# david-cortes/recometrics

Hardware: AMD Instinct MI355X
Metric: users/sec evaluated (all metrics, K=10) (higher is better)
Workload: dtype f32

## Files before the change

recometrics_amd/csrc/rm_device.hpp:

```cpp
#pragma once
#include <hip/hip_runtime.h>
#include <stdint.h>

namespace rm {

constexpr int WAVE = 64;
constexpr int GROUP_USERS = 32;
constexpr int TILE_ITEMS = 64;
constexpr int SWEEP_THREADS = 512;
constexpr int GROUPS_PER_BLOCK = 4;
constexpr int POS_CHUNK = 63;
constexpr int MAX_J = 6;
constexpr int STREAM_CLASS = MAX_J + 1;
constexpr int N_CLASSES = MAX_J + 2;
constexpr int IDX_EMPTY = 0x7fffffff;
constexpr int HEAVY_NPOS = 256;
enum : int { LM_LDS = 0, LM_HBM = 1, LM_HBM_APPEND = 2 };
constexpr int WAIT_VMCNT0 = 0x0F70;

enum : int { UF_NAN = 1, UF_ONLY_NDCG = 2, UF_KLEQN = 4, UF_ACTIVE = 8, UF_SKIP = 16 };

enum : int { RQ_P = 1, RQ_TP = 2, RQ_R = 4, RQ_AP = 8, RQ_TAP = 16, RQ_NDCG = 32, RQ_HIT = 64, RQ_RR = 128, RQ_ROC = 256, RQ_PR = 512 };

template <class T> struct Entry { T s; int idx; };
typedef Entry<float> ListEntry;

template <class T> struct PartialStat {
    T vmax, vmin;
    unsigned long long rocsum;
    int has_nan; int pad;
};

struct Plan {
    int n_active;
    int n_slots;
    int n_groups;
    int jmax;
    long long total_rows;
    int class_count[N_CLASSES];
    int class_offset[N_CLASSES + 1];
    int class_cursor[N_CLASSES];
    int n_long;
    int stream_enable;
    int max_npos;
    int n_stream_chunks;
    int nonfinite;
    int nonfinite_b;
    int n_noise_flagged;
    int n_heavy;
    int n_only_ndcg;
    unsigned long long amax_a, amax_b;
    int csr_bad;
    int csr_where;
    alignas(128) unsigned long long csr_desc_all[2];
    unsigned long long csr_desc_legit[2];
    unsigned long long csr_pad[12];
};
enum : int { CSR_BAD_INDPTR = 1, CSR_BAD_INDEX = 2, CSR_UNSORTED_TRAIN = 4, CSR_UNSORTED_TEST = 8 };

__device__ __forceinline__ float nan_sentinel_f() { return __int_as_float(0xffffffff); }
__device__ __forceinline__ float pos_inf_f() { return __int_as_float(0x7f800000); }
__device__ __forceinline__ float neg_inf_f() { return __int_as_float(0xff800000); }

__device__ __forceinline__ unsigned ord_key(float x) { const unsigned b = __float_as_uint(x); return b ^ ((b >> 31) ? 0xffffffffu : 0x80000000u); }
__device__ __forceinline__ float ord_unkey(unsigned k) { return __uint_as_float(k ^ ((k >> 31) ? 0x80000000u : 0xffffffffu)); }
__device__ __forceinline__ unsigned long long ord_key(double x)
{
    const unsigned long long b = (unsigned long long)__double_as_longlong(x);
    return b ^ ((b >> 63) ? 0xffffffffffffffffull : 0x8000000000000000ull);
}
__device__ __forceinline__ double ord_unkey(unsigned long long k)
{
    return __longlong_as_double((long long)(k ^ ((k >> 63) ? 0x8000000000000000ull : 0xffffffffffffffffull)));
}

template <class T> __device__ __forceinline__ T lane_bcast(T v, int src);
template <> __device__ __forceinline__ int lane_bcast<int>(int v, int src) { return __builtin_amdgcn_readlane(v, src); }
template <> __device__ __forceinline__ float lane_bcast<float>(float v, int src) { return __int_as_float(__builtin_amdgcn_readlane(__float_as_int(v), src)); }
template <> __device__ __forceinline__ double lane_bcast<double>(double v, int src)
{
    const long long b = __double_as_longlong(v);
    const unsigned lo = (unsigned)__builtin_amdgcn_readlane((int)(unsigned)b, src), hi = (unsigned)__builtin_amdgcn_readlane((int)(b >> 32), src);
    return __longlong_as_double((long long)(((unsigned long long)hi << 32) | lo));
}

__device__ __forceinline__ bool wave_any(bool c) { return __builtin_amdgcn_ballot_w64(c) != 0ull; }

template <class A> __device__ __forceinline__ const A *late_kernargs()
{
    auto p = __builtin_amdgcn_kernarg_segment_ptr();
    asm volatile("" : "+s"(p));
    return (const A *)p;
}
__device__ __forceinline__ constexpr int mfma32_row(int r, int h) { return (r & 3) + 8 * (r >> 2) + 4 * h; }

}
```

recometrics_amd/csrc/rm_finalize.hpp:

```cpp
#pragma once
#include "rm_device.hpp"
#include <type_traits>

namespace rm {

constexpr int MAX_PARTS = 128;
constexpr int FIN_THREADS = 128;
constexpr int FIN_TOPV = 64;
template <class T> inline size_t finalize_lds_bytes(int K, int n_part) { return (sizeof(T) * (size_t)(K < FIN_TOPV ? K : FIN_TOPV) + 4 * (size_t)n_part) * FIN_THREADS; }

struct AucPart { unsigned long long sum_ranks; double s1, s2; int nvalid, pad; };

template <class T, class S> struct FinalArgs {
    int m, n, K, n_part, req, cumulative, noise, gu, n_slots;
    const int *slot_user, *slot_chunk;
    const int *train_p, *test_p, *test_i; const T *test_v;
    const int *flags, *user_nslots, *uslot_base, *slot_index;
    const int *gj; const long long *grow;
    const Entry<S> *pl; const PartialStat<S> *pst; const unsigned *hist; const S *pos_score;
    const int *pos_item_tab;
    AucPart *auc_part;
    T *heavy_topv;
    unsigned char *heavy_nan;
    const int *heavy_users; int n_heavy;
    int heavy_npos, heavy_ld;
    const double *log2tab;
    T *p, *tp, *r, *ap, *tap, *ndcg, *hit, *rr, *roc, *pr;
    Entry<S> *merged;
    long long *rank_sorted;
    int *status;
    int stream_slot0;
    int rank_generic;
    int fin_slot0, fin_slot1;
    int fused_auc;
    int auc_defer_slot0;
    const S *stream_scores; long long stream_ld;
    const S *spos_score; const int *spos_item;
    unsigned *shist;
    int ext_topk; unsigned long long *sel_hi; unsigned *sel_lo; int sel_ld;
    int collected;
    int *noise_flag; Plan *plan;
};

template <class T> __device__ __forceinline__ T qnan();
template <> __device__ __forceinline__ float qnan<float>() { return __int_as_float(0x7fc00000); }
template <> __device__ __forceinline__ double qnan<double>() { return __longlong_as_double(0x7ff8000000000000ll); }

template <class T, class S>
__device__ void fill_user_nan(const FinalArgs<T, S> &a, int u)
{
    T *top8[8] = {a.p, a.tp, a.r, a.ap, a.tap, a.ndcg, a.hit, a.rr};
    for (int q = 0; q < 8; q++) {
        T *arr = top8[q];
        if (!arr) continue;
        if (!a.cumulative) arr[u] = qnan<T>();
        else for (int i = 0; i < a.K; i++) arr[(size_t)u * a.K + i] = qnan<T>();
    }
    if (a.roc) a.roc[u] = qnan<T>();
    if (a.pr) a.pr[u] = qnan<T>();
}

template <class S> __device__ __forceinline__ bool ent_before(const Entry<S> &x, const Entry<S> &y)
{
    return x.s > y.s || (x.s == y.s && x.idx < y.idx);
}

template <class T, class S>
__global__ void k_auc_slots(FinalArgs<T, S> a)
{
    const int slot = blockIdx.x * blockDim.x + threadIdx.x;
    if (slot >= a.stream_slot0) return;
    const int u = a.slot_user[slot], c = a.slot_chunk[slot];
    if (a.flags[u] & UF_ONLY_NDCG) return;
    const int te0 = a.test_p[u], npos = a.test_p[u + 1] - te0;
    const int GUr = a.gu;
    const int g = slot / GUr, ul = slot % GUr;
    const int PLg = (1 << a.gj[g]) - 1;
    const unsigned *H = a.hist + (a.grow[g] + g) * GUr + ul;
    const S *PS = a.pos_score + (a.grow[g] + g) * GUr + ul;
    const int pc = min(POS_CHUNK, npos - c * POS_CHUNK);
    unsigned long long above = 0, sum_ranks = 0;
    double s1 = 0, s2 = 0;
    int nvalid = 0;
    for (int b = PLg; b >= 1; b--) {
        above += H[(size_t)b * GUr];
        const int j = b - 1;
        if (j >= pc) continue;
        const S ps = PS[(size_t)j * GUr];
        if (isinf(ps) && ps > 0) continue;
        const unsigned long long rank = above + 1;
        sum_ranks += rank; nvalid++;
        s1 += 1. / (double)rank;
        s2 += (double)nvalid / (double)rank;
        if (a.rank_sorted) a.rank_sorted[te0 + c * POS_CHUNK + j] = (long long)rank;
    }
    AucPart r; r.sum_ranks = sum_ranks; r.s1 = s1; r.s2 = s2; r.nvalid = nvalid; r.pad = 0;
    a.auc_part[slot] = r;
}

constexpr int MERGE_WAVES = 4;
template <class T, class S>
__global__ __launch_bounds__(MERGE_WAVES * WAVE) void k_merge_positives(FinalArgs<T, S> a, int extra, int slot0)
{
    const int slot = slot0 + __builtin_amdgcn_readfirstlane((int)((blockIdx.x * blockDim.x + threadIdx.x) >> 6)), lane = threadIdx.x & 63;
    if (slot >= a.n_slots) return;
    const int u = a.slot_user[slot];
    const int K = a.K, NP = a.n_part;
    Entry<S> *L = (Entry<S> *)a.pl + ((size_t)slot * NP + extra) * K;
    S vmax = -(S)INFINITY, vmin = (S)INFINITY;
    int has_nan = 0, filled = 0;
    if (!(a.flags[u] & UF_ONLY_NDCG)) {
        const int te0 = a.test_p[u], npos = a.test_p[u + 1] - te0;
        const S *PS = a.spos_score + te0;
        const int *PI = a.spos_item + te0;
        for (int top = npos - 1; top >= 0; top -= WAVE) {
            const int i = top - lane;
            const S x = i >= 0 ? PS[i] : (S)INFINITY;
            const bool masked = isinf(x) && x > 0;
            const bool isn = x != x;
            const bool cand = !masked && !isn;
            has_nan |= isn ? 1 : 0;
            if (cand) {
                vmax = x > vmax ? x : vmax;
                vmin = x < vmin ? x : vmin;
                if (i >= 1) atomicAdd(&a.shist[te0 + i - 1], 1u);
            }
            if (filled < K) {
                const unsigned long long mk = __ballot(cand);
                const int pos = filled + __popcll(mk & ((1ull << lane) - 1ull));
                if (cand && pos < K) { L[pos].s = x; L[pos].idx = PI[i]; }
                filled += __popcll(mk);
            }
        }
    }
    #pragma unroll
    for (int d = 32; d >= 1; d >>= 1) {
        const S om = __shfl_xor(vmax, d), on = __shfl_xor(vmin, d);
        vmax = om > vmax ? om : vmax; vmin = on < vmin ? on : vmin;
        has_nan |= __shfl_xor(has_nan, d);
    }
    for (int i = (filled < K ? filled : K) + lane; i < K; i += WAVE) { L[i].s = -(S)INFINITY; L[i].idx = IDX_EMPTY; }
    if (lane == 0) {
        PartialStat<S> ps;
        ps.vmax = vmax; ps.vmin = vmin; ps.rocsum = 0; ps.has_nan = has_nan; ps.pad = 0;
        ((PartialStat<S> *)a.pst)[(size_t)slot * NP + extra] = ps;
    }
}

constexpr int STREAM_RANK_THREADS = 256;
constexpr int STREAM_RANK_ITEMS = 128;
constexpr int STREAM_RANK_LDS = 20 * 1024;
template <class S, int ILP, int LV>
__device__ __forceinline__ void rank_streamed_lds(const S *row, long long i0, int ipt, int n, const int *pit, int P, int top_rt, int lgsb_rt,
                                                  unsigned tab_addr, unsigned hist_addr)
{
    const int top = LV ? (1 << LV) : top_rt;
    const int lgsb = LV ? 14 - LV : lgsb_rt;
    typedef __attribute__((address_space(3))) const S *LdsS;
    typedef __attribute__((address_space(3))) unsigned *LdsU;
    const unsigned sb = 1u << lgsb;
    auto load_batch = [&](int it, S (&x)[ILP]) {
        #pragma unroll
        for (int q = 0; q < ILP; q++) {
            const long long item = i0 + (long long)(it + q) * STREAM_RANK_THREADS + threadIdx.x;
            x[q] = row[item < n ? item : n - 1];
        }
    };
    S nxt[ILP];
    load_batch(0, nxt);
    for (int it = 0; it < ipt; it += ILP) {
        S v[ILP]; unsigned o[ILP];
        #pragma unroll
        for (int q = 0; q < ILP; q++) {
            const long long item = i0 + (long long)(it + q) * STREAM_RANK_THREADS + threadIdx.x;
            v[q] = (nxt[q] == nxt[q] && item < n) ? nxt[q] : -(S)INFINITY; o[q] = 0;
        }
        load_batch(it + ILP, nxt);
        #pragma unroll
        for (unsigned st = ((unsigned)top >> 1) << lgsb; st >= sb; st >>= 1) {
            S pv[ILP];
            #pragma unroll
            for (int q = 0; q < ILP; q++) pv[q] = *(LdsS)(tab_addr + o[q] + st - sb);
            #pragma unroll
            for (int q = 0; q < ILP; q++) o[q] = (pv[q] < v[q]) ? o[q] + st : o[q];
        }
        S nx[ILP];
        #pragma unroll
        for (int q = 0; q < ILP; q++) nx[q] = *(LdsS)(tab_addr + o[q]);
        #pragma unroll
        for (int q = 0; q < ILP; q++) {
            int l = (int)(o[q] >> lgsb);
            if (nx[q] == v[q]) {
                const int item = (int)(i0 + (long long)(it + q) * STREAM_RANK_THREADS + threadIdx.x);
                while (l < P && *(LdsS)(tab_addr + ((unsigned)l << lgsb)) == v[q] && pit[l] > item) l++;
            }
            if (l >= 1) __hip_atomic_fetch_add((LdsU)(hist_addr + 4u * (unsigned)(l - 1)), 1u, __ATOMIC_RELAXED, __HIP_MEMORY_SCOPE_WORKGROUP);
        }
    }
}

template <class T, class S, class Count>
__device__ __forceinline__ void auc_walk_streamed(const FinalArgs<T, S> &a, int slot, int te0, int P, int lane, Count count)
{
    unsigned long long above = 0, sum_ranks = 0;
    double s2 = 0;
    int nvalid = 0;
    for (int base = P; base > 0; base -= WAVE) {
        const int j = base - 1 - lane;
        const bool live = j >= 0;
        const unsigned long long h = live ? (unsigned long long)count(j) : 0ull;
        unsigned long long incl = h;
        #pragma unroll
        for (int dd = 1; dd < WAVE; dd <<= 1) {
            const unsigned lo32 = (unsigned)__shfl_up((int)(unsigned)incl, dd), hi32 = (unsigned)__shfl_up((int)(unsigned)(incl >> 32), dd);
            if (lane >= dd) incl += ((unsigned long long)hi32 << 32) | lo32;
        }
        const S ps = live ? a.spos_score[te0 + j] : (S)0;
        const bool valid = live && !(isinf(ps) && ps > 0);
        const unsigned long long vm = __ballot(valid);
        const unsigned long long rank = above + incl + 1;
        const int myidx = nvalid + __popcll(vm & ((1ull << lane) - 1ull)) + 1;
        const double term = valid ? (double)myidx / (double)rank : 0.;
        unsigned long long rs = valid ? rank : 0ull;
        #pragma unroll
        for (int dd = 32; dd >= 1; dd >>= 1) {
            const unsigned lo32 = (unsigned)__shfl_xor((int)(unsigned)rs, dd), hi32 = (unsigned)__shfl_xor((int)(unsigned)(rs >> 32), dd);
            rs += ((unsigned long long)hi32 << 32) | lo32;
        }
        sum_ranks += rs;
        for (unsigned long long mm = vm; mm; mm &= mm - 1) s2 += lane_bcast<double>(term, __ffsll((long long)mm) - 1);
        if (a.rank_sorted && valid) a.rank_sorted[te0 + j] = (long long)rank;
        const int last = (base < WAVE ? base : WAVE) - 1;
        above += ((unsigned long long)(unsigned)__shfl((int)(unsigned)(incl >> 32), last) << 32) | (unsigned)__shfl((int)(unsigned)incl, last);
        nvalid += __popcll(vm);
    }
    if (lane == 0) { AucPart r; r.sum_ranks = sum_ranks; r.s1 = 0; r.s2 = s2; r.nvalid = nvalid; r.pad = 0; a.auc_part[slot] = r; }
}

template <class S>
__device__ __forceinline__ bool rank_block_walks(int fused_auc, int P)
{
    if (!(fused_auc & 1)) return false;
    constexpr int per = (int)sizeof(S) / 4;
    int top = 1;
    while (top <= P) top <<= 1;
    return (long long)top * per + P + 1 <= STREAM_RANK_LDS / 4;
}

#define RM_FCMP_LT(m, p, x) asm volatile("v_cmp_lt_f32 %0, %1, %2" : "=s"(m) : "v"(p), "v"(x))
#define RM_FCMP_LT_S(m, p, x) asm volatile("v_cmp_lt_f32 %0, %1, %2" : "=s"(m) : "s"(p), "v"(x))
#define RM_FSEL(d, a, b, m) asm volatile("v_cndmask_b32 %0, %1, %2, %3" : "=v"(d) : "v"(a), "v"(b), "s"(m))
template <int LV>
__device__ __forceinline__ void rank_streamed_fast(const float *row, int i0, int iters, const int *pit, int P, unsigned tab_addr, unsigned hist0_addr,
                                                   float piv_lo, float piv_root, float piv_hi)
{
    constexpr int ILP = 8;
    constexpr int LGSB = 14 - LV;
    constexpr unsigned SB = 1u << LGSB;
    constexpr unsigned Q = SB << (LV - 2);
    typedef __attribute__((address_space(3))) const float *LdsS;
    const float *src = row + i0 + (int)threadIdx.x;
    float nxt[ILP];
    #pragma unroll
    for (int q = 0; q < ILP; q++) nxt[q] = src[q * STREAM_RANK_THREADS];
    const unsigned a1 = tab_addr | Q, a2 = tab_addr | (2 * Q), a3 = tab_addr | (3 * Q);
    for (int it = 0; it < iters; it += ILP) {
        float v[ILP]; unsigned at[ILP];
        #pragma unroll
        for (int q = 0; q < ILP; q++) { v[q] = nxt[q]; at[q] = tab_addr; }
        src += ILP * STREAM_RANK_THREADS;
        if (it + ILP < iters) {
            #pragma unroll
            for (int q = 0; q < ILP; q++) nxt[q] = src[q * STREAM_RANK_THREADS];
        }
        unsigned long long mk0, mk1, mk2;
        #pragma unroll
        for (int i = 0; i < 3 * ILP + 2; i++) {
            if (i < 3 * ILP) {
                const float pv = i < ILP ? piv_lo : (i < 2 * ILP ? piv_root : piv_hi);
                if (i % 3 == 0) RM_FCMP_LT_S(mk0, pv, v[i % ILP]); else if (i % 3 == 1) RM_FCMP_LT_S(mk1, pv, v[i % ILP]); else RM_FCMP_LT_S(mk2, pv, v[i % ILP]);
            }
            if (i >= 2) {
                const int j = i - 2;
                const unsigned tgt = j < ILP ? a1 : (j < 2 * ILP ? a2 : a3);
                if (j % 3 == 0) RM_FSEL(at[j % ILP], at[j % ILP], tgt, mk0); else if (j % 3 == 1) RM_FSEL(at[j % ILP], at[j % ILP], tgt, mk1); else RM_FSEL(at[j % ILP], at[j % ILP], tgt, mk2);
            }
        }
        #pragma unroll
        for (int st = 1 << (LV - 3); st >= 1; st >>= 1) {
            float pv[ILP];
            #pragma unroll
            for (int q = 0; q < ILP; q++) pv[q] = *(LdsS)(at[q] + (unsigned)(st - 1) * SB);
            #pragma unroll
            for (int i = 0; i < ILP + 2; i++) {
                if (i == 0) __builtin_amdgcn_s_waitcnt(0xC47F); else if (i == 4) __builtin_amdgcn_s_waitcnt(0xC07F);
                if (i < ILP) { if (i % 3 == 0) RM_FCMP_LT(mk0, pv[i], v[i]); else if (i % 3 == 1) RM_FCMP_LT(mk1, pv[i], v[i]); else RM_FCMP_LT(mk2, pv[i], v[i]); }
                if (i >= 2) {
                    const int j = i - 2;
                    const unsigned cand = at[j] | ((unsigned)st * SB);
                    if (j % 3 == 0) RM_FSEL(at[j], at[j], cand, mk0); else if (j % 3 == 1) RM_FSEL(at[j], at[j], cand, mk1); else RM_FSEL(at[j], at[j], cand, mk2);
                }
            }
        }
        float nx[ILP];
        #pragma unroll
        for (int q = 0; q < ILP; q++) nx[q] = *(LdsS)(at[q]);
        bool tie = false;
        #pragma unroll
        for (int q = 0; q < ILP; q++) tie |= nx[q] == v[q];
        if (__any(tie)) {
            #pragma unroll
            for (int q = 0; q < ILP; q++) {
                if (nx[q] == v[q]) {
                    const int item = i0 + (it + q) * STREAM_RANK_THREADS + (int)threadIdx.x;
                    int l = (int)((at[q] - tab_addr) >> LGSB);
                    while (l < P && *(LdsS)(tab_addr + ((unsigned)l << LGSB)) == v[q] && pit[l] > item) l++;
                    at[q] = tab_addr + ((unsigned)l << LGSB);
                }
            }
        }
        const unsigned one = 1u;
        #pragma unroll
        for (int q = 0; q < ILP; q++) {
            const unsigned ha = hist0_addr + (((at[q] - tab_addr) >> LGSB) << 2);
            asm volatile("ds_add_u32 %0, %1" :: "v"(ha), "v"(one) : "memory");
        }
    }
    __builtin_amdgcn_s_waitcnt(0xC07F);
}

template <class T, class S>
__global__ __launch_bounds__(STREAM_RANK_THREADS) void k_rank_streamed(FinalArgs<T, S> a, int parts, int ipt, int row0)
{
    __shared__ __attribute__((aligned(16384))) char rk_smem[STREAM_RANK_LDS];
    const int d = row0 + blockIdx.x / parts, part = blockIdx.x % parts;
    const int slot = a.stream_slot0 + d;
    const int u = a.slot_user[slot];
    if (a.flags[u] & UF_ONLY_NDCG) return;
    const int te0 = a.test_p[u], P = a.test_p[u + 1] - te0;
    constexpr int WORDS = STREAM_RANK_LDS / 4;
    constexpr int per = (int)sizeof(S) / 4;
    int top = 1;
    while (top <= P) top <<= 1;
    int R = 0;
    if ((long long)top * per + P + 1 <= WORDS) { R = 1; while (R < 32 && (long long)top * 2 * R * per + P + 1 <= WORDS) R *= 2; }
    const int *pit = a.spos_item + te0;
    const S *row = a.stream_scores + (size_t)d * (size_t)a.stream_ld;
    const long long i0 = (long long)part * STREAM_RANK_THREADS * ipt;
    if (R > 0) {
        S *lds_s = (S *)rk_smem;
        unsigned *lds_h = (unsigned *)(rk_smem + sizeof(S) * (size_t)top * (size_t)R) + 1;
        for (int i = threadIdx.x; i < top * R; i += STREAM_RANK_THREADS) { const int e = i / R; lds_s[i] = e < P ? a.spos_score[te0 + e] : (S)INFINITY; }
        for (int i = threadIdx.x; i < P; i += STREAM_RANK_THREADS) lds_h[i] = 0u;
        __syncthreads();
        int lgsb = sizeof(S) == 4 ? 2 : 3;
        for (int r = R; r > 1; r >>= 1) lgsb++;
        const unsigned tab_addr = (unsigned)(size_t)(__attribute__((address_space(3))) char *)rk_smem + (unsigned)((threadIdx.x & (R - 1)) * sizeof(S));
        const unsigned hist_addr = (unsigned)(size_t)(__attribute__((address_space(3))) char *)lds_h;
        const bool full = (long long)top * R == 4096 / per;
        if (sizeof(S) == 4 && full && top >= 128 && top <= 1024 && !a.rank_generic) {
            const int inside = (int)((a.n - i0) / STREAM_RANK_THREADS);
            const int iters = inside <= 0 ? 0 : (inside < ipt ? inside : ipt) / 8 * 8;
            if (iters > 0) {
                const float *tabf = (const float *)lds_s;
                const float p_lo = tabf[(top / 4 - 1) * R], p_root = tabf[(top / 2 - 1) * R], p_hi = tabf[(3 * top / 4 - 1) * R];
                const float s_lo = __builtin_bit_cast(float, __builtin_amdgcn_readfirstlane(__builtin_bit_cast(int, p_lo)));
                const float s_root = __builtin_bit_cast(float, __builtin_amdgcn_readfirstlane(__builtin_bit_cast(int, p_root)));
                const float s_hi = __builtin_bit_cast(float, __builtin_amdgcn_readfirstlane(__builtin_bit_cast(int, p_hi)));
                const float *rowf = (const float *)row;
                const unsigned h0 = hist_addr - 4u;
                if (top == 128) rank_streamed_fast<7>(rowf, (int)i0, iters, pit, P, tab_addr, h0, s_lo, s_root, s_hi);
                else if (top == 256) rank_streamed_fast<8>(rowf, (int)i0, iters, pit, P, tab_addr, h0, s_lo, s_root, s_hi);
                else if (top == 512) rank_streamed_fast<9>(rowf, (int)i0, iters, pit, P, tab_addr, h0, s_lo, s_root, s_hi);
                else rank_streamed_fast<10>(rowf, (int)i0, iters, pit, P, tab_addr, h0, s_lo, s_root, s_hi);
            }
            if (iters < ipt) rank_streamed_lds<S, 8, 0>(row, i0 + (long long)iters * STREAM_RANK_THREADS, ipt - iters, a.n, pit, P, top, lgsb, tab_addr, hist_addr);
// ... 120 lines not shown
            }
            __syncthreads();
        }
    }
    for (int i = tid; i < K; i += SELECT_THREADS) {
        Entry<S> e;
        if (i < got) { e.s = ord_unkey((KeyT)hi[i]); e.idx = (int)~lo[i]; }
        else { e.s = (S)qnan<float>(); e.idx = -1; }
        M[i] = e;
    }
}

struct CollectGeom {
    int ublock0, n_ublocks, n_splits, tail_ublocks, tail_splits;
    int nsub, gu, lpu;
    int lane_cap;
    int extra_part;
};
template <class S> struct CollectKey;
template <> struct CollectKey<float> { typedef unsigned T; };
template <> struct CollectKey<double> { typedef unsigned long long T; };
inline int collect_capw(int K, int lane_cap) { return K <= 128 ? 512 : (K + lane_cap <= 1024 && 2 * K <= 1024 ? 1024 : 4096); }
constexpr int COLLECT_MAX_ENTRIES = 4096;
inline unsigned collect_grid(long long blocks) { return (unsigned)((blocks + 7) / 8 * 8); }
template <class T, class S, class ThrT, int CAPW>
__global__ __launch_bounds__(CAPW <= 1024 ? 256 : 64) void k_collect_topk(FinalArgs<T, S> a, CollectGeom g, const char *glists, const int *lane_cnt, const ThrT *thr_shared)
{
    typedef typename CollectKey<S>::T KeyT;
    constexpr int WPB = CAPW <= 1024 ? 4 : 1;
    __shared__ KeyT kh_all[WPB * CAPW];
    __shared__ unsigned kl_all[WPB * CAPW];
    const int lane = threadIdx.x & 63, wv_in_blk = __builtin_amdgcn_readfirstlane(threadIdx.x >> 6);
    const int per_xcd = gridDim.x >> 3;
    const int lblock = (blockIdx.x & 7) * per_xcd + (blockIdx.x >> 3);
    const int slot = lblock * WPB + wv_in_blk;
    if (slot >= a.n_slots) return;
    const int chunk = a.slot_chunk[slot], u = a.slot_user[slot];
    const ThrT bound_raw = thr_shared[slot];
    const bool live = chunk == 0;
    KeyT *kh = kh_all + wv_in_blk * CAPW;
    unsigned *kl = kl_all + wv_in_blk * CAPW;
    const int K = a.K;
    const int group = slot / g.gu, ul = slot % g.gu, gi = group % GROUPS_PER_BLOCK, blk_u = group / GROUPS_PER_BLOCK;
    const int nwaves = GROUPS_PER_BLOCK * g.nsub;
    const int rel = blk_u - g.ublock0, n_ub1 = g.n_ublocks - g.tail_ublocks;
    const bool in_tail = rel < g.tail_ublocks;
    const int nsplit = in_tail ? g.tail_splits : g.n_splits;
    const KeyT bound = (KeyT)bound_raw;
    int cur = 0;
    auto wave_sync = [&]() { __builtin_amdgcn_fence(__ATOMIC_ACQ_REL, "wavefront"); __builtin_amdgcn_wave_barrier(); };
    auto select_best = [&]() __attribute__((always_inline)) {
        if (cur <= K) return;
        wave_sync();
        constexpr int ROWS = CAPW / WAVE;
        KeyT kr[ROWS];
        #pragma unroll
        for (int r = 0; r < ROWS; r++) { const int i = r * WAVE + lane; kr[r] = i < cur ? kh[i] : (KeyT)0; }
        KeyT all_and = ~(KeyT)0, all_or = 0;
        #pragma unroll
        for (int r = 0; r < ROWS; r++) if (r * WAVE + lane < cur) { all_and &= kr[r]; all_or |= kr[r]; }
        #pragma unroll
        for (int d = 32; d >= 1; d >>= 1) { all_and &= __shfl_xor(all_and, d); all_or |= __shfl_xor(all_or, d); }
        const KeyT diff = all_and ^ all_or;
        constexpr int BITS = (int)sizeof(KeyT) * 8;
        int top = BITS - 1;
        while (top >= 0 && !((diff >> top) & 1)) top--;
        KeyT Tk = top >= 0 ? (all_and & ~(((KeyT)2 << top) - 1)) : all_and;
        for (int bit = top; bit >= 0; bit--) {
            const KeyT cand = Tk | ((KeyT)1 << bit);
            int c = 0;
            #pragma unroll
            for (int r = 0; r < ROWS; r++) c += __popcll(__ballot(kr[r] >= cand));
            if (c >= K) Tk = cand;
        }
        int n_gt = 0, n_eq = 0;
        #pragma unroll
        for (int r = 0; r < ROWS; r++) {
            const bool in = r * WAVE + lane < cur;
            n_gt += __popcll(__ballot(in && kr[r] > Tk)); n_eq += __popcll(__ballot(in && kr[r] == Tk));
        }
        const int need = K - n_gt;
        unsigned Lk = 0u;
        if (n_eq > need) {
            const int rows = (cur + WAVE - 1) / WAVE;
            for (int bit = 31; bit >= 0; bit--) {
                const unsigned cand = Lk | (1u << bit);
                int c = 0;
                for (int r = 0; r < rows; r++) { const int i = r * WAVE + lane; c += __popcll(__ballot(i < cur && kh[i] == Tk && kl[i] >= cand)); }
                if (c >= need) Lk = cand;
            }
        }
        int out = 0;
        #pragma unroll
        for (int r = 0; r < ROWS; r++) {
            if (r * WAVE >= cur) break;
            const int i = r * WAVE + lane;
            const KeyT x = kr[r]; const unsigned y = i < cur ? kl[i] : 0u;
            const bool keep = i < cur && (x > Tk || (x == Tk && y >= Lk));
            const unsigned long long m = __ballot(keep);
            if (keep) { const int at = out + __popcll(m & ((1ull << lane) - 1ull)); kh[at] = x; kl[at] = y; }
            out += __popcll(m);
        }
        cur = out;
        wave_sync();
    };
    auto sort_regs = [&](auto pr_tag) __attribute__((always_inline)) {
        constexpr int PR = decltype(pr_tag)::value, P = PR * WAVE;
        KeyT h[PR]; unsigned l[PR];
        #pragma unroll
        for (int r = 0; r < PR; r++) { const int i = r * WAVE + lane; const bool in = i < cur; h[r] = in ? kh[i] : (KeyT)0; l[r] = in ? kl[i] : 0u; }
        #pragma unroll
        for (int k2 = 2; k2 <= P; k2 <<= 1) {
            #pragma unroll
            for (int j = k2 >> 1; j > 0; j >>= 1) {
                if (j >= WAVE) {
                    const int jr = j / WAVE;
                    #pragma unroll
                    for (int r = 0; r < PR; r++) {
                        if (r & jr) continue;
                        const bool desc = (r & (k2 / WAVE)) == 0;
                        const bool lt = h[r] < h[r | jr] || (h[r] == h[r | jr] && l[r] < l[r | jr]);
                        if (desc ? lt : !lt) { const KeyT th = h[r]; h[r] = h[r | jr]; h[r | jr] = th; const unsigned tl = l[r]; l[r] = l[r | jr]; l[r | jr] = tl; }
                    }
                } else {
                    #pragma unroll
                    for (int r = 0; r < PR; r++) {
                        const KeyT oh = __shfl_xor(h[r], j); const unsigned ol = __shfl_xor(l[r], j);
                        const bool take_max = ((lane & j) == 0) == ((((r * WAVE) | lane) & k2) == 0);
                        const bool other_better = oh > h[r] || (oh == h[r] && ol > l[r]);
                        if (take_max ? other_better : !other_better) { h[r] = oh; l[r] = ol; }
                    }
                }
            }
        }
        #pragma unroll
        for (int r = 0; r < PR; r++) { kh[r * WAVE + lane] = h[r]; kl[r * WAVE + lane] = l[r]; }
        wave_sync();
    };
    auto sort_kept = [&]() __attribute__((always_inline)) {
        wave_sync();
        if (CAPW <= 1024) {
            if (cur <= 64) sort_regs(std::integral_constant<int, 1>{});
            else if (cur <= 128) sort_regs(std::integral_constant<int, 2>{});
            else if (cur <= 256) sort_regs(std::integral_constant<int, 4>{});
            else sort_regs(std::integral_constant<int, 8>{});
        } else {
            if (cur <= 512) sort_regs(std::integral_constant<int, 8>{});
            else if (cur <= 1024) sort_regs(std::integral_constant<int, 16>{});
            else sort_regs(std::integral_constant<int, 32>{});
        }
    };
    auto reduce = [&]() __attribute__((always_inline)) { select_best(); };
    auto gather = [&](int c, auto get) __attribute__((always_inline)) {
        for (int i0 = 0; i0 < c; i0 += WAVE) {
            if (cur + WAVE > CAPW) reduce();
            KeyT key = 0; unsigned low = 0u;
            const bool take = i0 + lane < c && get(i0 + lane, key, low);
            const unsigned long long m = __ballot(take);
            if (take) { const int at = cur + __popcll(m & ((1ull << lane) - 1ull)); kh[at] = key; kl[at] = low; }
            cur += __popcll(m);
        }
    };
    constexpr int G = 4;
    constexpr bool PAIRS = sizeof(S) == 4;
    const int per_range = g.nsub * g.lpu, nsrc = nsplit * per_range;
    const char *bs[G]; const int *bi[G]; int cn[G]; int cmax = 0;
    auto describe = [&](int s0) __attribute__((always_inline)) {
        size_t cidx[G]; bool on[G];
        #pragma unroll
        for (int j = 0; j < G; j++) {
            const int src = s0 + j;
            on[j] = src < nsrc;
            const int srcc = on[j] ? src : 0;
            const int sp = srcc / per_range, rem = srcc % per_range, sub = rem / g.lpu, l = rem % g.lpu;
            const int bidx = in_tail ? n_ub1 * g.n_splits + sp * g.tail_ublocks + (g.tail_ublocks - 1 - rel)
                                     : sp * n_ub1 + (g.n_ublocks - 1 - rel);
            const size_t wv = (size_t)bidx * nwaves + (size_t)(sub * GROUPS_PER_BLOCK + gi);
            const int src_lane = ul + l * g.gu;
            const char *wbase = glists + wv * ((size_t)g.lane_cap * WAVE * (sizeof(S) + 4));
            cidx[j] = wv * WAVE + src_lane;
            bs[j] = wbase + (size_t)src_lane * (PAIRS ? 8 : sizeof(S));
            bi[j] = (const int *)(wbase + (size_t)g.lane_cap * WAVE * sizeof(S)) + src_lane;
        }
        int c[G];
        #pragma unroll
        for (int j = 0; j < G; j++) c[j] = lane_cnt[cidx[j]];
        cmax = 0;
        #pragma unroll
        for (int j = 0; j < G; j++) { cn[j] = (live && on[j]) ? c[j] : 0; cmax = cn[j] > cmax ? cn[j] : cmax; }
    };
    describe(0);
    if (g.extra_part >= 0) {
        const Entry<S> *px = a.pl + ((size_t)slot * a.n_part + g.extra_part) * K;
        gather(live ? K : 0, [&](int i, KeyT &key, unsigned &low) {
            Entry<S> e;
            __builtin_memcpy(&e, px + i, sizeof(e));
            if (e.idx == IDX_EMPTY) return false;
            key = ord_key(e.s); low = ~(unsigned)e.idx;
            return true;
        });
    }
    for (int s0 = 0; s0 < nsrc; s0 += G) {
        if (s0) describe(s0);
        for (int i0 = 0; i0 < cmax; i0 += WAVE) {
            if (cur + G * WAVE > CAPW) reduce();
            const int i = i0 + lane;
            S sc[G]; int it[G];
            #pragma unroll
            for (int j = 0; j < G; j++) {
                sc[j] = (S)0; it[j] = 0;
                if (i < cn[j]) {
                    if (PAIRS) {
                        const uint2 e = *(const uint2 *)(bs[j] + (size_t)i * (WAVE * 8));
                        sc[j] = (S)__uint_as_float(e.x); it[j] = (int)e.y;
                    } else {
                        sc[j] = *(const S *)(bs[j] + (size_t)i * (WAVE * sizeof(S)));
                        it[j] = bi[j][(size_t)i * WAVE];
                    }
                }
            }
            #pragma unroll
            for (int j = 0; j < G; j++) {
                const KeyT key = ord_key(sc[j]);
                const bool take = i < cn[j] && key >= bound;
                const unsigned long long m = __ballot(take);
                if (take) { const int at = cur + __popcll(m & ((1ull << lane) - 1ull)); kh[at] = key; kl[at] = ~(unsigned)it[j]; }
                cur += __popcll(m);
            }
        }
    }
    wave_sync();
    select_best();
    sort_kept();
    if (!live) return;
    Entry<S> *M = a.merged + (size_t)u * K;
    for (int i = lane; i < K; i += WAVE) {
        Entry<S> e;
        if (i < cur) { e.s = ord_unkey(kh[i]); e.idx = (int)~kl[i]; }
        else { e.s = (S)qnan<float>(); e.idx = -1; }
        M[i] = e;
    }
}

template <class T, class S>
__global__ void k_auc_streamed(FinalArgs<T, S> a, int row0, int row1)
{
    const int w = row0 + __builtin_amdgcn_readfirstlane((blockIdx.x * blockDim.x + threadIdx.x) >> 6), lane = threadIdx.x & 63;
    if (w >= row1) return;
    const int slot = a.stream_slot0 + w;
    const int u = a.slot_user[slot];
    if (a.flags[u] & UF_ONLY_NDCG) return;
    const int te0 = a.test_p[u], P = a.test_p[u + 1] - te0;
    if (rank_block_walks<S>(a.fused_auc, P)) return;
    const unsigned *sh = a.shist + te0;
    auc_walk_streamed<T, S>(a, slot, te0, P, lane, [&](int j) { return sh[j]; });
}

template <class T, class S>
__global__ void k_top_values(FinalArgs<T, S> a)
{
    const int w = __builtin_amdgcn_readfirstlane((blockIdx.x * blockDim.x + threadIdx.x) >> 6), lane = threadIdx.x & 63;
    if (w >= a.n_heavy) return;
    const int u = a.heavy_users[w];
    const int te0 = a.test_p[u], npos = a.test_p[u + 1] - te0;
    const int L = a.K < npos ? a.K : npos;
    if (L > a.heavy_ld) return;
    const T *tv = a.test_v + te0;
    T *out = a.heavy_topv + (size_t)u * a.heavy_ld;
    bool any_nan = false;
    T pv = 0; int pi = -1;
    constexpr int CACHE = 32;
    const bool cached = npos <= WAVE * CACHE;
    T xv[CACHE];
    if (cached) {
        #pragma unroll
        for (int i = 0; i < CACHE; i++) xv[i] = lane + WAVE * i < npos ? tv[lane + WAVE * i] : (T)0;
    }
    for (int r = 0; r < L; r++) {
        bool found = false; T bv = 0; int bi = 0x7fffffff;
        auto consider = [&](T x, int t) {
            if (r == 0) any_nan |= x != x;
            if (r > 0 && !(x < pv || (x == pv && t > pi))) return;
            if (!found || x > bv) { found = true; bv = x; bi = t; }
        };
        if (cached) {
            #pragma unroll
            for (int i = 0; i < CACHE; i++) if (lane + WAVE * i < npos) consider(xv[i], lane + WAVE * i);
        } else {
            for (int t = lane; t < npos; t += WAVE) consider(tv[t], t);
        }
        #pragma unroll
        for (int d = 32; d >= 1; d >>= 1) {
            const T ov = __shfl_xor(bv, d); const int oi = __shfl_xor(bi, d); const bool of = __shfl_xor((int)found, d) != 0;
            if (of && (!found || ov > bv || (ov == bv && oi < bi))) { found = true; bv = ov; bi = oi; }
        }
        pv = bv; pi = bi;
        if (lane == 0) out[r] = bv;
    }
    const unsigned long long nm = __ballot(any_nan);
    if (lane == 0) a.heavy_nan[u] = nm ? 1 : 0;
}

template <class T, class S>
__global__ void k_finalize_skipped(FinalArgs<T, S> a)
{
    const int u = blockIdx.x * blockDim.x + threadIdx.x;
    if (u >= a.m || !(a.flags[u] & UF_NAN)) return;
    const int te0 = a.test_p[u], npos = a.test_p[u + 1] - te0;
    if (a.status) a.status[u] = 1;
    Entry<S> *M = a.merged + (size_t)u * a.K;
    for (int i = 0; i < a.K; i++) { M[i].s = (S)qnan<float>(); M[i].idx = -1; }
    fill_user_nan(a, u);
}

template <class T, class S>
__device__ __forceinline__ void finalize_auc(const FinalArgs<T, S> &a, int u, int base, int npos, int C)
{
    const int nsl = a.user_nslots[u];
    unsigned long long sum_ranks = 0; int h = 0; double ap_full = 0;
    for (int c = nsl - 1; c >= 0; c--) {
        const AucPart r = a.auc_part[a.slot_index[base + c]];
        sum_ranks += r.sum_ranks;
        ap_full = nsl == 1 ? r.s2 : ap_full + ((double)h * r.s1 + r.s2);
        h += r.nvalid;
    }
    const unsigned long long P = (unsigned long long)npos, Nneg = (unsigned long long)C - P;
    if (a.roc) a.roc[u] = (T)(1. - (double)(sum_ranks - (P * (P + 1)) / 2) / (double)(P * Nneg));
    if (a.pr) a.pr[u] = (T)(ap_full / (double)npos);
}

template <class T, class S>
__global__ void k_finalize_auc(FinalArgs<T, S> a)
{
    const int slot = a.auc_defer_slot0 + blockIdx.x * blockDim.x + threadIdx.x;
    if (slot >= a.n_slots || a.slot_chunk[slot] != 0) return;
    const int u = a.slot_user[slot];
    const T probe = a.roc ? a.roc[u] : a.pr[u];
    if (probe != probe) return;
    const int npos = a.test_p[u + 1] - a.test_p[u];
    const int C = a.n - (a.train_p[u + 1] - a.train_p[u]);
    finalize_auc(a, u, a.uslot_base[u], npos, C);
}

template <class T, class S>
__global__ void k_finalize(FinalArgs<T, S> a)
{
    extern __shared__ __attribute__((aligned(16))) char fin_smem[];
    T *topv_base = (T *)fin_smem;
    unsigned short *head_base = (unsigned short *)(fin_smem + sizeof(T) * (a.K < FIN_TOPV ? a.K : FIN_TOPV) * FIN_THREADS);
    const int slot = a.fin_slot0 + blockIdx.x * blockDim.x + threadIdx.x;
    if (slot >= a.fin_slot1 || a.slot_chunk[slot] != 0) return;
    const int u = a.slot_user[slot];
    const int K = a.K, n = a.n;
    const int f = a.flags[u];
    const int te0 = a.test_p[u], npos = a.test_p[u + 1] - te0;
    if (a.status) a.status[u] = 1;
    Entry<S> *M = a.merged + (size_t)u * K;
    const bool merged_ready = a.ext_topk || a.collected;
    if (!merged_ready) for (int i = 0; i < K; i++) { M[i].s = (S)qnan<float>(); M[i].idx = -1; }

    const int ntr = a.train_p[u + 1] - a.train_p[u];
    const int C = n - ntr;
    const bool only_ndcg = f & UF_ONLY_NDCG, kleqn = f & UF_KLEQN;
    const int base = a.uslot_base[u];
    const int s0 = a.slot_index[base];
    const int NP = a.n_part;

    unsigned short *head = head_base + threadIdx.x;
    unsigned short *alive = head_base + (size_t)NP * FIN_THREADS + threadIdx.x;
    S vmax = -(S)INFINITY, vmin = (S)INFINITY; bool any_nan = false;
    const Entry<S> *PL = a.pl + (size_t)s0 * NP * K;
    int n_alive = 0;
    for (int q = 0; q < NP; q++) {
        const bool empty = !merged_ready && PL[(size_t)q * K].idx == IDX_EMPTY;
        head[q * FIN_THREADS] = empty ? (unsigned short)K : (unsigned short)0;
        if (!empty) alive[(n_alive++) * FIN_THREADS] = (unsigned short)q;
        const PartialStat<S> ps = a.pst[(size_t)s0 * NP + q];
        vmax = ps.vmax > vmax ? ps.vmax : vmax;
        vmin = ps.vmin < vmin ? ps.vmin : vmin;
        any_nan |= ps.has_nan != 0;
    }
    for (int i = 0; i < (merged_ready ? 0 : K); i++) {
        int best = -1; Entry<S> be; be.s = 0; be.idx = 0;
        for (int t = 0; t < n_alive; t++) {
            const int q = alive[t * FIN_THREADS];
            const int hq = head[q * FIN_THREADS];
            if (hq >= K) continue;
            const Entry<S> e = PL[(size_t)q * K + hq];
            if (best < 0 || ent_before(e, be)) { best = q; be = e; }
        }
        if (best >= 0) head[best * FIN_THREADS]++;
        else be.idx = IDX_EMPTY;
        if (be.idx == IDX_EMPTY) { be.idx = -1; be.s = (S)qnan<float>(); }
        M[i] = be;
    }
    const int W = K < C ? K : C;

    const bool ref_full = ((a.req & RQ_ROC) && !only_ndcg) || K >= C;
    bool invalid = any_nan;
    if (a.noise) invalid |= (vmax == vmin) || isinf(vmax) || isinf(vmin);
    else {
        const S hi = M[0].s, lo = ref_full ? vmin : M[W - 1].s;
        invalid |= isinf(hi) || isinf(lo) || hi == lo || M[W - 1].idx < 0;
    }
    if (invalid) {
        for (int i = 0; i < K; i++) { M[i].s = (S)qnan<float>(); M[i].idx = -1; }
        if (a.rank_sorted) for (int t = 0; t < npos; t++) a.rank_sorted[te0 + t] = 0;
        fill_user_nan(a, u); return;
    }
    if (a.status) a.status[u] = 0;
    if (a.noise_flag) {
        bool zone = false;
        for (int i = 0; i < W; i++) { const S x = M[i].s; zone |= (x < (S)0 ? -x : x) < (S)6.103515625e-05f; }
        if (zone && atomicExch(&a.noise_flag[u], 1) == 0) atomicAdd(&a.plan->n_noise_flagged, 1);
    }

    const int *ti = a.test_i + te0;
    const T *tv = a.test_v ? a.test_v + te0 : nullptr;
    const size_t st = (size_t)u * K;
    T *cp = a.p ? a.p + st : nullptr, *ctp = a.tp ? a.tp + st : nullptr, *cr = a.r ? a.r + st : nullptr;
    T *cap = a.ap ? a.ap + st : nullptr, *ctap = a.tap ? a.tap + st : nullptr, *cndcg = a.ndcg ? a.ndcg + st : nullptr;
    T *chit = a.hit ? a.hit + st : nullptr, *crr = a.rr ? a.rr + st : nullptr;
    const bool cum = a.cumulative;

    const bool top = a.req & (RQ_P | RQ_TP | RQ_R | RQ_AP | RQ_TAP | RQ_NDCG | RQ_HIT | RQ_RR);
    bool walked = false;
    int hits = 0, first = 0x7fffffff;
    double avg_p = 0, dcg = 0;
    if (top && (!kleqn || (a.req & (RQ_AP | RQ_TAP | RQ_RR | RQ_NDCG)))) {
        walked = true;
        for (int ix = 0; ix < W; ix++) {
            const int item = M[ix].idx;
            int lo = 0, hi = npos;
            while (lo < hi) { const int mid = (lo + hi) >> 1; if (ti[mid] < item) lo = mid + 1; else hi = mid; }
            if (lo < npos && ti[lo] == item) {
                hits++;
                avg_p += hits / (double)(ix + 1);
                dcg += tv ? ((double)tv[lo] / a.log2tab[ix]) : 0.;
                first = first < ix ? first : ix;
            }
            if (cum) {
                const int mn = (ix + 1) < npos ? (ix + 1) : npos;
                if (cp) cp[ix] = (T)(hits / (double)(ix + 1));
                if (ctp) ctp[ix] = (T)(hits / (double)mn);
                if (cr) cr[ix] = (T)(hits / (double)npos);
                if (cap) cap[ix] = (T)(avg_p / (double)npos);
                if (ctap) ctap[ix] = (T)(avg_p / (double)mn);
                if (cndcg) cndcg[ix] = (T)dcg;
                if (chit) chit[ix] = (T)(hits > 0);
                if (crr) crr[ix] = (T)(hits ? ((double)1 / (double)(first + 1)) : 0.);
            }
        }
        if (!cum) {
            const int mn = K < npos ? K : npos;
            if (a.p) a.p[u] = (T)((double)hits / (double)K);
            if (a.tp) a.tp[u] = (T)((double)hits / (double)mn);
            if (a.r) a.r[u] = (T)((double)hits / (double)npos);
            if (a.ap) a.ap[u] = (T)(avg_p / (double)npos);
            if (a.tap) a.tap[u] = (T)(avg_p / (double)mn);
            if (a.hit) a.hit[u] = (T)(hits > 0);
            if (a.rr) a.rr[u] = (T)(hits ? (1. / (double)(first + 1)) : 0.);
        } else if (K > C) {
            for (int i = C; i < K; i++) {
                if (cp) cp[i] = qnan<T>(); if (ctp) ctp[i] = qnan<T>(); if (cr) cr[i] = qnan<T>(); if (chit) chit[i] = qnan<T>();
                if (cap) cap[i] = cap[C - 1]; if (ctap) ctap[i] = ctap[C - 1]; if (crr) crr[i] = crr[C - 1]; if (cndcg) cndcg[i] = cndcg[C - 1];
            }
        }
    }

    if (kleqn) {
        if (!cum) {
            if (a.p) a.p[u] = qnan<T>(); if (a.tp) a.tp[u] = qnan<T>(); if (a.r) a.r[u] = qnan<T>(); if (a.hit) a.hit[u] = qnan<T>();
        } else if (!walked) {
            for (int i = 0; i < K; i++) { if (cp) cp[i] = qnan<T>(); if (ctp) ctp[i] = qnan<T>(); if (cr) cr[i] = qnan<T>(); if (chit) chit[i] = qnan<T>(); }
        }
    } else if (only_ndcg) {
        if (!cum) {
            if (a.p) a.p[u] = qnan<T>(); if (a.tp) a.tp[u] = qnan<T>(); if (a.r) a.r[u] = qnan<T>(); if (a.ap) a.ap[u] = qnan<T>();
            if (a.tap) a.tap[u] = qnan<T>(); if (a.hit) a.hit[u] = qnan<T>(); if (a.rr) a.rr[u] = qnan<T>();
        } else {
            for (int i = 0; i < K; i++) {
                if (cp) cp[i] = qnan<T>(); if (ctp) ctp[i] = qnan<T>(); if (cr) cr[i] = qnan<T>(); if (cap) cap[i] = qnan<T>();
                if (ctap) ctap[i] = qnan<T>(); if (chit) chit[i] = qnan<T>(); if (crr) crr[i] = qnan<T>();
            }
        }
    }

    if (only_ndcg) {
        if (a.roc) a.roc[u] = qnan<T>();
        if (a.pr) a.pr[u] = qnan<T>();
    } else if (a.req & (RQ_ROC | RQ_PR)) {
        if (slot >= a.auc_defer_slot0) {
            if (a.roc) a.roc[u] = (T)0;
            if (a.pr) a.pr[u] = (T)0;
        } else finalize_auc(a, u, base, npos, C);
    }

    if (a.ndcg) {
        const int L = K < npos ? K : npos;
        constexpr int TOPV = FIN_TOPV;
        T *topv = topv_base + threadIdx.x;
        bool has_nan_val = false;
        const bool buffered = L <= TOPV;
        auto pick_next = [&](bool have_prev, T pv, int pi, T &ov, int &oi) {
            bool found = false; T bv = 0; int bi = -1;
            for (int t = 0; t < npos; t++) {
                const T x = tv[t];
                if (have_prev && !(x < pv || (x == pv && t > pi))) continue;
                if (!found || x > bv) { found = true; bv = x; bi = t; }
            }
            ov = bv; oi = bi; return found;
        };
        const bool listed = a.heavy_topv && npos > a.heavy_npos && L <= a.heavy_ld;
        const T *hv = listed ? a.heavy_topv + (size_t)u * a.heavy_ld : nullptr;
        if (listed) has_nan_val = a.heavy_nan[u] != 0;
        if (listed && buffered) {
            for (int i = 0; i < L; i++) topv[i * FIN_THREADS] = hv[i];
        } else if (listed) {
        } else if (buffered) {
            int cnt = 0;
            T kth = 0;
            for (int t0 = 0; t0 < npos; t0 += 8) {
                T xb[8];
                #pragma unroll
                for (int q = 0; q < 8; q++) xb[q] = t0 + q < npos ? tv[t0 + q] : (T)0;
                #pragma unroll
                for (int q = 0; q < 8; q++) {
                    if (t0 + q >= npos) break;
                    const T x = xb[q];
                    has_nan_val |= x != x;
                    if (cnt < L || x > kth) {
                        int j = cnt < L ? cnt : L - 1;
                        while (j > 0 && topv[(j - 1) * FIN_THREADS] < x) { topv[j * FIN_THREADS] = topv[(j - 1) * FIN_THREADS]; j--; }
                        topv[j * FIN_THREADS] = x;
                        cnt = cnt < L ? cnt + 1 : cnt;
                        if (cnt == L) kth = topv[(L - 1) * FIN_THREADS];
                    }
                }
            }
        } else {
            for (int t = 0; t < npos; t++) has_nan_val |= tv[t] != tv[t];
        }
        T pv = 0; int pi = -1; bool hp = false;
        auto next_value = [&](int i) -> T {
            if (buffered) return topv[i * FIN_THREADS];
            if (listed) return hv[i];
            T x; int xi; pick_next(hp, pv, pi, x, xi); hp = true; pv = x; pi = xi; return x;
        };
        T vmaxv = 0, vlast = 0;
        if (buffered) { vmaxv = topv[0]; vlast = topv[(L - 1) * FIN_THREADS]; }
        else if (listed) { vmaxv = hv[0]; vlast = hv[L - 1]; }
        else {
            for (int i = 0; i < L; i++) { const T x = next_value(i); if (i == 0) vmaxv = x; vlast = x; }
            hp = false; pv = 0; pi = -1;
        }
        if (has_nan_val || isinf(vmaxv) || isinf(vlast) || vmaxv <= 0) {
            if (!cum) a.ndcg[u] = qnan<T>(); else for (int i = 0; i < K; i++) cndcg[i] = qnan<T>();
            return;
        }
        double idcg = 0;
        if (!cum) {
            for (int ix = 0; ix < L; ix++) {
                const T x = next_value(ix);
                if (!(vlast >= 0) && x <= 0) break;
                idcg += (double)x / a.log2tab[ix];
            }
            a.ndcg[u] = (T)(dcg / idcg);
        } else {
            if (vlast >= 0) {
                for (int ix = 0; ix < L; ix++) {
                    const T x = next_value(ix);
                    idcg += (double)x / a.log2tab[ix];
                    cndcg[ix] = (T)((double)cndcg[ix] / idcg);
                }
            } else {
                int ix = 0;
                for (; ix < L; ix++) {
                    const T x = next_value(ix);
                    if (x < 0) break;
                    idcg += (double)x / a.log2tab[ix];
                    cndcg[ix] = (T)((double)cndcg[ix] / idcg);
                }
                for (; ix < L; ix++) cndcg[ix] = (T)((double)cndcg[ix] / idcg);
            }
            if (npos < K) { const int e = K < C ? K : C; for (int i = npos; i < e; i++) cndcg[i] = cndcg[npos - 1]; }
        }
    }
}

template <class S> struct RecoArgs {
    int m, n, K, n_part;
    const int *flags, *uslot_base, *slot_index, *train_p;
    const Entry<S> *pl; const PartialStat<S> *pst;
    const Entry<S> *merged;
    int *idx; S *score; int *status;
};
constexpr int RECO_THREADS = 128, RECO_CHUNK = 16, RECO_LD = RECO_CHUNK + 1;
template <class S> inline size_t reco_lds_bytes(int n_part, bool merged_ready)
{
    return merged_ready ? 0 : (sizeof(S) + 4) * (size_t)RECO_THREADS * RECO_LD + 4 * (size_t)n_part * RECO_THREADS;
}

template <class S>
__global__ __launch_bounds__(RECO_THREADS) void k_finalize_reco(RecoArgs<S> a)
{
    extern __shared__ __attribute__((aligned(16))) char reco_smem[];
    __shared__ int len_s[RECO_THREADS];
    const int tid = threadIdx.x;
    const long long u0 = (long long)blockIdx.x * RECO_THREADS;
    const int users_here = (int)(a.m - u0 < RECO_THREADS ? a.m - u0 : RECO_THREADS);
    const int u = (int)u0 + tid;
    const int K = a.K, NP = a.n_part;
    const bool active = tid < users_here && (a.flags[u] & UF_ACTIVE);
    int s0 = 0, W = 0, status = 1;
    if (active) {
        s0 = a.slot_index[a.uslot_base[u]];
        const int C = a.n - (a.train_p[u + 1] - a.train_p[u]);
        S vmax = -(S)INFINITY, vmin = (S)INFINITY; bool any_nan = false;
        for (int q = 0; q < NP; q++) {
            const PartialStat<S> ps = a.pst[(size_t)s0 * NP + q];
            vmax = ps.vmax > vmax ? ps.vmax : vmax;
            vmin = ps.vmin < vmin ? ps.vmin : vmin;
            any_nan |= ps.has_nan != 0;
        }
        status = (any_nan || vmax == (S)INFINITY || vmin == -(S)INFINITY) ? 2 : 0;
        W = status ? 0 : (K < C ? K : C);
    }
    if (tid < users_here) a.status[u] = status;
    const size_t out0 = (size_t)u0 * K;
    if (a.merged) {
        len_s[tid] = W;
        __syncthreads();
        const long long total = (long long)users_here * K;
        for (long long e = tid; e < total; e += RECO_THREADS) {
            const int ul = (int)(e / K), p = (int)(e - (long long)ul * K);
            Entry<S> be; be.s = (S)qnan<float>(); be.idx = -1;
            if (p < len_s[ul]) be = a.merged[out0 + e];
            a.idx[out0 + e] = be.idx;
            if (a.score) a.score[out0 + e] = be.s;
        }
        return;
    }
    S *tile_s = (S *)reco_smem;
    int *tile_i = (int *)(reco_smem + sizeof(S) * RECO_THREADS * RECO_LD);
    unsigned short *head_base = (unsigned short *)(tile_i + RECO_THREADS * RECO_LD);
    unsigned short *head = head_base + tid, *alive = head_base + (size_t)NP * RECO_THREADS + tid;
    const Entry<S> *PL = a.pl + (size_t)s0 * NP * K;
    int n_alive = 0;
    if (W > 0) {
        for (int q = 0; q < NP; q++) {
            const bool empty = PL[(size_t)q * K].idx == IDX_EMPTY;
            head[q * RECO_THREADS] = empty ? (unsigned short)K : (unsigned short)0;
            if (!empty) alive[(n_alive++) * RECO_THREADS] = (unsigned short)q;
        }
    }
    for (int c0 = 0; c0 < K; c0 += RECO_CHUNK) {
        const int kc = K - c0 < RECO_CHUNK ? K - c0 : RECO_CHUNK;
        for (int i = 0; i < kc; i++) {
            Entry<S> be; be.s = (S)qnan<float>(); be.idx = -1;
            if (c0 + i < W) {
                int best = -1;
                for (int t = 0; t < n_alive; t++) {
                    const int q = alive[t * RECO_THREADS];
                    const int hq = head[q * RECO_THREADS];
                    if (hq >= K) continue;
                    const Entry<S> e = PL[(size_t)q * K + hq];
                    if (best < 0 || ent_before(e, be)) { best = q; be = e; }
                }
                if (best >= 0) head[best * RECO_THREADS]++;
                if (best < 0 || be.idx == IDX_EMPTY) { be.s = (S)qnan<float>(); be.idx = -1; }
            }
            tile_s[tid * RECO_LD + i] = be.s; tile_i[tid * RECO_LD + i] = be.idx;
        }
        __syncthreads();
        for (int e = tid; e < users_here * kc; e += RECO_THREADS) {
            const int ul = e / kc, p = e - ul * kc;
            const size_t at = out0 + (size_t)ul * K + c0 + p;
            a.idx[at] = tile_i[ul * RECO_LD + p];
            if (a.score) a.score[at] = tile_s[ul * RECO_LD + p];
        }
        __syncthreads();
    }
}

}
```

recometrics_amd/csrc/rm_lib.hip:

```cpp
#include <hip/hip_runtime.h>

#include <algorithm>
#include <array>
#include <cmath>
#include <cstdio>
#include <cstring>
#include <cstdlib>
#include <type_traits>
#include <atomic>
#include <chrono>
#include <condition_variable>
#include <csignal>
#include <functional>
#include <limits>
#include <map>
#include <memory>
#include <mutex>
#include <string>
#include <thread>
#include <vector>

#include "../../include/recometrics_hip.h"
#include "rm_device.hpp"
#include "rm_prep.hpp"
#include "rm_launch.hpp"
#include "rm_finalize.hpp"
#include "rm_noise.hpp"

namespace {

using namespace rm;

thread_local std::string g_err;
struct RmError { int code; std::string msg; };

#define HIP_CHECK(expr)                                                                                   \
    do {                                                                                                  \
        hipError_t e_ = (expr);                                                                           \
        if (e_ != hipSuccess)                                                                             \
            throw RmError{e_ == hipErrorOutOfMemory ? RM_ERR_NOMEM : RM_ERR_HIP,                          \
                          std::string(#expr) + ": " + hipGetErrorString(e_)};                             \
    } while (0)

struct Switches {
    bool no_train_bits, no_spec, no_side, ext_topk, no_test_mask, hbm_lists, nsub2, no_pending, no_pos_beside, no_seed, rank_generic,
         no_fused_auc, no_defer_auc, noise_sequential, one_context, noise_per_batch, host_trace, no_pos_flat;
    long long free_mb, stream_budget_mb, noise_budget_mb, lane_cap_min, lane_min_k, lane_cap_set, sample_seed;
    double batch_users;
    std::string splits;
    static bool on(const char *name) { return getenv(name) != nullptr; }
    static long long num(const char *name) { const char *e = getenv(name); return e ? atoll(e) : -1; }
    void load()
    {
        no_train_bits = on("RM_DEBUG_NO_TRAIN_BITS"); no_spec = on("RM_DEBUG_NO_SPEC"); no_side = on("RM_DEBUG_NO_SIDE");
        ext_topk = on("RM_DEBUG_EXT_TOPK"); no_test_mask = on("RM_DEBUG_NO_TEST_MASK");
        hbm_lists = on("RM_DEBUG_HBM_LISTS"); nsub2 = on("RM_DEBUG_NSUB2"); no_pending = on("RM_DEBUG_NO_PENDING");
        no_pos_beside = on("RM_DEBUG_NO_POS_BESIDE"); no_seed = on("RM_DEBUG_NO_SEED");
        rank_generic = on("RM_DEBUG_RANK_GENERIC"); no_fused_auc = on("RM_DEBUG_NO_FUSED_AUC");
        no_defer_auc = on("RM_DEBUG_NO_DEFER_AUC"); noise_sequential = on("RM_DEBUG_NOISE_SEQUENTIAL");
        one_context = on("RM_DEBUG_ONE_CONTEXT"); noise_per_batch = on("RM_DEBUG_NOISE_PER_BATCH"); host_trace = on("RM_HOST_TRACE");
        no_pos_flat = on("RM_DEBUG_NO_POS_FLAT");
        free_mb = num("RM_DEBUG_FREE_MB"); stream_budget_mb = num("RM_STREAM_BUDGET_MB");
        noise_budget_mb = num("RM_NOISE_BUDGET_MB");
        lane_min_k = num("RM_DEBUG_LANE_MIN_K");
        lane_cap_set = num("RM_DEBUG_LANE_CAP");
        sample_seed = num("RM_DEBUG_SAMPLE_SEED");
        lane_cap_min = num("RM_DEBUG_LANE_CAP_MIN");
        const char *b = getenv("RM_BATCH_USERS"); batch_users = b ? atof(b) : 0.0;
        const char *s = getenv("RM_DEBUG_SPLITS"); splits = s ? s : "";
    }
    Switches() { load(); }
};
Switches g_sw;

std::atomic<long long> g_ws_bytes{0};
inline long long debug_free_cap()
{
    return g_sw.free_mb >= 0 ? (g_sw.free_mb << 20) : -1;
}

struct RunTrace {
    std::mutex mu; std::vector<std::pair<const char *, double>> pts; std::chrono::steady_clock::time_point t0 = std::chrono::steady_clock::now();
    void point(const char *what) { std::lock_guard<std::mutex> lk(mu); if (pts.size() > 4096) pts.clear(); pts.emplace_back(what, std::chrono::duration<double, std::milli>(std::chrono::steady_clock::now() - t0).count()); }
};
RunTrace g_run_trace;
#define RM_TRACE_POINT(what) do { if (g_sw.host_trace) g_run_trace.point(what); } while (0)

std::atomic<unsigned long long> g_ws_stamp{1};
struct Workspace {
    struct Buf { void *ptr = nullptr; size_t bytes = 0; unsigned long long stamp = 0; };
    std::map<std::string, Buf> bufs;
    void *get(const std::string &name, size_t bytes)
    {
        bytes = std::max<size_t>(bytes, 256);
        Buf &b = bufs[name];
        if (b.bytes < bytes) {
            if (b.ptr) { (void)hipFree(b.ptr); g_ws_bytes -= (long long)b.bytes; b = Buf{}; }
            const size_t cap = bytes + bytes / 8;
            const long long sim = debug_free_cap();
            if (sim >= 0 && g_ws_bytes.load() + (long long)cap > sim)
                throw RmError{RM_ERR_NOMEM, "hipMalloc(" + name + ", " + std::to_string(cap) + " B): beyond RM_DEBUG_FREE_MB"};
            hipError_t e = hipMalloc(&b.ptr, cap);
            if (e != hipSuccess) { b.ptr = nullptr; throw RmError{RM_ERR_NOMEM, "hipMalloc(" + name + ", " + std::to_string(cap) + " B): " + hipGetErrorString(e)}; }
            b.bytes = cap; b.stamp = g_ws_stamp.fetch_add(1);
            g_ws_bytes += (long long)cap;
        }
        return b.ptr;
    }
    Buf peek(const char *name) const { auto it = bufs.find(name); return it == bufs.end() ? Buf{} : it->second; }
    void release()
    {
        for (auto &kv : bufs) if (kv.second.ptr) { (void)hipFree(kv.second.ptr); g_ws_bytes -= (long long)kv.second.bytes; }
        bufs.clear();
    }
};
struct PackedItems {
    unsigned long long stamp = 0, tag = 0; int tile = 0, ng = 0;
    unsigned long long amax_b = 0; int nonfinite_b = 0;
    bool of_call(unsigned long long t) const { return t != 0 && t == tag; }
    bool holds(const Workspace &ws, unsigned long long t, int tile_items, int NG) const { return of_call(t) && stamp == ws.peek("Bp").stamp && tile == tile_items && ng == NG; }
    void set(const Workspace &ws, unsigned long long t, int tile_items, int NG) { stamp = ws.peek("Bp").stamp; tag = t; tile = tile_items; ng = NG; }
    void invalidate() { stamp = 0; tag = 0; }
};
struct DenseRows {
    unsigned long long stamp = 0; long long words = 0; int m = 0;
    bool masked = false, partial = false;
    unsigned long long tag = 0; const int *train_p = nullptr;
    bool valid(const Workspace &ws) const { return stamp != 0 && stamp == ws.peek("train_bits").stamp; }
    bool fits(const Workspace &ws, int m_, long long words_, bool masked_) const { return valid(ws) && !partial && words == words_ && m == m_ && masked == masked_; }
    bool built_by(const Workspace &ws, unsigned long long t, const int *train_p_, int m_) const { return valid(ws) && t != 0 && t == tag && train_p == train_p_ && m == m_ && !partial; }
    const unsigned *rows(const Workspace &ws) const { return (const unsigned *)ws.peek("train_bits").ptr; }
    void set(const Workspace &ws, long long words_, int m_, bool masked_, bool partial_, unsigned long long t, const int *train_p_)
    { stamp = ws.peek("train_bits").stamp; words = words_; m = m_; masked = masked_; partial = partial_; tag = t; train_p = train_p_; }
    void invalidate() { stamp = 0; tag = 0; }
};
struct DiscountTable {
    unsigned long long stamp = 0; int K = 0;
    bool holds(const Workspace &ws, int K_) const { return stamp != 0 && stamp == ws.peek("log2tab").stamp && K >= K_; }
    void set(const Workspace &ws, int K_) { stamp = ws.peek("log2tab").stamp; K = K_; }
};
enum SideMark { SIDE_FORK, SIDE_JOIN, SIDE_PLAN_FORK, SIDE_CHECKS_DONE, SIDE_ROWS_AND_PACKS, SIDE_ROWS_FOR_POS, SIDE_TOP_VALUES,
                SIDE_SWEEP_FORK, SIDE_SWEEP_DEEP_DONE, SIDE_MERGED, SIDE_MARKS };
enum PosMark { POS_PLAN_FORK, POS_MAXIMA_DONE, POS_SCORES_AFTER_COPY, POS_SCORES_DONE, POS_TABLES_INIT, POS_STREAMED_PLACED, POS_MARKS };
enum PassEvent { EV_START, EV_PREP_END , EV_SWEEP_END, EV_END, EV_COUNT };
struct NoiseWords {
    int first_early;
    int first_final;
    int sequential;
    int range_early;
    int batch_flagged;
};
static_assert(sizeof(NoiseWords) <= 64, "the noise words share one 64-byte page-locked allocation");
struct Ctx {
    int device = 0, slot = 0;
    std::mutex mu;
    Workspace ws;
    hipEvent_t ev[EV_COUNT] = {nullptr, nullptr, nullptr, nullptr};
    bool ev_valid = false, ev_recorded = false;
    hipStream_t side_stream = nullptr; std::array<hipEvent_t, SIDE_MARKS> side_marks{};
    hipStream_t pos_stream = nullptr; std::array<hipEvent_t, POS_MARKS> pos_marks{};
    hipEvent_t done = nullptr;
    hipStream_t own_stream = nullptr;
    hipStream_t up_stream = nullptr;
    hipEvent_t up_ev[2] = {nullptr, nullptr};
    NoiseWords *noise_words = nullptr; hipEvent_t flags_ev = nullptr, pass_ev = nullptr;
    void need_noise_words()
    {
        if (noise_words) return;
        HIP_CHECK(hipHostMalloc((void **)&noise_words, 64, hipHostMallocDefault));
        HIP_CHECK(hipEventCreateWithFlags(&flags_ev, hipEventDisableTiming));
        HIP_CHECK(hipEventCreateWithFlags(&pass_ev, hipEventDisableTiming));
    }
    void *pinned = nullptr; size_t pinned_bytes = 0;
    void *pinned_get(size_t bytes)
    {
        if (pinned_bytes < bytes) {
            if (pinned) { (void)hipHostFree(pinned); pinned = nullptr; pinned_bytes = 0; }
            if (hipHostMalloc(&pinned, bytes + bytes / 8, hipHostMallocDefault) != hipSuccess) { pinned = nullptr; throw RmError{RM_ERR_NOMEM, "hipHostMalloc of the output staging buffer failed"}; }
            pinned_bytes = bytes + bytes / 8;
        }
        return pinned;
    }
    double timings[8] = {0, 0, 0, 0, 0, 0, 0, 0};
    int timed_slots = 0, total_slots = 0;
    double acc[4] = {0, 0, 0, 0};
    PackedItems packed; DenseRows dense; DiscountTable discounts;
    bool high_priority = false;
    Plan *pinned_plan = nullptr;
    void stage_ms(float ms[4]) const
    {
        const int from[4] = {EV_START, EV_PREP_END, EV_SWEEP_END, EV_START}, to[4] = {EV_PREP_END, EV_SWEEP_END, EV_END, EV_END};
        for (int i = 0; i < 4; i++) (void)hipEventElapsedTime(&ms[i], ev[from[i]], ev[to[i]]);
    }
};
inline hipError_t create_stream(hipStream_t *st, bool high_priority)
{
    if (high_priority) {
        int least = 0, greatest = 0;
        if (hipDeviceGetStreamPriorityRange(&least, &greatest) == hipSuccess && greatest != least)
            return hipStreamCreateWithPriority(st, hipStreamNonBlocking, greatest);
        (void)hipGetLastError();
    }
    return hipStreamCreateWithFlags(st, hipStreamNonBlocking);
}
std::mutex g_ctx_mu;
std::map<std::pair<int, int>, std::unique_ptr<Ctx>> g_ctx;
thread_local Ctx *g_last_ctx = nullptr;

Ctx &context(int slot)
{
    int dev = 0;
    HIP_CHECK(hipGetDevice(&dev));
    std::lock_guard<std::mutex> lk(g_ctx_mu);
    auto &p = g_ctx[std::make_pair(dev, slot)];
    if (!p) { p.reset(new Ctx()); p->device = dev; p->slot = slot; }
    return *p;
}
constexpr int PEER_SLOT = 1 << 12, NOISE_SLOT = 1 << 13;
Ctx &peer_context(const Ctx &cx, int offset = PEER_SLOT)
{
    std::lock_guard<std::mutex> lk(g_ctx_mu);
    auto &p = g_ctx[std::make_pair(cx.device, cx.slot + offset)];
    if (!p) { p.reset(new Ctx()); p->device = cx.device; p->slot = cx.slot + offset; p->high_priority = offset == NOISE_SLOT; }
    return *p;
}

template <class T> struct Call {
    const T *A; size_t lda; const T *B; size_t ldb;
    int m, n, k;
    const int *train_p, *train_i; long long nnz_train;
    const int *test_p, *test_i; const T *test_v; long long nnz_test;
    int K; bool cumulative, noise;
    T *out[10];
    bool cold; int min_items_pool, min_pos_test;
    int *topk_idx; T *topk_score; long long *pos_rank; int *status;
    unsigned long long items_tag;
    unsigned long long seed; long long user0;
    const unsigned char *only_users;
    const int *noise_row; int noise_row0;
    const T *noise_E; long long noise_ld;
    int *noise_flag;
    bool same_train_rows = false;
    long long eval_users = -1;
    int *flag_snapshot = nullptr; int *flag_count_host = nullptr; hipEvent_t flags_event = nullptr;
    const unsigned *ext_bits = nullptr; long long ext_words = 0; bool ext_masked = false;
    int *first_pass_flags = nullptr;
    bool csr_checked = false;
    int dense_fit = -1;
    bool reco = false;
};
struct MetricLayout {
    bool want[10]; size_t per, rec_off[10], rec_w = 0;
    template <class P> MetricLayout(P *const *outs, size_t per_) : per(per_)
    {
        for (int i = 0; i < 10; i++) { want[i] = outs[i] != nullptr; rec_off[i] = rec_w; if (want[i]) rec_w += width(i); }
    }
    size_t width(int i) const { return i >= 8 ? 1 : per; }
    size_t block_off(int i, size_t users) const { return rec_off[i] * users; }
    size_t block_size(size_t users) const { return rec_w * users; }
    template <class T> void point_at(T *block, size_t users, T **out) const { for (int i = 0; i < 10; i++) out[i] = want[i] ? block + block_off(i, users) : nullptr; }
};
template <class T>
inline void set_exact_pass(Call<T> &c, const unsigned char *only, const int *noise_row, int row0, const T *E, long long ld, int rows)
{
    c.only_users = only; c.noise_row = noise_row; c.noise_row0 = row0; c.noise_E = E; c.noise_ld = ld; c.eval_users = rows;
    c.noise_flag = nullptr; c.first_pass_flags = nullptr; c.flag_snapshot = nullptr;
    c.csr_checked = true;
}
constexpr int RM_INTERNAL_UNSORTED = 1000;

inline unsigned cdiv(long long a, long long b) { return (unsigned)((a + b - 1) / b); }

template <class T> __global__ void k_iota(T *p, int count)
{
    const int i = blockIdx.x * blockDim.x + threadIdx.x;
    if (i < count) p[i] = (T)i;
}

template <class S>
__global__ void k_export_rank(int m, int K, const Entry<S> *merged, int *topk_idx, S *topk_score, const int *flags)
{
    const long long i = (long long)blockIdx.x * blockDim.x + threadIdx.x;
    if (i >= (long long)m * K || (flags[i / K] & UF_SKIP)) return;
    topk_idx[i] = merged[i].idx;
    topk_score[i] = merged[i].s;
}

__global__ void k_export_pos_rank(long long nnz, int m, const int *test_p, const int *flags, const int *pos_order,
                                  const long long *rank_sorted, long long *pos_rank, int have_ranks, const int *status)
{
    const int u = blockIdx.x * blockDim.x + threadIdx.x;
    if (u >= m || (flags[u] & UF_SKIP)) return;
    const bool ranked = have_ranks && (flags[u] & UF_ACTIVE) && !(flags[u] & UF_ONLY_NDCG) && !(status && status[u] == 1);
    for (int e = test_p[u]; e < test_p[u + 1]; e++) pos_rank[e] = ranked ? rank_sorted[test_p[u] + pos_order[e]] : 0;
}

template <class T> struct Prec;
template <> struct Prec<float> {
    static constexpr int GU = GROUP_USERS;
    typedef float4 PackT;  typedef u32x2 ListT;  typedef SweepArgs Args;
    static int supported_ng(int k) { const int ng = (k + 7) / 8; for (int o : {2, 3, 4, 5, 6, 7, 8, 10, 12, 13, 16, 32, 64}) if (ng <= o) return o; return (ng + 15) / 16 * 16; }
    static const char *limit() { return "unsupported factor count"; }
    static size_t lds_b(int NG, int tile = TILE_ITEMS) { return 2ull * std::min(NG, 16) * 2 * tile * 16; }
    static long long items_units(int tiles, int NG, int tile = TILE_ITEMS) { return (long long)tiles * NG * 2 * tile; }
    static long long users_units(int groups, int NG) { return (long long)groups * NG * 2 * GU; }
    static constexpr bool has_pending = true, pending_for_append = false;
    static constexpr size_t pend_key_bytes = 8;
    static constexpr int pend_cap_max = 8;
    static constexpr int max_nsub = 3;
    static size_t lists_b(int, int K) { return (size_t)GROUPS_PER_BLOCK * (K + 2) * GU * 8; }
    static void set_pending(SweepArgs &sa, int cap, int off) { sa.pend_cap = cap; sa.pend_off = off; }
    static void set_sync(SweepArgs &sa, int off) { sa.sync_off = off; }
    static void set_ublocks(SweepArgs &sa, int first, int count) { sa.ublock0 = first; sa.n_ublocks = count; }
    static int lane_cap(int K) { return (2 * K + 16 + 15) / 16 * 16; }
    static constexpr int lanes_per_user = 2, lane_tile = 16;
};
template <> struct Prec<double> {
    static constexpr int GU = GROUP_USERS64;
    typedef double2 PackT;  typedef u32x4 ListT;  typedef Sweep64Args Args;
    static int supported_ng(int k) { const int ng = (k + 7) / 8; for (int o : {2, 3, 4, 5, 6, 7, 8, 16, 32, 64}) if (ng <= o) return o; return (ng + 7) / 8 * 8; }
    static const char *limit() { return "unsupported factor count"; }
    static size_t lds_b(int NG, int = TILE_ITEMS) { return 2ull * std::min(NG, 8) * 4 * TILE_ITEMS * 16; }
    static long long items_units(int tiles, int NG, int = TILE_ITEMS) { return (long long)tiles * NG * 4 * TILE_ITEMS; }
    static long long users_units(int groups, int NG) { return (long long)groups * NG * 4 * GU; }
    static constexpr bool has_pending = true, pending_for_append = true;
    static constexpr size_t pend_key_bytes = 12;
    static constexpr int pend_cap_max = 3;
    static constexpr int max_nsub = 2;
    static size_t lists_b(int ns, int K) { return 4ull * ns * K * GU * sizeof(ListT); }
    static void set_pending(Sweep64Args &sa, int cap, int off) { sa.pend_cap = cap; sa.pend_off = off; }
    static void set_sync(Sweep64Args &sa, int off) { sa.sync_off = off; }
    static void set_ublocks(Sweep64Args &sa, int first, int count) { sa.ublock0 = first; sa.n_ublocks = count; }
    static int lane_cap(int K) { return (K + lane_sel_slack(K) + 8 + 16 + 15) / 16 * 16; }
    static constexpr int lanes_per_user = 4, lane_tile = 8;
};

inline void check_launch(int rc)
{
    if (rc == -1) throw RmError{RM_ERR_UNSUPPORTED, "unsupported factor count"};
    if (rc != 0) throw RmError{RM_ERR_HIP, std::string("sweep launch: ") + hipGetErrorString((hipError_t)rc)};
}
inline void dispatch_sweep(bool auc, bool dump, bool llds, int nsub, int NG, dim3 grid, size_t lds, hipStream_t stream, const SweepArgs &sa)
{
    check_launch(launch_sweep32(auc, dump, llds ? 0 : (sa.buffered_lists ? 2 : 1), nsub, NG, grid, lds, stream, sa));
}
inline void dispatch_sweep(bool auc, bool dump, bool llds, int, int NG, dim3 grid, size_t lds, hipStream_t stream, const Sweep64Args &sa)
{
    check_launch(launch_sweep64(auc, dump, llds ? 0 : (sa.buffered_lists ? 2 : 1), NG, grid, lds, stream, sa));
}

inline void pack_operands(const float *A, size_t lda, const float *B, size_t ldb, int n, int k, int NG, int tile_items, const int *slot_user,
                          int n_slots, float4 *Ap, long long ap, float4 *Bp, long long bp, hipStream_t stream, bool items = true)
{
    if (items) {
        const size_t lds = pack_items_tile_lds(NG, tile_items);
        const long long tiles = bp / ((long long)NG * 2 * tile_items);
        bool tiled = lds <= 96 * 1024 && tiles * NG * 2 * tile_items == bp;
        if (tiled && lds > 48 * 1024)
            tiled = hipFuncSetAttribute((const void *)k_pack_items_tile<float>, hipFuncAttributeMaxDynamicSharedMemorySize, (int)lds) == hipSuccess;
        if (tiled) {
            hipLaunchKernelGGL(k_pack_items_tile<float>, dim3((unsigned)tiles), dim3(256), lds, stream, B, ldb, n, k, NG, tile_items, Bp);
            if (hipGetLastError() != hipSuccess) tiled = false;
        }
        if (!tiled) hipLaunchKernelGGL(k_pack_items<float>, dim3(cdiv(bp, 256)), dim3(256), 0, stream, B, ldb, n, k, NG, tile_items, Bp, bp);
    }
    if (ap > 0) hipLaunchKernelGGL(k_pack_users<float>, dim3(cdiv(ap, 256)), dim3(256), 0, stream, A, lda, k, NG, slot_user, n_slots, Ap, ap);
}
inline void pack_operands(const double *A, size_t lda, const double *B, size_t ldb, int n, int k, int NG, int, const int *slot_user,
                          int n_slots, double2 *Ap, long long ap, double2 *Bp, long long bp, hipStream_t stream, bool items = true)
{
    if (items) hipLaunchKernelGGL(k_pack_items64<double>, dim3(cdiv(bp, 256)), dim3(256), 0, stream, B, ldb, n, k, NG, Bp, bp);
    if (ap > 0) hipLaunchKernelGGL(k_pack_users64<double>, dim3(cdiv(ap, 256)), dim3(256), 0, stream, A, lda, k, NG, slot_user, n_slots, Ap, ap);
}

constexpr size_t LDS_LIMIT = 160 * 1024;
constexpr size_t SYNC_BYTES = 32;

inline long long free_plus_owned(const Workspace &ws, std::initializer_list<const char *> names)
{
    size_t fr = 0, tot = 0;
    HIP_CHECK(hipMemGetInfo(&fr, &tot));
    const long long sim = debug_free_cap();
    if (sim >= 0) fr = (size_t)std::max<long long>(0, std::min<long long>((long long)fr, sim - g_ws_bytes.load()));
    long long owned = 0;
    for (const char *nm : names) { auto it = ws.bufs.find(nm); if (it != ws.bufs.end()) owned += (long long)it->second.bytes; }
    return (long long)fr + owned;
}
inline long long stream_budget_bytes(const Workspace &ws)
{
    if (g_sw.stream_budget_mb >= 0) return g_sw.stream_budget_mb << 20;
    return free_plus_owned(ws, {"stream_scores", "sel_hi", "sel_lo"}) / 3;
}

template <class T> inline long long lane_list_bytes(int K, long long n_blocks) { return n_blocks * 8 * WAVE * (long long)Prec<T>::lane_cap(K) * (long long)(sizeof(T) + 4); }
template <class T> inline bool lane_lists_possible(int K, bool three_subtiles = false)
{
    const long long min_k = g_sw.lane_min_k >= 0 ? g_sw.lane_min_k : (three_subtiles ? 20 : (sizeof(T) == 8 ? 1 : 14));
    return !g_sw.ext_topk && K >= min_k && K + Prec<T>::lane_cap(K) <= COLLECT_MAX_ENTRIES;
}
template <class T> inline long long lane_blocks_bound(long long m) { return (m + 4 * Prec<T>::GU - 1) / (4 * Prec<T>::GU) + 1024; }
inline long long lane_budget_bytes(const Workspace &ws) { return free_plus_owned(ws, {"glists", "stream_scores", "sel_hi", "sel_lo"}) / 3; }
template <class T> inline bool lane_lists_fit(const Workspace &ws, int K, long long m, bool three_subtiles)
{
    return lane_lists_possible<T>(K, three_subtiles) && lane_list_bytes<T>(K, lane_blocks_bound<T>(m)) <= lane_budget_bytes(ws);
}

inline long long dense_row_words(long long n) { return (n + 191) / 192 * 6; }
inline bool dense_rows_fit(const Workspace &ws, int m, long long n)
{
    const long long words = dense_row_words(n);
    if (words > TRAIN_BITS_MAX_WORDS || g_sw.no_train_bits) return false;
    const unsigned long long bytes = (unsigned long long)m * (unsigned long long)words * 4ull;
    if (bytes <= (1ull << 30)) return true;
    if (bytes > (8ull << 30)) return false;
    return (long long)bytes <= free_plus_owned(ws, {"train_bits", "stream_scores", "sel_hi", "sel_lo"}) / 4;
}
template <class C> inline void set_train_bits(SweepArgs &sa, Ctx &cx, const C &c, int m, int n, bool fit, hipStream_t stream, bool mask_test, bool early = false, bool early_masked = false,
                                              unsigned char *ent_masked = nullptr)
{
    Workspace &ws = cx.ws;
    const long long words = dense_row_words(n);
    const size_t bytes = (size_t)m * (size_t)words * 4;
    sa.train_bits = nullptr; sa.train_words = 0;
    if (!fit) { cx.dense.invalidate(); return; }
    unsigned *bits = (unsigned *)ws.get("train_bits", bytes);
    const bool ready = (early && early_masked == mask_test) || (c.same_train_rows && cx.dense.fits(ws, m, words, mask_test));
    if (!ready)
        launch_train_bits(stream, m, n, (int)words, c.train_p, c.train_i, (mask_test || ent_masked) ? c.test_p : nullptr, c.test_i, bits,
                          (const Plan *)ws.get("plan", sizeof(Plan)), c.only_users, ent_masked, mask_test);
    cx.dense.set(ws, words, m, mask_test, ready ? cx.dense.partial : c.only_users != nullptr, c.items_tag, c.train_p);
    sa.train_bits = bits; sa.train_words = (int)words;
}
template <class C> inline void set_train_bits(Sweep64Args &, Ctx &, const C &, int, int, bool, hipStream_t, bool, bool = false, bool = false, unsigned char * = nullptr) {}
inline void set_part_extra(SweepArgs &sa, int extra) { sa.part_extra = extra; }
inline void set_part_extra(Sweep64Args &, int) {}
inline void set_spec(SweepArgs &sa)
{
    sa.spec = (sa.check_nan || sa.noise_E || sa.ext_topk || g_sw.no_spec) ? 0 : (sa.train_bits ? 1 : 2);
}
inline void set_spec(Sweep64Args &sa) { sa.spec = (sa.check_nan || sa.noise_E || sa.ext_topk || g_sw.no_spec) ? 0 : 1; }
inline void set_ext_bits(SweepArgs &sa, const unsigned *bits, int words) { sa.train_bits = bits; sa.train_words = words; }
inline void set_ext_bits(Sweep64Args &, const unsigned *, int) {}

template <class T> inline int sample_seed_items(const Workspace &ws, int K, int n, long long n_slots, bool off, bool lists = false)
{
    if (off || g_sw.sample_seed == 0) return 0;
    int S;
    if (g_sw.sample_seed > 0) {
        S = 64;
        for (int c : {256, 1024, 2048, 4096}) if (g_sw.sample_seed >= c) S = c;
    } else {
        S = K <= 128 ? 1024 : (K <= 384 ? 2048 : 4096);
        if (lists) { if (K < 12) return 0; S = 256; }
        if ((long long)S * 6 > n || K * 2 > S) return 0;
        if (sizeof(T) == 8 && K < 16) return 0;
    }
    if (S > n || K > S) return 0;
    if ((long long)sizeof(T) * n_slots * S > free_plus_owned(ws, {"sample_scores"}) / 8) return 0;
    return S;
}
template <class T, class Args>
inline void seed_from_sample(const Args &sa, Workspace &ws, int S, int NG, int n_slots, int n_ublocks, hipStream_t stream, const void *items64 = nullptr, void *lists = nullptr)
{
    typedef Prec<T> P;
    typedef typename std::remove_pointer<decltype(Args{}.thr_shared)>::type ThrT;
    T *sample = (T *)ws.get("sample_scores", sizeof(T) * (size_t)n_slots * (size_t)S);
    Args sd = sa;
    sd.n = S; sd.tiles_total = S / TILE_ITEMS; sd.K = 1; sd.n_splits = 1; sd.tail_ublocks = 0; sd.tail_splits = 1; sd.part_splits = 1;
    sd.buffered_lists = 0; sd.ext_topk = 0; sd.lane_cap = 0; sd.lane_cnt = nullptr; sd.spec = 0; sd.dump = sample;
    if (items64) { sd.Bp = (decltype(sd.Bp))items64; sd.glists = (decltype(sd.glists))lists; set_ext_bits(sd, nullptr, 0); }
    P::set_pending(sd, 0, 0);
    P::set_sync(sd, (int)P::lds_b(NG));
    dispatch_sweep(false, true, false, 2, NG, dim3((unsigned)n_ublocks), P::lds_b(NG) + SYNC_BYTES, stream, sd);
    const dim3 grid((unsigned)cdiv(n_slots, 4)), block(256);
#define RM_SEED_LAUNCH(NV) hipLaunchKernelGGL((k_seed_from_sample<T, ThrT, NV>), grid, block, 0, stream, n_slots, sa.K, (const T *)sample, sa.slot_user, sa.slot_chunk, sa.train_p, sa.train_i, sa.thr_shared)
    switch (S) {
    case 4096: RM_SEED_LAUNCH(64); break;
    case 2048: RM_SEED_LAUNCH(32); break;
    case 1024: RM_SEED_LAUNCH(16); break;
    case 256: RM_SEED_LAUNCH(4); break;
    default: RM_SEED_LAUNCH(1); break;
    }
#undef RM_SEED_LAUNCH
    check_launch(hipGetLastError());
}

template <class T>
void throw_csr_defects(const Plan &hp, const Call<T> &c, Ctx &cx)
{
    const bool unsorted = hp.csr_desc_all[0] != hp.csr_desc_legit[0] || hp.csr_desc_all[1] != hp.csr_desc_legit[1];
    if (!hp.csr_bad && !unsorted) return;
    cx.dense.invalidate();
    if (hp.csr_bad & CSR_BAD_INDPTR)
        throw RmError{RM_ERR_INVALID, "CSR index pointers of row " + std::to_string((long long)c.user0 + hp.csr_where) + " are negative, decreasing or beyond the index array"};
    if (hp.csr_bad & CSR_BAD_INDEX)
        throw RmError{RM_ERR_INVALID, "CSR column index out of range [0, " + std::to_string(c.n) + ") in row " + std::to_string((long long)c.user0 + hp.csr_where)};
    throw RmError{RM_INTERNAL_UNSORTED, "CSR rows are not sorted"};
}
inline void launch_csr_index_checks(int m, int n, const int *train_p, const int *train_i, long long nnz_train, const int *test_p, const int *test_i, long long nnz_test,
                                    Plan *plan, hipStream_t stream)
{
    hipLaunchKernelGGL(k_check_csr_starts, dim3(cdiv(m, 1024)), dim3(1024), 0, stream, m, train_p, train_i, test_p, test_i, plan);
    auto blocks = [](long long nnz) { return dim3((unsigned)std::min<long long>((nnz / 4 + 2 + CHECK_FLAT_THREADS - 1) / CHECK_FLAT_THREADS, CHECK_FLAT_BLOCKS)); };
    if (nnz_train > 0) hipLaunchKernelGGL(k_check_csr_flat, blocks(nnz_train), dim3(CHECK_FLAT_THREADS), 0, stream, m, n, train_p, train_i, plan, 0);
    if (nnz_test > 0) hipLaunchKernelGGL(k_check_csr_flat, blocks(nnz_test), dim3(CHECK_FLAT_THREADS), 0, stream, m, n, test_p, test_i, plan, 1);
}
inline void launch_csr_checks(int m, int n, const int *train_p, const int *train_i, long long nnz_train, const int *test_p, const int *test_i, long long nnz_test,
                              Plan *plan, const unsigned char *, hipStream_t stream)
{
    hipLaunchKernelGGL(k_check_csr_ptr, dim3(cdiv(m, 256)), dim3(256), 0, stream, m, train_p, nnz_train, test_p, nnz_test, plan);
    launch_csr_index_checks(m, n, train_p, train_i, nnz_train, test_p, test_i, nnz_test, plan, stream);
}
template <class T>
void check_csr_now(const Call<T> &c, hipStream_t stream, Ctx &cx)
{
    Plan *plan = (Plan *)cx.ws.get("plan", sizeof(Plan));
    if (cx.ev_valid) HIP_CHECK(hipStreamWaitEvent(stream, cx.done, 0));
    HIP_CHECK(hipMemsetAsync(plan, 0, sizeof(Plan), stream));
    launch_csr_checks(c.m, c.n, c.train_p, c.train_i, c.nnz_train, c.test_p, c.test_i, c.nnz_test, plan, c.only_users, stream);
    Plan hp;
    HIP_CHECK(hipMemcpyAsync(&hp, plan, sizeof(Plan), hipMemcpyDeviceToHost, stream));
    HIP_CHECK(hipStreamSynchronize(stream));
    throw_csr_defects(hp, c, cx);
}

struct Beside {
    hipStream_t &st; hipEvent_t *const ev; const int n_ev; const hipStream_t call; const bool high_priority; bool enabled;
    long long handed = 0, joined = 0, at[SIDE_MARKS] = {};
    static_assert((int)POS_MARKS <= (int)SIDE_MARKS, "at[] holds the roles of either stream");
    Beside(hipStream_t &s, hipEvent_t *e, int n, hipStream_t call_, bool hp, bool on_) : st(s), ev(e), n_ev(n), call(call_), high_priority(hp), enabled(on_) {}
    ~Beside() { if (handed > joined && st) (void)hipStreamSynchronize(st); }
    hipStream_t get()
    {
        if (!st) {
            HIP_CHECK(create_stream(&st, high_priority));
            for (int i = 0; i < n_ev; i++) HIP_CHECK(hipEventCreateWithFlags(&ev[i], hipEventDisableTiming));
        }
        return st;
    }
    hipStream_t on() { if (!enabled) return call; handed++; return get(); }
    void cut(int role) { if (enabled) { get(); HIP_CHECK(hipEventRecord(ev[role], call)); } }
    hipStream_t behind(int role) { if (!enabled) return call; HIP_CHECK(hipStreamWaitEvent(st, ev[role], 0)); handed++; return st; }
    hipStream_t fork(int role) { cut(role); return behind(role); }
    void mark(int role) { if (enabled) { HIP_CHECK(hipEventRecord(ev[role], st)); at[role] = handed; } }
    void joined_at(int role) { joined = std::max(joined, at[role]); at[role] = 0; }
    void await(int role, hipStream_t into) { if (enabled) { HIP_CHECK(hipStreamWaitEvent(into, ev[role], 0)); if (into == call) joined_at(role); } }
    void join(int role) { mark(role); await(role, call); }
    bool marked(int role) const { return at[role] != 0; }
    void sync() { if (enabled && st) { HIP_CHECK(hipStreamSynchronize(st)); joined = handed; } }
};

template <class T> inline size_t sweep_lds(int NG, int K, bool want_auc, bool with_lists, int ns, int j)
{
    typedef Prec<T> P;
    const size_t head = P::lds_b(NG, 32 * ns) + (with_lists ? P::lists_b(ns, K) : 0);
    const size_t tb = ((size_t)1 << j) * P::GU * sizeof(T);
    return want_auc ? (head + tb - 1) / tb * tb + (size_t)GROUPS_PER_BLOCK * (1 << j) * P::GU * (sizeof(T) + 4) : head;
}

struct Geometry {
    int jmax, n_ublocks, nsub, tile_items, n_waves, tiles_total;
    int n_splits, tail_ublocks, tail_splits, part_splits;
    bool mask_test, use_ext_bits, list_in_lds, want_pending;
    int n_part, part_extra;
    size_t per_key, lds_total, sync_off; int pend_cap;
    int u_split, j_shallow; size_t lds_l;
};
template <class T>
Geometry sweep_geometry(const Call<T> &c, const Plan &hp, int NG, bool want_auc, bool want_lane, bool ext_topk, bool check_nan, bool dense_ok,
                        const Switches &sw)
{
    typedef Prec<T> P;
    const int n = c.n, K = c.K;
    Geometry g{};
    g.jmax = want_auc ? hp.jmax : 0;
    g.n_ublocks = (hp.n_groups + GROUPS_PER_BLOCK - 1) / GROUPS_PER_BLOCK;
    const int n_ublocks = g.n_ublocks;
    auto lds_need_n = [&](bool with_lists, int ns) { return sweep_lds<T>(NG, K, want_auc, with_lists, ns, g.jmax); };
    g.nsub = 2;
    if (!ext_topk && !want_lane && P::max_nsub >= 3 && NG <= 8 && lds_need_n(true, 3) + SYNC_BYTES <= LDS_LIMIT && !sw.hbm_lists && !sw.nsub2)
        g.nsub = 3;
    const int nsub = g.nsub;
    g.tile_items = 32 * nsub; g.n_waves = 4 * nsub;
    g.tiles_total = (n + g.tile_items - 1) / g.tile_items;
    const int tiles_total = g.tiles_total;
    int n_splits = 1, tail_ublocks = 0, tail_splits = 0;
    if (n_ublocks > 0) {
        const int n_cu = 256;
        const int max_splits = std::max(1, std::min(MAX_PARTS / nsub, tiles_total / 16));
        const int max_tail = max_splits;
        const double fixed = 13.0 + 0.004 * std::max(0.25, K / 10.0) * tiles_total;
        auto block = [&](int sct) { return (double)tiles_total / sct + fixed; };
        const double slack = want_lane ? 0.2 : 0.1;
        auto last = [&](double rounds) { return std::max(std::ceil(rounds - 1e-9), rounds + slack); };
        double best = 1e300;
        for (int sct = 1; sct <= max_splits; sct++) {
            const double t1 = last((double)n_ublocks * sct / n_cu) * block(sct);
            if (t1 < best - 1e-9) { best = t1; n_splits = sct; tail_ublocks = 0; tail_splits = 0; }
            const long long full = (long long)n_ublocks * sct / n_cu;
            const int main_ub = (int)(full * n_cu / sct), tail_ub = n_ublocks - main_ub;
            if (full == 0 || tail_ub == 0) continue;
            for (int ts = sct + 1; ts <= max_tail; ts++) {
                const double t2 = (double)main_ub * sct / n_cu * block(sct) + last((double)tail_ub * ts / n_cu) * block(ts);
                if (t2 < best * 0.99) { best = t2; n_splits = sct; tail_ublocks = tail_ub; tail_splits = ts; }
            }
        }
    }
    if (!sw.splits.empty()) {
        int v[3] = {1, 0, 0};
        sscanf(sw.splits.c_str(), "%d,%d,%d", &v[0], &v[1], &v[2]);
        n_splits = std::max(1, std::min(v[0], std::max(1, MAX_PARTS / nsub)));
        tail_ublocks = std::max(0, std::min(v[1], n_ublocks)); tail_splits = std::max(1, std::min(v[2], std::max(1, MAX_PARTS / nsub)));
        if (tail_ublocks == 0) tail_splits = 0;
    }
    g.n_splits = n_splits; g.tail_ublocks = tail_ublocks; g.tail_splits = tail_splits;
    g.part_splits = std::max(n_splits, tail_splits);
    g.mask_test = std::is_same<T, float>::value && want_auc && !ext_topk && !check_nan && hp.n_slots > 0 &&
                  dense_ok && hp.n_slots == hp.n_active && hp.n_only_ndcg == 0 &&
                  nsub * g.part_splits + 1 <= MAX_PARTS && !sw.no_test_mask;
    g.use_ext_bits = c.ext_bits != nullptr && c.ext_words == dense_row_words(n) && (!c.ext_masked || g.mask_test);
    if (g.use_ext_bits) g.mask_test = c.ext_masked;
    g.n_part = nsub * g.part_splits + (g.mask_test ? 1 : 0);
    g.part_extra = g.mask_test ? 1 : 0;
    g.list_in_lds = !ext_topk && !want_lane && lds_need_n(true, nsub) + SYNC_BYTES <= LDS_LIMIT && !sw.hbm_lists;
    g.want_pending = !ext_topk && !want_lane && P::has_pending && !sw.no_pending;
    g.per_key = (size_t)g.n_waves * WAVE * P::pend_key_bytes;
    g.pend_cap = g.want_pending ? P::pend_cap_max : 0;
    g.lds_total = std::min<size_t>(LDS_LIMIT, lds_need_n(g.list_in_lds, nsub) + SYNC_BYTES + g.pend_cap * g.per_key);
    g.sync_off = g.lds_total - SYNC_BYTES;
    g.u_split = 0; g.j_shallow = -1; g.lds_l = 0;
    if (!g.list_in_lds && !want_lane && K <= 32 && want_auc && !sw.hbm_lists) {
        for (int j = g.jmax - 1; j >= 0 && g.j_shallow < 0; j--)
            if (sweep_lds<T>(NG, K, want_auc, true, nsub, j) + SYNC_BYTES <= LDS_LIMIT) g.j_shallow = j;
        if (g.j_shallow >= 0) g.u_split = hp.class_offset[g.j_shallow + 1] / (GROUPS_PER_BLOCK * P::GU);
    }
    if (g.u_split > 0)
        g.lds_l = std::min<size_t>(LDS_LIMIT, sweep_lds<T>(NG, K, want_auc, true, nsub, g.j_shallow) + SYNC_BYTES + g.pend_cap * g.per_key);
    return g;
}

template <class T>
struct Pipeline {
    typedef Prec<T> P;
    typedef typename std::remove_pointer<decltype(typename P::Args{}.thr_shared)>::type ThrT;
    static constexpr int GU = P::GU;
    const Call<T> &c; hipStream_t stream; Ctx &cx; Workspace &ws;
    const int m, n, k, K;
    const bool use_side = !g_sw.no_side;
    Beside side, pos;
    int min_items_pool = 0, min_pos_test = 0, req = 0, NG = 0; bool want_auc = false;
    int *flags = nullptr, *user_nslots = nullptr, *uslot_base = nullptr, *heavy_users = nullptr; Plan *plan = nullptr;
    int *slot_user = nullptr, *slot_chunk = nullptr, *slot_index = nullptr, *gj = nullptr, *sc_user = nullptr, *sc_chunk = nullptr;
    long long *grow = nullptr; double *log2tab = nullptr;
    ClassifyArgs ca{};
    bool want_lane = false, ext_topk = false, items_known = false, dense_ok = false;
    bool bits_early = false, bits_early_masked = false, masked_from_bits = false, flat_early = false;
    Plan hp{};
    int n_slots = 0, n_stream = 0, stream_slot0 = 0; bool check_nan = false;
    Geometry g{};
    FinalArgs<T, T> fa{};
    Entry<T> *merged = nullptr; long long *rank_sorted = nullptr;
    T *pos_score = nullptr; unsigned *hist = nullptr; int *pos_order = nullptr, *pos_item = nullptr;
    Entry<T> *pl = nullptr; PartialStat<T> *pst = nullptr;
    T *stream_scores = nullptr, *spos_score = nullptr; int *spos_item = nullptr; unsigned *shist = nullptr;
    long long stream_ld = 0;
    typename P::Args sa{};
    typename P::ListT *glists = nullptr; int *lane_cnt = nullptr; ThrT *thr_shared = nullptr;
    bool lane_lists = false;
    bool collect = false; CollectGeom collect_g{};

    Pipeline(const Call<T> &c_, hipStream_t s, Ctx &cx_)
        : c(c_), stream(s), cx(cx_), ws(cx_.ws), m(c_.m), n(c_.n), k(c_.k), K(c_.K),
          side(cx_.side_stream, cx_.side_marks.data(), SIDE_MARKS, s, cx_.high_priority, use_side),
          pos(cx_.pos_stream, cx_.pos_marks.data(), POS_MARKS, s, cx_.high_priority, use_side) {}

    void begin()
    {
        min_items_pool = std::max(std::max(c.min_items_pool, K), 2);
        min_pos_test = std::min(c.min_pos_test, 1);
        if (c.reco) { min_items_pool = 1; min_pos_test = 0; }
        for (int i = 0; i < 10; i++) if (c.out[i] && !c.reco) req |= (1 << i);
        want_auc = req & (RQ_ROC | RQ_PR);
        NG = P::supported_ng(k);
        if (NG < 0) throw RmError{RM_ERR_UNSUPPORTED, std::string(P::limit()) + " (got " + std::to_string(k) + ")"};
        if (!cx.ev_valid) {
            for (int i = 0; i < EV_COUNT; i++) HIP_CHECK(hipEventCreate(&cx.ev[i]));
            HIP_CHECK(hipEventCreateWithFlags(&cx.done, hipEventDisableTiming));
            cx.ev_valid = true;
        } else {
            HIP_CHECK(hipStreamWaitEvent(stream, cx.done, 0));
        }
        g_last_ctx = &cx;
        HIP_CHECK(hipEventRecord(cx.ev[EV_START], stream));
        RM_TRACE_POINT("run: start");
    }

    void plan_stage()
    {
        flags = (int *)ws.get("flags", sizeof(int) * (size_t)m);
        user_nslots = (int *)ws.get("user_nslots", sizeof(int) * (size_t)m);
        uslot_base = (int *)ws.get("uslot_base", sizeof(int) * (size_t)m);
        plan = (Plan *)ws.get("plan", sizeof(Plan));
        heavy_users = (int *)ws.get("heavy_users", sizeof(int) * (size_t)m);
        ca = ClassifyArgs{m, n, K, c.train_p, c.test_p, req, c.cold ? 1 : 0, min_items_pool, min_pos_test, want_auc ? 1 : 0,
                          flags, user_nslots, heavy_users, plan};
        ca.only = c.only_users; ca.reco = c.reco ? 1 : 0;
        ca.heavy_npos = K > FIN_TOPV ? FIN_TOPV : HEAVY_NPOS;
        ca.check_ptr = c.csr_checked ? 0 : 1; ca.nnz_train = c.nnz_train; ca.nnz_test = c.nnz_test;
        const long long stream_ld_max = ((long long)n + 191) / 192 * 192;
        want_lane = lane_lists_fit<T>(ws, K, c.eval_users >= 0 ? std::min<long long>(c.eval_users, m) : m, P::max_nsub >= 3 && NG <= 8);
        ext_topk = (!want_lane && K > 256) || g_sw.ext_topk;
        long long stream_cap = 0;
        if (want_auc || ext_topk) {
            stream_cap = stream_budget_bytes(ws) / (stream_ld_max * (long long)sizeof(T));
            const long long m_rows = c.eval_users >= 0 ? std::min<long long>(c.eval_users, m) : m;
            if (ext_topk) {
                if (m_rows > stream_cap) throw RmError{RM_ERR_NOMEM, "k_metrics > 256 keeps one score row (" + std::to_string(stream_ld_max * (long long)sizeof(T)) +
                                           " B) per user in device memory: " + std::to_string(m_rows) + " users do not fit, at most " + std::to_string(stream_cap) + " per call"};
                ca.force_stream = 1;
            } else if (stream_cap > 0) ca.allow_stream = 1;
        }
        const long long slot_bound = (long long)m + c.nnz_test / POS_CHUNK + 1;
        const long long group_bound = slot_bound / GU + 2;
        slot_user = (int *)ws.get("slot_user", sizeof(int) * (size_t)slot_bound);
        slot_chunk = (int *)ws.get("slot_chunk", sizeof(int) * (size_t)slot_bound);
        slot_index = (int *)ws.get("slot_index", sizeof(int) * (size_t)slot_bound);
        unsigned char *slot_j = (unsigned char *)ws.get("slot_j", (size_t)slot_bound);
        gj = (int *)ws.get("gj", sizeof(int) * (size_t)group_bound);
        grow = (long long *)ws.get("grow", sizeof(long long) * (size_t)group_bound);
        sc_user = (int *)ws.get("sc_user", sizeof(int) * (size_t)slot_bound);
        sc_chunk = (int *)ws.get("sc_chunk", sizeof(int) * (size_t)slot_bound);
        int *tile_total = nullptr, *tile_offset = nullptr;
        const int n_tiles = (int)cdiv(m, 1024);
        if (m > 8192) {
            tile_total = (int *)ws.get("scan_tile_total", sizeof(int) * (size_t)n_tiles);
            tile_offset = (int *)ws.get("scan_tile_offset", sizeof(int) * (size_t)n_tiles);
        }
        items_known = cx.packed.of_call(c.items_tag);
        if (!c.reco) log2tab = (double *)ws.get("log2tab", sizeof(double) * (size_t)K);
        if (!c.reco && !cx.discounts.holds(ws, K)) {
            std::vector<double> lt((size_t)K);
            for (int i = 0; i < K; i++) lt[i] = std::log2(i + 2);
            HIP_CHECK(hipMemcpy(log2tab, lt.data(), sizeof(double) * (size_t)K, hipMemcpyHostToDevice));
            cx.discounts.set(ws, K);
        }
        if (!cx.pinned_plan) HIP_CHECK(hipHostMalloc((void **)&cx.pinned_plan, sizeof(Plan), hipHostMallocDefault));
        dense_ok = std::is_same<T, float>::value && (c.ext_bits ? true : c.dense_fit >= 0 ? c.dense_fit != 0 : dense_rows_fit(ws, m, n));
        flat_early = want_auc && !c.only_users && c.nnz_test > 0 && !g_sw.no_pos_flat;
        int *ent_user = nullptr; unsigned char *ent_masked = nullptr;
        PosArgs<T> pf{};
        if (flat_early) {
            ent_user = (int *)ws.get("ent_user", sizeof(int) * (size_t)c.nnz_test);
            ent_masked = (unsigned char *)ws.get("ent_masked", (size_t)c.nnz_test);
            pf.m = m; pf.n = n; pf.k = k; pf.A = c.A; pf.lda = c.lda; pf.B = c.B; pf.ldb = c.ldb;
            pf.train_p = c.train_p; pf.train_i = c.train_i; pf.test_p = c.test_p; pf.test_i = c.test_i; pf.flags = flags;
            pf.pos_tmp = (T *)ws.get("pos_tmp", sizeof(T) * (size_t)c.nnz_test);
            if (sizeof(T) == 4) pf.pos_key = (unsigned long long *)ws.get("pos_key", 8 * ((size_t)c.nnz_test + 8));
            pf.noise_row = c.noise_row; pf.noise_row0 = c.noise_row0; pf.noise_E = c.noise_E; pf.noise_ld = c.noise_ld;
            pf.noise_flag = c.noise_flag; pf.plan = plan;
        }
        for (int attempt = 0; ; attempt++) {
            if (attempt == 0) HIP_CHECK(hipMemsetAsync(plan, 0, sizeof(Plan), stream));
            else {
                const size_t at = offsetof(Plan, n_noise_flagged);
                HIP_CHECK(hipMemsetAsync(plan, 0, at, stream));
                HIP_CHECK(hipMemsetAsync((char *)plan + at + sizeof(int), 0, sizeof(Plan) - at - sizeof(int), stream));
            }
            hipLaunchKernelGGL(k_classify, dim3(cdiv(m, 1024)), dim3(1024), 0, stream, ca);
            side.cut(SIDE_PLAN_FORK); pos.cut(POS_PLAN_FORK);
            if (tile_total) {
                hipLaunchKernelGGL(k_scan_tiles, dim3(n_tiles), dim3(1024), 0, stream, user_nslots, uslot_base, m, tile_total);
                hipLaunchKernelGGL(k_scan_exclusive, dim3(1), dim3(1024), 0, stream, tile_total, tile_offset, n_tiles, &plan->n_slots, plan, GU);
            } else {
                hipLaunchKernelGGL(k_scan_exclusive, dim3(1), dim3(1024), 0, stream, user_nslots, uslot_base, m, &plan->n_slots, plan, GU);
            }
            AssignArgs aa{m, c.test_p, flags, user_nslots, uslot_base, want_auc ? 1 : 0, plan, slot_user, slot_chunk, slot_index, slot_j, sc_user, sc_chunk,
                          ext_topk ? 1 : 0, tile_offset};
            hipLaunchKernelGGL(k_assign_slots, dim3(cdiv(m, ASSIGN_THREADS)), dim3(ASSIGN_THREADS), 0, stream, aa);
            hipLaunchKernelGGL(k_block_tables, dim3(1), dim3(1024), 0, stream, plan, slot_j, gj, grow, GU);
            const hipStream_t aux = side.behind(SIDE_PLAN_FORK), aux2 = pos.behind(POS_PLAN_FORK);
            if (!c.csr_checked) launch_csr_index_checks(m, n, c.train_p, c.train_i, c.nnz_train, c.test_p, c.test_i, c.nnz_test, plan, aux);
            side.mark(SIDE_CHECKS_DONE);
            hipLaunchKernelGGL(k_absmax<T>, dim3(512), dim3(256), 0, aux2, c.A, c.lda, (long long)m, k, &plan->amax_a, &plan->nonfinite);
            if (!items_known) hipLaunchKernelGGL(k_absmax<T>, dim3(1024), dim3(256), 0, aux2, c.B, c.ldb, (long long)n, k, &plan->amax_b, &plan->nonfinite_b);
            pos.mark(POS_MAXIMA_DONE);
            if (attempt == 0 && flat_early) hipLaunchKernelGGL(k_entry_users, dim3(cdiv(cdiv(m, WAVE) * WAVE, 256)), dim3(256), 0, pos.on(), m, c.test_p, ent_user, plan);
            if (attempt == 0 && std::is_same<T, float>::value && use_side && !c.ext_bits && dense_ok) {
                SweepArgs probe{};
                const bool guess = want_auc && !ext_topk && !g_sw.no_test_mask;
                (void)ws.get("train_bits", (size_t)m * (size_t)dense_row_words(n) * 4);
                if (!(c.same_train_rows && cx.dense.fits(ws, m, dense_row_words(n), guess))) {
                    set_train_bits(probe, cx, c, m, n, dense_ok, side.on(), guess, false, false, flat_early ? ent_masked : nullptr);
                    side.mark(SIDE_ROWS_AND_PACKS); side.mark(SIDE_ROWS_FOR_POS);
                    bits_early = true; bits_early_masked = guess; masked_from_bits = flat_early;
                }
            }
            side.await(SIDE_CHECKS_DONE, stream); pos.await(POS_MAXIMA_DONE, stream);
            HIP_CHECK(hipMemcpyAsync(cx.pinned_plan, plan, sizeof(Plan), hipMemcpyDeviceToHost, stream));
            if (attempt == 0 && flat_early) {
                const hipStream_t sc = pos.fork(POS_SCORES_AFTER_COPY);
                hipLaunchKernelGGL(k_pos_scores_flat<T>, dim3(cdiv(c.nnz_test, POSF_WAVES * WAVE)), dim3(POSF_WAVES * WAVE), 0, sc, pf, ent_user);
                if (masked_from_bits) side.await(SIDE_ROWS_FOR_POS, sc);
                else hipLaunchKernelGGL(k_test_masked, dim3(cdiv(m, TM_USERS)), dim3(256), 0, sc, m, c.test_p, c.test_i, c.train_p, c.train_i, ent_user, ent_masked, plan);
                hipLaunchKernelGGL(k_pos_apply_masked<T>, dim3(cdiv(c.nnz_test, 256)), dim3(256), 0, sc, pf, ent_masked);
                pos.mark(POS_SCORES_DONE);
            }
            RM_TRACE_POINT("run: plan chain + side kernels enqueued");
            HIP_CHECK(hipStreamSynchronize(stream));
            RM_TRACE_POINT("run: plan read back");
            hp = *cx.pinned_plan;
            throw_csr_defects(hp, c, cx);
            if (ca.allow_stream && !ca.force_stream && hp.class_count[STREAM_CLASS] > stream_cap && attempt == 0) {
                ca.allow_stream = 0; ca.check_ptr = 0;
                side.sync(); pos.sync();
                continue;
            }
            break;
        }
        throw_csr_defects(hp, c, cx);
        n_slots = hp.n_slots;
        n_stream = (want_auc || ext_topk) ? hp.class_count[STREAM_CLASS] : 0;
        stream_slot0 = n_stream > 0 ? hp.class_offset[STREAM_CLASS] : n_slots;
        if (items_known) { hp.amax_b = cx.packed.amax_b; hp.nonfinite_b = cx.packed.nonfinite_b; }
        else { cx.packed.amax_b = hp.amax_b; cx.packed.nonfinite_b = hp.nonfinite_b; }
        double amax_a, amax_b;
        std::memcpy(&amax_a, &hp.amax_a, 8); std::memcpy(&amax_b, &hp.amax_b, 8);
        const double tmax = std::is_same<T, float>::value ? 3.0e38 : 1.0e308;
        check_nan = hp.nonfinite || hp.nonfinite_b || !((double)k * amax_a * 1.001 < tmax / std::max(amax_b, 1e-300));
    }

    void launch_top_values()
    {
        if (!(fa.ndcg && hp.n_heavy > 0)) return;
        fa.heavy_ld = std::max(1, std::min(K, hp.max_npos));
        fa.heavy_topv = (T *)ws.get("heavy_topv", sizeof(T) * (size_t)m * (size_t)fa.heavy_ld);
        fa.heavy_nan = (unsigned char *)ws.get("heavy_nan", (size_t)m);
        fa.heavy_users = heavy_users; fa.n_heavy = hp.n_heavy;
        hipLaunchKernelGGL((k_top_values<T, T>), dim3(cdiv((long long)hp.n_heavy * WAVE, 256)), dim3(256), 0, side.fork(SIDE_FORK), fa);
        side.mark(SIDE_TOP_VALUES);
    }

    void prep()
    {
        if (!c.reco || want_lane || ext_topk) merged = (Entry<T> *)ws.get("merged", sizeof(Entry<T>) * (size_t)m * K);
        if (c.pos_rank) rank_sorted = (long long *)ws.get("rank_sorted", sizeof(long long) * (size_t)std::max<long long>(c.nnz_test, 1));
        if (rank_sorted) HIP_CHECK(hipMemsetAsync(rank_sorted, 0, sizeof(long long) * (size_t)std::max<long long>(c.nnz_test, 1), stream));
        fa.m = m; fa.n = n; fa.K = K; fa.req = req; fa.cumulative = c.cumulative ? 1 : 0; fa.noise = c.noise ? 1 : 0; fa.gu = GU;
        fa.train_p = c.train_p; fa.test_p = c.test_p; fa.test_i = c.test_i; fa.test_v = c.test_v;
        fa.flags = flags; fa.user_nslots = user_nslots; fa.uslot_base = uslot_base; fa.slot_index = slot_index;
        fa.gj = gj; fa.grow = grow; fa.log2tab = log2tab;
        fa.p = c.out[0]; fa.tp = c.out[1]; fa.r = c.out[2]; fa.ap = c.out[3]; fa.tap = c.out[4];
        fa.ndcg = c.out[5]; fa.hit = c.out[6]; fa.rr = c.out[7]; fa.roc = c.out[8]; fa.pr = c.out[9];
        fa.merged = merged; fa.rank_sorted = rank_sorted; fa.status = c.status;
        fa.noise_flag = c.noise_flag; fa.plan = plan;
        fa.n_slots = n_slots; fa.slot_user = slot_user; fa.slot_chunk = slot_chunk;
        fa.stream_slot0 = stream_slot0;
        if (want_auc && n_slots > 0) fa.auc_part = (AucPart *)ws.get("auc_part", sizeof(AucPart) * (size_t)n_slots);
        fa.heavy_npos = ca.heavy_npos;
        stream_ld = (long long)g.tiles_total * g.tile_items;
        if (n_slots == 0) return;
        const int n_groups = hp.n_groups, tiles_total = g.tiles_total, tile_items = g.tile_items;

        const long long bp_units = P::items_units(tiles_total, NG, tile_items), ap_units = P::users_units(n_groups, NG);
        typename P::PackT *Bp = (typename P::PackT *)ws.get("Bp", 16 * (size_t)bp_units);
        typename P::PackT *Ap = (typename P::PackT *)ws.get("Ap", 16 * (size_t)ap_units);
        const bool items_packed = cx.packed.holds(ws, c.items_tag, tile_items, NG);
        const bool packs_side = use_side && want_auc && cx.side_stream != nullptr;
        pack_operands(c.A, c.lda, c.B, c.ldb, n, k, NG, tile_items, slot_user, n_slots, Ap, ap_units, Bp, bp_units, packs_side ? side.on() : stream, !items_packed);
        if (packs_side) side.mark(SIDE_ROWS_AND_PACKS);
        cx.packed.set(ws, c.items_tag, tile_items, NG);
        launch_top_values();

        if (bits_early && (bits_early_masked != g.mask_test || (g.use_ext_bits && dense_ok))) side.await(SIDE_ROWS_AND_PACKS, stream);
        if (g.use_ext_bits && dense_ok) set_ext_bits(sa, c.ext_bits, (int)c.ext_words);
        else set_train_bits(sa, cx, c, m, n, dense_ok, stream, g.mask_test, bits_early, bits_early_masked);

        if (want_auc) positives();

        if (n_stream > 0) stream_scores = (T *)ws.get("stream_scores", sizeof(T) * (size_t)n_stream * (size_t)stream_ld);
        if (!ext_topk) pl = (Entry<T> *)ws.get("pl", sizeof(Entry<T>) * (size_t)n_slots * g.n_part * K);
        pst = (PartialStat<T> *)ws.get("pst", sizeof(PartialStat<T>) * (size_t)n_slots * g.n_part);
        const unsigned n_blocks = (unsigned)((g.n_ublocks - g.tail_ublocks) * g.n_splits + g.tail_ublocks * g.tail_splits);
        lane_lists = want_lane && !ext_topk;
        int lane_cap = lane_lists ? P::lane_cap(K) : 0;
        if (lane_lists && g_sw.lane_cap_set > 0) lane_cap = (int)std::min<long long>(std::max<long long>(P::lane_cap(K), (g_sw.lane_cap_set + 15) / 16 * 16), (COLLECT_MAX_ENTRIES - K) / 16 * 16);
        if (lane_lists && g_sw.lane_cap_min >= 0)
            lane_cap = std::min(lane_cap, (K + lane_sel_slack(K) + 16 + 1 + 15) / 16 * 16);
        if (lane_lists) {
            glists = (typename P::ListT *)ws.get("glists", (size_t)n_blocks * g.n_waves * WAVE * (size_t)lane_cap * (sizeof(T) + 4));
            lane_cnt = (int *)ws.get("lane_cnt", sizeof(int) * (size_t)n_blocks * g.n_waves * WAVE);
        } else if (!g.list_in_lds && !ext_topk) {
            glists = (typename P::ListT *)ws.get("glists", sizeof(typename P::ListT) * (size_t)n_blocks * g.n_waves * GU * (2 * K + 32));
        }

        thr_shared = (ThrT *)ws.get("thr_shared", sizeof(ThrT) * (size_t)n_slots);
        if (want_auc && !ext_topk && !g_sw.no_seed)
            hipLaunchKernelGGL((k_seed_thresholds<T, ThrT>), dim3(cdiv(n_slots, 256)), dim3(256), 0, stream, n_slots, stream_slot0, K, GU, slot_user, slot_chunk,
                               user_nslots, flags, c.test_p, grow, pos_score, spos_score, thr_shared);
        else HIP_CHECK(hipMemsetAsync(thr_shared, 0, sizeof(ThrT) * (size_t)n_slots, stream));
        sa.thr_shared = thr_shared;
        sa.n = n; sa.K = K; sa.ngt = NG; sa.n_slots = n_slots; sa.n_groups = n_groups; sa.n_ublocks = g.n_ublocks;
        sa.n_splits = g.n_splits; sa.tail_ublocks = g.tail_ublocks; sa.tail_splits = g.tail_splits; sa.part_splits = g.part_splits; sa.tiles_total = tiles_total; sa.jmax = g.jmax; sa.check_nan = check_nan ? 1 : 0; sa.buffered_lists = (want_lane || ext_topk) ? 1 : 0; sa.ext_topk = ext_topk ? 1 : 0;
        sa.Ap = (decltype(sa.Ap))Ap; sa.Bp = (decltype(sa.Bp))Bp; sa.slot_user = slot_user; sa.slot_chunk = slot_chunk;
        sa.train_p = c.train_p; sa.train_i = c.train_i; sa.gj = gj; sa.grow = grow;
        sa.pos_score = pos_score; sa.pos_item = pos_item; sa.hist = hist; sa.glists = glists; sa.lane_cap = lane_cap; sa.lane_cnt = lane_cnt; sa.pl = pl; sa.pst = pst; sa.dump = nullptr;
        P::set_pending(sa, g.pend_cap, 0);
        P::set_sync(sa, (int)g.sync_off);
        sa.stream_slot0 = stream_slot0; sa.stream_ld = stream_ld; sa.stream_scores = stream_scores;
        set_part_extra(sa, g.part_extra);
        sa.noise_row = c.noise_row; sa.noise_row0 = c.noise_row0; sa.noise_E = c.noise_E; sa.noise_ld = c.noise_ld;
        set_spec(sa);

        if (side.marked(SIDE_ROWS_AND_PACKS)) side.await(SIDE_ROWS_AND_PACKS, stream);
        const bool sample_lists = !lane_lists && !ext_topk && sizeof(T) == 4;
        const int sample_S = (lane_lists || sample_lists) ? sample_seed_items<T>(ws, K, n, n_slots, check_nan || c.noise_E != nullptr, sample_lists) : 0;
        if (sample_S > 0 && !sample_lists) seed_from_sample<T>(sa, ws, sample_S, NG, n_slots, g.n_ublocks, stream);
        else if (sample_S > 0) {
            const long long units = P::items_units(sample_S / TILE_ITEMS, NG);
            typename P::PackT *Bs = (typename P::PackT *)ws.get("sample_items", 16 * (size_t)units);
            void *Ls = ws.get("sample_lists", sizeof(typename P::ListT) * (size_t)g.n_ublocks * 8 * GU * (2 + 32));
            pack_operands(c.A, c.lda, c.B, c.ldb, sample_S, k, NG, TILE_ITEMS, slot_user, 0, Ap, 0, Bs, units, stream, true);
            seed_from_sample<T>(sa, ws, sample_S, NG, n_slots, g.n_ublocks, stream, Bs, Ls);
        }
        RM_TRACE_POINT("run: preparation enqueued");
    }

    void positives()
    {
        const int n_groups = hp.n_groups;
        const long long rows = hp.total_rows + n_groups;
        pos_score = (T *)ws.get("pos_score", sizeof(T) * (size_t)(rows + 1) * GU);
        pos_item = (int *)ws.get("pos_item", sizeof(int) * (size_t)(rows + 1) * GU);
        hist = (unsigned *)ws.get("hist", sizeof(unsigned) * (size_t)(rows + 1) * GU);
        T *pos_tmp = (T *)ws.get("pos_tmp", sizeof(T) * (size_t)std::max<long long>(c.nnz_test, 1));
        pos_order = (int *)ws.get("pos_order", sizeof(int) * (size_t)std::max<long long>(c.nnz_test, 1));
        PosArgs<T> pa{m, n, k, c.A, c.lda, c.B, c.ldb, c.train_p, c.train_i, c.test_p, c.test_i,
                      flags, user_nslots, uslot_base, slot_index, grow, pos_tmp, pos_order, pos_score, pos_item, GU};
        pa.noise_row = c.noise_row; pa.noise_row0 = c.noise_row0; pa.noise_E = c.noise_E; pa.noise_ld = c.noise_ld;
        pa.noise_flag = c.noise_flag; pa.plan = plan;
        if (sizeof(T) == 4)
            pa.pos_key = (unsigned long long *)ws.get("pos_key", 8 * ((size_t)std::max<long long>(c.nnz_test, 1) + 8));
        const bool flat = flat_early;
        const bool pos_beside = use_side && n_stream > 0 && stream_slot0 > 0 && !g_sw.no_pos_beside;
        hipStream_t ps = pos_beside ? pos.on() : stream;
        PosArgs<T> pb = pa;
        const hipStream_t fill = (flat && pos_beside) ? stream : ps;
        if (n_stream > 0) {
            const size_t nz = (size_t)std::max<long long>(c.nnz_test, 1);
            spos_score = (T *)ws.get("spos_score", sizeof(T) * nz);
            spos_item = (int *)ws.get("spos_item", sizeof(int) * nz);
            shist = (unsigned *)ws.get("shist", sizeof(unsigned) * nz);
            pb.stream = 1; pb.spos_score = spos_score; pb.spos_item = spos_item;
            hipLaunchKernelGGL(k_init_tables<T>, dim3(cdiv((long long)nz, 256)), dim3(256), 0, fill, spos_score, shist, (long long)nz);
        }
        const int nsc = hp.n_stream_chunks;
        hipLaunchKernelGGL(k_init_tables<T>, dim3(cdiv(rows * GU, 256)), dim3(256), 0, stream, pos_score, hist, rows * GU);
        if (flat) {
            if (pos_beside) ps = pos.fork(POS_TABLES_INIT);
            pos.await(POS_SCORES_DONE, stream);
        } else {
            if (n_stream > 0) hipLaunchKernelGGL(k_pos_scores<T>, dim3(cdiv(nsc, POSS_WAVES)), dim3(POSS_WAVES * WAVE), 0, ps, pb, sc_user, sc_chunk, nsc);
            if (stream_slot0 > 0) hipLaunchKernelGGL(k_pos_scores<T>, dim3(cdiv(stream_slot0, POSS_WAVES)), dim3(POSS_WAVES * WAVE), 0, stream, pa, slot_user, slot_chunk, stream_slot0);
        }
        if (n_stream > 0) hipLaunchKernelGGL(k_pos_place<T>, dim3(cdiv((long long)nsc * WAVE, 256)), dim3(256), 0, ps, pb, sc_user, sc_chunk, nsc);
        if (stream_slot0 > 0) hipLaunchKernelGGL(k_pos_place<T>, dim3(cdiv((long long)stream_slot0 * WAVE, 256)), dim3(256), 0, stream, pa, slot_user, slot_chunk, stream_slot0);
        if (pos_beside) pos.join(POS_STREAMED_PLACED);
    }

    void sweep()
    {
        if (c.flag_snapshot) {
            if (n_slots > 0) {
                HIP_CHECK(hipMemcpyAsync(c.flag_snapshot, c.noise_flag, sizeof(int) * (size_t)m, hipMemcpyDeviceToDevice, stream));
                HIP_CHECK(hipMemcpyAsync(c.flag_count_host, &plan->n_noise_flagged, sizeof(int), hipMemcpyDeviceToHost, stream));
            } else {
                HIP_CHECK(hipMemsetAsync(c.flag_snapshot, 0, sizeof(int) * (size_t)m, stream));
                *c.flag_count_host = 0;
            }
            HIP_CHECK(hipEventRecord(c.flags_event, stream));
        }
        HIP_CHECK(hipEventRecord(cx.ev[EV_PREP_END], stream));
        double *tm = cx.timings;
        if (n_slots == 0) {
            HIP_CHECK(hipEventRecord(cx.ev[EV_SWEEP_END], stream));
            tm[4] = 0; tm[5] = 0; tm[6] = 0; tm[7] = 0;
            return;
        }
        const unsigned n_blocks = (unsigned)((g.n_ublocks - g.tail_ublocks) * g.n_splits + g.tail_ublocks * g.tail_splits);
        if (g.u_split > 0) {
            const int u_split = g.u_split, n_ublocks = g.n_ublocks;
            side.enabled = true;
            typename P::Args sb = sa;
            P::set_ublocks(sb, u_split, n_ublocks - u_split);
            typename P::Args sl = sa;
            P::set_ublocks(sl, 0, u_split);
            sl.tail_ublocks = std::min(g.tail_ublocks, u_split);
            sb.tail_ublocks = g.tail_ublocks - sl.tail_ublocks;
            P::set_pending(sl, g.pend_cap, 0);
            P::set_sync(sl, (int)(g.lds_l - SYNC_BYTES));
            dispatch_sweep(want_auc, false, false, g.nsub, NG, dim3((unsigned)((n_ublocks - u_split - sb.tail_ublocks) * g.n_splits + sb.tail_ublocks * g.tail_splits)), g.lds_total, side.fork(SIDE_SWEEP_FORK), sb);
            side.mark(SIDE_SWEEP_DEEP_DONE);
            dispatch_sweep(want_auc, false, true, g.nsub, NG, dim3((unsigned)((u_split - sl.tail_ublocks) * g.n_splits + sl.tail_ublocks * g.tail_splits)), g.lds_l, stream, sl);
            side.await(SIDE_SWEEP_DEEP_DONE, stream);
            side.enabled = use_side;
        } else {
            dispatch_sweep(want_auc, false, g.list_in_lds, g.nsub, NG, dim3(n_blocks), g.lds_total, stream, sa);
        }
        RM_TRACE_POINT("run: sweep enqueued");
        HIP_CHECK(hipEventRecord(cx.ev[EV_SWEEP_END], stream));
        if (lane_lists) {
            collect = true;
            collect_g = CollectGeom{sa.ublock0, sa.n_ublocks, g.n_splits, g.tail_ublocks, g.tail_splits, g.nsub, GU, P::lanes_per_user, sa.lane_cap, g.part_extra ? g.n_part - 1 : -1};
        }
        tm[4] = g.u_split > 0 ? 2 : 1; tm[5] = g.n_splits; tm[6] = n_blocks; tm[7] = (double)g.lds_total;
        cx.timed_slots = n_slots;
        cx.total_slots = n_slots;
    }

    int stream_parts() const { return (int)cdiv(n, STREAM_RANK_THREADS * STREAM_RANK_ITEMS); }
    void rank_streamed_rows(int r0, int r1, hipStream_t st)
    {
        if (r1 <= r0) return;
        const int parts = stream_parts();
        const int ipt = ((int)cdiv(n, (long long)parts * STREAM_RANK_THREADS) + 7) / 8 * 8;
        hipLaunchKernelGGL((k_rank_streamed<T, T>), dim3((unsigned)((long long)(r1 - r0) * parts)), dim3(STREAM_RANK_THREADS), 0, st, fa, parts, ipt, r0);
    }
    void auc_streamed_rows(int r0, int r1, hipStream_t st)
    {
        if (r1 <= r0) return;
        hipLaunchKernelGGL((k_auc_streamed<T, T>), dim3(cdiv((long long)(r1 - r0) * WAVE, 256)), dim3(256), 0, st, fa, r0, r1);
    }
    void finalize_slots(int s0, int s1, size_t fin_lds)
    {
        if (s1 <= s0) return;
        fa.fin_slot0 = s0; fa.fin_slot1 = s1;
        hipLaunchKernelGGL((k_finalize<T, T>), dim3(cdiv(s1 - s0, FIN_THREADS)), dim3(FIN_THREADS), fin_lds, stream, fa);
    }

    void collect_lists()
    {
        if (!collect) return;
        fa.collected = 1;
        const char *gl = (const char *)glists;
        if (collect_capw(K, collect_g.lane_cap) == 512)
            hipLaunchKernelGGL((k_collect_topk<T, T, ThrT, 512>), dim3(collect_grid(cdiv(n_slots, 4))), dim3(256), 0, stream, fa, collect_g, gl, lane_cnt, (const ThrT *)thr_shared);
        else if (collect_capw(K, collect_g.lane_cap) == 1024)
            hipLaunchKernelGGL((k_collect_topk<T, T, ThrT, 1024>), dim3(collect_grid(cdiv(n_slots, 4))), dim3(256), 0, stream, fa, collect_g, gl, lane_cnt, (const ThrT *)thr_shared);
        else
            hipLaunchKernelGGL((k_collect_topk<T, T, ThrT, 4096>), dim3(collect_grid(n_slots)), dim3(64), 0, stream, fa, collect_g, gl, lane_cnt, (const ThrT *)thr_shared);
    }
    void select_lists()
    {
        if (!(n_slots > 0 && ext_topk)) return;
        int sel_ld = 2;
        while (sel_ld < K) sel_ld <<= 1;
        fa.ext_topk = 1; fa.sel_ld = sel_ld;
        fa.sel_hi = (unsigned long long *)ws.get("sel_hi", sizeof(unsigned long long) * (size_t)n_slots * sel_ld);
        fa.sel_lo = (unsigned *)ws.get("sel_lo", sizeof(unsigned) * (size_t)n_slots * sel_ld);
        hipLaunchKernelGGL((k_select_topk<T, T>), dim3(n_slots), dim3(SELECT_THREADS), 0, stream, fa);
    }

    void finalize_reco()
    {
        fa.n_part = g.n_part; fa.pl = pl; fa.pst = pst;
        fa.stream_slot0 = stream_slot0; fa.stream_scores = stream_scores; fa.stream_ld = stream_ld;
        collect_lists();
        select_lists();
        const bool merged_ready = n_slots > 0 && (collect || ext_topk);
        RecoArgs<T> ra{m, n, K, g.n_part, flags, uslot_base, slot_index, c.train_p, pl, pst, merged_ready ? merged : nullptr,
                       c.topk_idx, c.topk_score, c.status};
        const size_t lds = reco_lds_bytes<T>(g.n_part, merged_ready);
        if (lds > 48 * 1024) HIP_CHECK(hipFuncSetAttribute((const void *)k_finalize_reco<T>, hipFuncAttributeMaxDynamicSharedMemorySize, (int)lds));
        hipLaunchKernelGGL(k_finalize_reco<T>, dim3(cdiv(m, RECO_THREADS)), dim3(RECO_THREADS), lds, stream, ra);
        HIP_CHECK(hipGetLastError());
    }

    void finalize()
    {
        fa.n_part = g.n_part; fa.pl = pl; fa.pst = pst; fa.hist = hist; fa.pos_score = pos_score; fa.pos_item_tab = pos_item;
        fa.stream_slot0 = stream_slot0; fa.stream_scores = stream_scores; fa.stream_ld = stream_ld;
        fa.spos_score = spos_score; fa.spos_item = spos_item; fa.shist = shist;
        fa.rank_generic = (g_sw.rank_generic ? 1 : 0);
        const bool ranks_beside = use_side && n_slots > 0 && want_auc && n_stream > 0;
        bool auc_launch = true;
        if (stream_parts() == 1 && !g_sw.no_fused_auc) {
            fa.fused_auc = 1 | (g.mask_test ? 2 : 0);
            long long top = 1;
            while (top <= hp.max_npos) top <<= 1;
            auc_launch = ext_topk || !(top * (long long)(sizeof(T) / 4) + hp.max_npos + 1 <= STREAM_RANK_LDS / 4);
        }
        hipStream_t rank_stream = stream;
        if (ranks_beside) { rank_stream = side.fork(SIDE_FORK); rank_streamed_rows(0, n_stream, rank_stream); }
        if (g.mask_test) {
            if (n_slots > stream_slot0)
                hipLaunchKernelGGL((k_merge_positives<T, T>), dim3(cdiv(n_slots - stream_slot0, MERGE_WAVES)), dim3(MERGE_WAVES * WAVE), 0, stream, fa, g.n_part - 1, stream_slot0);
            if (ranks_beside && auc_launch) rank_stream = side.fork(SIDE_MERGED);
        }
        if (ranks_beside && auc_launch) auc_streamed_rows(0, n_stream, rank_stream);
        hipLaunchKernelGGL((k_finalize_skipped<T, T>), dim3(cdiv(m, 256)), dim3(256), 0, stream, fa);
        if (side.marked(SIDE_TOP_VALUES)) side.await(SIDE_TOP_VALUES, stream);
        collect_lists();
        select_lists();
        if (n_slots > 0) {
            if (want_auc) {
                if (n_stream > 0 && !ranks_beside) { rank_streamed_rows(0, n_stream, stream); if (auc_launch) auc_streamed_rows(0, n_stream, stream); }
                if (stream_slot0 > 0) hipLaunchKernelGGL((k_auc_slots<T, T>), dim3(cdiv(stream_slot0, 256)), dim3(256), 0, stream, fa);
            }
            const size_t fin_lds = finalize_lds_bytes<T>(K, g.n_part);
            HIP_CHECK(hipFuncSetAttribute((const void *)k_finalize<T, T>, hipFuncAttributeMaxDynamicSharedMemorySize, (int)fin_lds));
            fa.auc_defer_slot0 = n_slots;
            if (ranks_beside && (req & (RQ_ROC | RQ_PR)) && !g_sw.no_defer_auc) {
                fa.auc_defer_slot0 = stream_slot0;
                finalize_slots(0, n_slots, fin_lds);
                side.join(SIDE_JOIN);
                hipLaunchKernelGGL((k_finalize_auc<T, T>), dim3(cdiv(n_slots - stream_slot0, 256)), dim3(256), 0, stream, fa);
            } else if (ranks_beside) {
                finalize_slots(0, stream_slot0, fin_lds);
                side.join(SIDE_JOIN);
                finalize_slots(stream_slot0, n_slots, fin_lds);
            } else finalize_slots(0, n_slots, fin_lds);
        }
        HIP_CHECK(hipGetLastError());
    }

    void export_ranks()
    {
        if (c.topk_idx && !c.reco)
            hipLaunchKernelGGL(k_export_rank<T>, dim3(cdiv((long long)m * K, 256)), dim3(256), 0, stream, m, K, merged, c.topk_idx, c.topk_score, flags);
        if (c.pos_rank)
            hipLaunchKernelGGL(k_export_pos_rank, dim3(cdiv(m, 128)), dim3(128), 0, stream, c.nnz_test, m, c.test_p, flags, pos_order, rank_sorted, c.pos_rank,
                               (want_auc && n_slots > 0) ? 1 : 0, c.status);
        RM_TRACE_POINT("run: finalisation enqueued");
        HIP_CHECK(hipEventRecord(cx.ev[EV_END], stream));
        HIP_CHECK(hipEventRecord(cx.done, stream));
        cx.ev_recorded = true;
        HIP_CHECK(hipGetLastError());
    }
};

template <class T>
void run(const Call<T> &c, hipStream_t stream, Ctx &cx)
{
    Pipeline<T> p(c, stream, cx);
    p.begin();
    p.plan_stage();
    p.g = sweep_geometry<T>(c, p.hp, p.NG, p.want_auc, p.want_lane, p.ext_topk, p.check_nan, p.dense_ok, g_sw);
    p.prep();
    p.sweep();
    if (c.reco) p.finalize_reco(); else p.finalize();
    p.export_ranks();
}

std::atomic<unsigned long long> g_call_counter{1};

template <class T> struct NoiseGeom {
    int per; long long e_ld, d_ld, cap;
    NoiseGeom(const Workspace &ws, int n)
    {
        per = sizeof(T) == 4 ? 1 : 2;
        e_ld = ((long long)n + 191) / 192 * 192;
        d_ld = ((long long)n * per + MT_N - 1) / MT_N * MT_N;
        const long long row_bytes = e_ld * (long long)sizeof(T) + d_ld * 4;
        long long budget;
        if (g_sw.noise_budget_mb >= 0) budget = g_sw.noise_budget_mb << 20;
        else budget = free_plus_owned(ws, {"noise_draws", "noise_rows"}) / 3;
        cap = std::max<long long>(1, std::min<long long>(budget / row_bytes, 1 << 20));
    }
};
template <class T>
void noise_make_rows(Ctx &cx, const Call<T> &c0, const NoiseGeom<T> &g, const int *row_user, int rows, const int *train_p, long long user0,
                     unsigned *D, T *E, hipStream_t stream, const unsigned *own_bits = nullptr, long long own_words = 0)
{
    const int n = c0.n, m = c0.m;
    hipLaunchKernelGGL(k_mt_draws, dim3(cdiv(rows, MT_WAVES)), dim3(MT_WAVES * WAVE), 0, stream, row_user, rows, c0.seed, user0,
                       train_p, n, g.per, D, g.d_ld);
    const bool dense = row_user != nullptr && cx.dense.built_by(cx.ws, c0.items_tag, train_p, m);
    if (own_bits)
        hipLaunchKernelGGL(k_noise_rows_bits<T>, dim3(rows), dim3(NOISE_ROWS_THREADS), sizeof(int) * (size_t)(2 * own_words + 1), stream, row_user, rows,
                           own_bits, (int)own_words, n, 0, train_p, c0.train_i, c0.test_p, c0.test_i, D, g.d_ld, E, g.e_ld);
    else if (dense)
        hipLaunchKernelGGL(k_noise_rows_bits<T>, dim3(rows), dim3(NOISE_ROWS_THREADS), sizeof(int) * (size_t)(2 * cx.dense.words + 1), stream, row_user, rows,
                           cx.dense.rows(cx.ws), (int)cx.dense.words, n, cx.dense.masked ? 1 : 0, train_p, c0.train_i, c0.test_p, c0.test_i,
                           D, g.d_ld, E, g.e_ld);
    else
        hipLaunchKernelGGL(k_noise_rows<T>, dim3(cdiv((long long)rows * g.e_ld, 256)), dim3(256), 0, stream, row_user, rows, train_p, c0.train_i, n,
                           D, g.d_ld, E, g.e_ld);
}

template <class T>
int noise_exact_pass(const Call<T> &c0, const int *flag, const int *skip, int n_known, hipStream_t stream, Ctx &cx, const int **row_user_out = nullptr)
{
    Workspace &ws = cx.ws;
    const int m = c0.m;
    const NoiseGeom<T> g(ws, c0.n);
    int *noise_row = (int *)ws.get("noise_row", sizeof(int) * (size_t)m);
    int *row_user = (int *)ws.get("noise_row_user", sizeof(int) * (size_t)(n_known >= 0 ? std::max(n_known, 1) : m));
    int *counter = (int *)ws.get("noise_counter", sizeof(int));
    unsigned char *only = (unsigned char *)ws.get("noise_only", (size_t)m);
    HIP_CHECK(hipMemsetAsync(counter, 0, sizeof(int), stream));
    hipLaunchKernelGGL(k_noise_assign_rows, dim3(cdiv(m, 256)), dim3(256), 0, stream, m, flag, skip, noise_row, row_user, counter);
    int n_flagged = n_known;
    if (n_known < 0) {
        HIP_CHECK(hipMemcpyAsync(&cx.noise_words->sequential, counter, sizeof(int), hipMemcpyDeviceToHost, stream));
        HIP_CHECK(hipStreamSynchronize(stream));
        n_flagged = cx.noise_words->sequential;
    }
    if (row_user_out) *row_user_out = row_user;
    for (long long r0 = 0; r0 < n_flagged; r0 += g.cap) {
        const int rows = (int)std::min<long long>(g.cap, n_flagged - r0);
        hipLaunchKernelGGL(k_noise_select, dim3(cdiv(m, 256)), dim3(256), 0, stream, m, noise_row, (int)r0, (int)r0 + rows, only);
        unsigned *D = (unsigned *)ws.get("noise_draws", sizeof(unsigned) * (size_t)rows * (size_t)g.d_ld);
        T *E = (T *)ws.get("noise_rows", sizeof(T) * (size_t)rows * (size_t)g.e_ld);
        noise_make_rows<T>(cx, c0, g, row_user + r0, rows, c0.train_p, c0.user0, D, E, stream);
        Call<T> c = c0;
        set_exact_pass<T>(c, only, noise_row, (int)r0, E, g.e_ld, rows);
        run<T>(c, stream, cx);
    }
    return n_flagged;
}

template <class T> struct NoiseBeside {
    Ctx &cx;
    Ctx *pc = nullptr; hipStream_t ps = nullptr;
    std::unique_lock<std::mutex> lock;
    int *noise_row = nullptr, *row_user = nullptr; unsigned char *only = nullptr;
    explicit NoiseBeside(Ctx &c) : cx(c) {}
    void open(hipEvent_t other = nullptr)
    {
        pc = &peer_context(cx, NOISE_SLOT);
        lock = std::unique_lock<std::mutex>(pc->mu);
        if (!pc->own_stream) HIP_CHECK(create_stream(&pc->own_stream, pc->high_priority));
        ps = pc->own_stream;
        HIP_CHECK(hipStreamWaitEvent(ps, cx.flags_ev, 0));
        if (other) HIP_CHECK(hipStreamWaitEvent(ps, other, 0));
    }
    int assign(int m, const int *flags, int known, int *word)
    {
        Workspace &pw = pc->ws;
        noise_row = (int *)pw.get("noise_row", sizeof(int) * (size_t)m);
        row_user = (int *)pw.get("noise_row_user", sizeof(int) * (size_t)(known > 0 ? known : m));
        int *counter = (int *)pw.get("noise_counter", sizeof(int));
        only = (unsigned char *)pw.get("noise_only", (size_t)m);
        HIP_CHECK(hipMemsetAsync(counter, 0, sizeof(int), ps));
        hipLaunchKernelGGL(k_noise_assign_rows, dim3(cdiv(m, 256)), dim3(256), 0, ps, m, flags, (const int *)nullptr, noise_row, row_user, counter);
        if (known > 0) return known;
        HIP_CHECK(hipMemcpyAsync(word, counter, sizeof(int), hipMemcpyDeviceToHost, ps));
        HIP_CHECK(hipStreamSynchronize(ps));
        return *word;
    }
    void rows(Call<T> &c, const NoiseGeom<T> &g, int rows_n, bool own_rows)
    {
        Workspace &pw = pc->ws;
        const int m = c.m, n = c.n;
        hipLaunchKernelGGL(k_noise_select, dim3(cdiv(m, 256)), dim3(256), 0, ps, m, noise_row, 0, rows_n, only);
        unsigned *D = (unsigned *)pw.get("noise_draws", sizeof(unsigned) * (size_t)rows_n * (size_t)g.d_ld);
        T *E = (T *)pw.get("noise_rows", sizeof(T) * (size_t)rows_n * (size_t)g.e_ld);
        const long long words = dense_row_words(n);
        unsigned *bits = nullptr;
        if (own_rows) {
            const bool fit = std::is_same<T, float>::value && dense_rows_fit(pw, m, n);
            if (fit) {
                bits = (unsigned *)pw.get("train_bits", (size_t)m * (size_t)words * 4);
                pc->dense.invalidate();
                launch_train_bits(ps, m, n, (int)words, c.train_p, c.train_i, (const int *)nullptr, c.test_i, bits, (const Plan *)nullptr, only);
                c.ext_bits = bits; c.ext_words = words; c.ext_masked = false;
            }
            c.dense_fit = fit ? 1 : 0;
        } else if (cx.dense.built_by(cx.ws, c.items_tag, c.train_p, m)) {
            c.ext_bits = cx.dense.rows(cx.ws); c.ext_words = cx.dense.words; c.ext_masked = cx.dense.masked;
        }
        noise_make_rows<T>(own_rows ? *pc : cx, c, g, row_user, rows_n, c.train_p, c.user0, D, E, ps, bits, words);
        set_exact_pass<T>(c, only, noise_row, 0, E, g.e_ld, rows_n);
    }
    void run_pass(const Call<T> &c)
    {
        try { run<T>(c, ps, *pc); }
        catch (...) {
            sync();
            if (pc->side_stream) (void)hipStreamSynchronize(pc->side_stream);
            g_last_ctx = &cx;
            throw;
        }
        g_last_ctx = &cx;
    }
    void sync() { if (pc) (void)hipStreamSynchronize(ps); }
};

template <class T>
void run_call(const Call<T> &c_in, hipStream_t stream, Ctx &cx, std::function<bool()> *defer = nullptr)
{
    if (defer) *defer = nullptr;
    if (!c_in.noise) { run<T>(c_in, stream, cx); return; }
    Call<T> c0 = c_in;
    if (c0.items_tag == 0) c0.items_tag = g_call_counter.fetch_add(1);
    Workspace &ws = cx.ws;
    const int m = c0.m;
    cx.need_noise_words();
    if (sizeof(T) == 4 && c0.first_pass_flags) {
        Call<T> c1 = c0;
        c1.noise_flag = c0.first_pass_flags;
        run<T>(c1, stream, cx);
        return;
    }
    if (sizeof(T) == 4 && c0.dense_fit < 0) c0.dense_fit = dense_rows_fit(ws, m, c0.n) ? 1 : 0;
    const NoiseGeom<T> g(ws, c0.n);
    const MetricLayout lay(c0.out, c0.cumulative ? (size_t)c0.K : 1);
    if (sizeof(T) == 8) {
        if (!c0.csr_checked) { check_csr_now<T>(c0, stream, cx); c0.csr_checked = true; }
        for (long long b0 = 0; b0 < m; b0 += g.cap) {
            const int mb = (int)std::min<long long>(g.cap, m - b0);
            Call<T> c = c0;
            c.A = c0.A + (size_t)b0 * c0.lda; c.m = mb; c.train_p = c0.train_p + b0; c.test_p = c0.test_p + b0; c.user0 = c0.user0 + b0;
            for (int i = 0; i < 10; i++) if (c0.out[i]) c.out[i] = c0.out[i] + (size_t)b0 * lay.width(i);
            if (c0.topk_idx) { c.topk_idx = c0.topk_idx + (size_t)b0 * c0.K; c.topk_score = c0.topk_score + (size_t)b0 * c0.K; c.status = c0.status + b0; }
            if (c0.only_users) c.only_users = c0.only_users + b0;
            unsigned *D = (unsigned *)ws.get("noise_draws", sizeof(unsigned) * (size_t)mb * (size_t)g.d_ld);
            T *E = (T *)ws.get("noise_rows", sizeof(T) * (size_t)mb * (size_t)g.e_ld);
            noise_make_rows<T>(cx, c0, g, nullptr, mb, c.train_p, c.user0, D, E, stream);
            c.noise_E = E; c.noise_ld = g.e_ld; c.noise_row = nullptr; c.noise_row0 = 0;
            run<T>(c, stream, cx);
        }
        return;
    }
    int *flag = (int *)ws.get("noise_flag", sizeof(int) * (size_t)m);
    HIP_CHECK(hipMemsetAsync(flag, 0, sizeof(int) * (size_t)m, stream));
    Call<T> c1 = c0;
    c1.noise_flag = flag;
    const bool beside = !c0.topk_idx && !c0.only_users && !g_sw.noise_sequential;
    int *snap = nullptr;
    if (beside) {
        snap = (int *)ws.get("noise_flag_snap", sizeof(int) * (size_t)m);
        cx.noise_words->first_early = 0;
        c1.flag_snapshot = snap; c1.flag_count_host = &cx.noise_words->first_early; c1.flags_event = cx.flags_ev;
    }
    Plan *plan = (Plan *)ws.get("plan", sizeof(Plan));
    int n_beside = 0;
    NoiseBeside<T> nb(cx);
    run<T>(c1, stream, cx);
    if (beside) {
        HIP_CHECK(hipEventSynchronize(cx.flags_ev));
        const int n_early = cx.noise_words->first_early;
        if (n_early > 0 && n_early <= g.cap) {
            nb.open();
            nb.assign(m, snap, n_early, nullptr);
            Call<T> c = c0;
            nb.rows(c, g, n_early, false);
            static const char *tnames[10] = {"t_p", "t_tp", "t_r", "t_ap", "t_tap", "t_ndcg", "t_hit", "t_rr", "t_roc", "t_pr"};
            ScatterArgs<T> sc{};
            for (int i = 0; i < 10; i++) {
                sc.width[i] = (int)lay.width(i);
                sc.dst[i] = c0.out[i];
                c.out[i] = c0.out[i] ? (T *)nb.pc->ws.get(tnames[i], sizeof(T) * (size_t)m * lay.width(i)) : nullptr;
                sc.src[i] = c.out[i];
            }
            nb.run_pass(c);
            HIP_CHECK(hipEventRecord(cx.pass_ev, nb.ps));
            HIP_CHECK(hipStreamWaitEvent(stream, cx.pass_ev, 0));
            hipLaunchKernelGGL(k_noise_scatter<T>, dim3(cdiv(m, 256)), dim3(256), 0, stream, m, snap, sc);
            HIP_CHECK(hipEventRecord(cx.done, stream));
            n_beside = n_early;
        }
    }
    int *n_flagged_host = &cx.noise_words->first_final;
    HIP_CHECK(hipMemcpyAsync(n_flagged_host, &plan->n_noise_flagged, sizeof(int), hipMemcpyDeviceToHost, stream));
    auto tail = [=, &cx]() -> bool {
        HIP_CHECK(hipStreamSynchronize(stream));
        cx.timings[4] = 0;
        const int n_flagged = *n_flagged_host - n_beside;
        if (n_flagged <= 0) return false;
        Call<T> c = c0;
        c.same_train_rows = true;
        noise_exact_pass<T>(c, flag, n_beside > 0 ? (const int *)snap : (const int *)nullptr, n_flagged, stream, cx);
        return true;
    };
    if (defer) *defer = tail;
    else tail();
}

template <class F> int guarded(F &&f)
{
    g_err.clear();
    try { f(); return RM_OK; }
    catch (const RmError &e) { g_err = e.msg; return e.code; }
    catch (const std::bad_alloc &) { g_err = "host allocation failed"; return RM_ERR_NOMEM; }
    catch (const std::exception &e) { g_err = e.what(); return RM_ERR_HIP; }
}

volatile std::sig_atomic_t g_interrupt = 0, g_interrupt_by_signal = 0;
std::atomic<bool> g_handler_locked{false};
extern "C" void rm_on_sigint(int) { g_interrupt = 1; g_interrupt_by_signal = 1; }
struct SignalGuard {
    void (*old_handler)(int) = nullptr;
    bool active = false;
    SignalGuard()
    {
        bool expected = false;
        if (g_handler_locked.compare_exchange_strong(expected, true)) {
            g_interrupt = 0; g_interrupt_by_signal = 0;
            old_handler = std::signal(SIGINT, rm_on_sigint);
            active = true;
        }
    }
    void restore()
    {
        if (active) { std::signal(SIGINT, old_handler); active = false; g_handler_locked.store(false); }
    }
    ~SignalGuard() { const bool mine = active; restore(); if (mine) { g_interrupt = 0; g_interrupt_by_signal = 0; } }
    void check()
    {
        if (!g_interrupt) return;
        const bool by_signal = g_interrupt_by_signal != 0;
        const bool mine = active;
        restore();
        if (mine) { g_interrupt = 0; g_interrupt_by_signal = 0; }
        if (by_signal && mine) std::raise(SIGINT);
        throw RmError{RM_ERR_INTERRUPTED, "Error: procedure was interrupted.\n"};
    }
};

std::mutex g_dev_mu;
std::vector<int> g_devices;

template <class T> struct HostCall {
    const T *A; size_t lda; const T *B; size_t ldb; int m, n, k;
    const int *trp, *tri, *tep, *tei; const T *tev;
    int K; bool cumulative, noise; T *outs[10]; bool cold; int mip, mpt;
    int *topk_idx; T *topk_score; long long *pos_rank; int *status;
    unsigned long long seed;
    int nthreads = 0;
    bool reco = false;
};

struct SharedItems {
    std::mutex mu; std::condition_variable cv;
    bool ready = false, failed = false;
    const void *src = nullptr; int src_device = 0;
    int copies_pending = 0;
    void copy_done() { std::lock_guard<std::mutex> lk(mu); copies_pending--; cv.notify_all(); }
};

inline void enable_peer_access(int dst_device, int src_device)
{
    static std::mutex mu;
    static std::map<std::pair<int, int>, bool> done;
    if (dst_device == src_device) return;
    std::lock_guard<std::mutex> lk(mu);
    bool &d = done[std::make_pair(dst_device, src_device)];
    if (d) return;
    d = true;
// ... 779 lines not shown
```

recometrics_amd/csrc/rm_prep.hpp:

```cpp
#pragma once
#include "rm_device.hpp"

namespace rm {

struct ClassifyArgs {
    int m, n, K;
    const int *train_p, *test_p;
    int req;
    int cold, min_items_pool, min_pos_test;
    int want_auc;
    int *flags;
    int *user_nslots;
    int *heavy_users;
    Plan *plan;
    const unsigned char *only;
    int force_stream;
    int allow_stream;
    int check_ptr;
    int heavy_npos;
    long long nnz_train, nnz_test;
    int reco;
};

__device__ __forceinline__ int chunk_depth(int pc)
{
    return 32 - __clz(pc);
}

__global__ void k_check_csr_ptr(int m, const int *train_p, long long nnz_train, const int *test_p, long long nnz_test, Plan *plan)
{
    const int u = blockIdx.x * blockDim.x + threadIdx.x;
    if (u >= m) return;
    const int a0 = train_p[u], a1 = train_p[u + 1], b0 = test_p[u], b1 = test_p[u + 1];
    if (a0 < 0 || a1 < a0 || (long long)a1 > nnz_train || b0 < 0 || b1 < b0 || (long long)b1 > nnz_test) { atomicOr(&plan->csr_bad, CSR_BAD_INDPTR); plan->csr_where = u; }
}
constexpr int CHECK_FLAT_THREADS = 256, CHECK_FLAT_BLOCKS = 1024;
__global__ __launch_bounds__(CHECK_FLAT_THREADS) void k_check_csr_flat(int m, int n, const int *indptr, const int *idx, Plan *plan, int which)
{
    if (plan->csr_bad & CSR_BAD_INDPTR) return;
    const long long e0 = indptr[0], e1 = indptr[m];
    const bool aligned = (((size_t)idx) & 15) == 0;
    unsigned desc = 0; bool bad = false; long long bad_at = 0;
    for (long long g = (e0 >> 2) + (long long)blockIdx.x * blockDim.x + threadIdx.x; (g << 2) < e1; g += (long long)gridDim.x * blockDim.x) {
        const long long e = g << 2;
        if (e >= e0 && e + 4 < e1 && aligned) {
            const int4 q = *(const int4 *)(idx + e);
            const int x4 = idx[e + 4];
            const int x[5] = {q.x, q.y, q.z, q.w, x4};
            #pragma unroll
            for (int i = 0; i < 4; i++) { if ((unsigned)x[i] >= (unsigned)n) { bad = true; bad_at = e + i; } desc += x[i] > x[i + 1]; }
        } else {
            for (int i = 0; i < 4; i++) {
                const long long f = e + i;
                if (f < e0 || f >= e1) continue;
                const int v = idx[f];
                if ((unsigned)v >= (unsigned)n) { bad = true; bad_at = f; }
                if (f + 1 < e1) desc += v > idx[f + 1];
            }
        }
    }
    if (bad) {
        int lo = 0, hi = m;
        while (lo < hi) { const int mid = (lo + hi + 1) >> 1; if ((long long)indptr[mid] <= bad_at) lo = mid; else hi = mid - 1; }
        atomicOr(&plan->csr_bad, CSR_BAD_INDEX); plan->csr_where = lo;
    }
    #pragma unroll
    for (int d = 32; d >= 1; d >>= 1) desc += __shfl_xor(desc, d);
    __shared__ unsigned blk;
    if (threadIdx.x == 0) blk = 0;
    __syncthreads();
    if ((threadIdx.x & 63) == 0 && desc) atomicAdd(&blk, desc);
    __syncthreads();
    if (threadIdx.x == 0 && blk) atomicAdd(&plan->csr_desc_all[which], (unsigned long long)blk);
}
__global__ __launch_bounds__(1024) void k_check_csr_starts(int m, const int *train_p, const int *train_i, const int *test_p, const int *test_i, Plan *plan)
{
    if (plan->csr_bad & CSR_BAD_INDPTR) return;
    __shared__ unsigned blk[2];
    if (threadIdx.x < 2) blk[threadIdx.x] = 0;
    __syncthreads();
    const int u = blockIdx.x * blockDim.x + threadIdx.x;
    unsigned d0 = 0, d1 = 0;
    if (u >= 1 && u < m) {
        const int s = train_p[u], e1 = train_p[m], e0 = train_p[0];
        if (train_p[u - 1] < s && s > e0 && s < e1) d0 = train_i[s - 1] > train_i[s];
        if (test_p) {
            const int t = test_p[u], f1 = test_p[m], f0 = test_p[0];
            if (test_p[u - 1] < t && t > f0 && t < f1) d1 = test_i[t - 1] > test_i[t];
        }
    }
    const unsigned long long b0 = __ballot(d0), b1 = __ballot(d1);
    if ((threadIdx.x & 63) == 0) {
        if (b0) atomicAdd(&blk[0], (unsigned)__popcll(b0));
        if (b1) atomicAdd(&blk[1], (unsigned)__popcll(b1));
    }
    __syncthreads();
    if (threadIdx.x < 2 && blk[threadIdx.x]) atomicAdd(&plan->csr_desc_legit[threadIdx.x], (unsigned long long)blk[threadIdx.x]);
}

__global__ void k_classify(ClassifyArgs a)
{
    const int u = blockIdx.x * blockDim.x + threadIdx.x;
    const bool skip = u < a.m && a.only && !a.only[u];
    bool live = u < a.m && !skip;
    if (skip) { a.flags[u] = UF_SKIP; a.user_nslots[u] = 0; }
    int ntr = 0, npos = 0;
    if (live) {
        const int a0 = a.train_p[u], a1 = a.train_p[u + 1], b0 = a.reco ? 0 : a.test_p[u], b1 = a.reco ? 0 : a.test_p[u + 1];
        if (a.check_ptr && (a0 < 0 || a1 < a0 || (long long)a1 > a.nnz_train || b0 < 0 || b1 < b0 || (long long)b1 > a.nnz_test)) {
            atomicOr(&a.plan->csr_bad, CSR_BAD_INDPTR); a.plan->csr_where = u;
        } else { ntr = a1 - a0; npos = b1 - b0; }
    }
    const int cand = a.n - ntr;
    bool isnan_user = !live || npos <= 0 || (ntr + npos >= a.n && !(a.req & RQ_NDCG)) || cand < a.min_items_pool ||
                      (!a.cold && ntr == 0) || npos < a.min_pos_test;
    if (a.reco) isnan_user = !live || cand < 1;
    const bool only_ndcg = !a.reco && (ntr + npos) >= a.n;
    const bool kleqn = cand <= a.K;
    if (!a.reco && !isnan_user && kleqn && !(a.req & (RQ_ROC | RQ_PR | RQ_AP | RQ_TAP | RQ_RR))) isnan_user = true;
    int f = 0, nsl = 0, myclass = -1, nfull = 0;
    if (isnan_user) f = UF_NAN;
    else {
        f = UF_ACTIVE | (only_ndcg ? UF_ONLY_NDCG : 0) | (kleqn ? UF_KLEQN : 0);
        if (a.force_stream || (a.want_auc && !only_ndcg && npos > POS_CHUNK && a.allow_stream)) {
            nsl = 1;
            myclass = STREAM_CLASS;
        } else if (a.want_auc && !only_ndcg) {
            nfull = npos / POS_CHUNK;
            const int rem = npos % POS_CHUNK;
            nsl = nfull + (rem ? 1 : 0);
            myclass = rem ? chunk_depth(rem) : -1;
        } else {
            nsl = 1;
            myclass = 0;
        }
    }
    __shared__ int blk_count[N_CLASSES + 3];
    __shared__ int blk_heavy[2];
    if (threadIdx.x < N_CLASSES + 3) blk_count[threadIdx.x] = 0;
    if (threadIdx.x < 2) blk_heavy[threadIdx.x] = 0;
    __syncthreads();
    const int lane = threadIdx.x & 63;
    const unsigned long long act = __ballot(!isnan_user);
    if (act && lane == __ffsll((long long)act) - 1) atomicAdd(&blk_count[N_CLASSES], __popcll(act));
    for (int j = 0; j < N_CLASSES; j++) {
        const unsigned long long mk = __ballot(myclass == j);
        if (mk && lane == __ffsll((long long)mk) - 1) atomicAdd(&blk_count[j], __popcll(mk));
    }
    if (nfull) atomicAdd(&blk_count[MAX_J], nfull);
    const bool lng = live && npos > POS_CHUNK;
    const unsigned long long lm = __ballot(lng);
    if (lm) {
        int mx = lng ? npos : 0;
        #pragma unroll
        for (int d = 32; d >= 1; d >>= 1) { const int o = __shfl_xor(mx, d); mx = o > mx ? o : mx; }
        if (lane == __ffsll((long long)lm) - 1) { atomicAdd(&blk_count[N_CLASSES + 1], __popcll(lm)); atomicMax(&blk_count[N_CLASSES + 2], mx); }
    }
    if (live) { a.flags[u] = f; a.user_nslots[u] = nsl; }
    const bool heavy = live && !isnan_user && npos > a.heavy_npos;
    const int heavy_at = heavy ? atomicAdd(&blk_heavy[0], 1) : 0;
    if (live && !isnan_user && only_ndcg) atomicAdd(&a.plan->n_only_ndcg, 1);
    __syncthreads();
    if (threadIdx.x == 0 && blk_heavy[0]) blk_heavy[1] = atomicAdd(&a.plan->n_heavy, blk_heavy[0]);
    __syncthreads();
    if (heavy) a.heavy_users[blk_heavy[1] + heavy_at] = u;
    if (threadIdx.x < N_CLASSES && blk_count[threadIdx.x]) atomicAdd(&a.plan->class_count[threadIdx.x], blk_count[threadIdx.x]);
    if (threadIdx.x == N_CLASSES && blk_count[N_CLASSES]) atomicAdd(&a.plan->n_active, blk_count[N_CLASSES]);
    if (threadIdx.x == N_CLASSES + 1 && blk_count[N_CLASSES + 1]) { atomicAdd(&a.plan->n_long, blk_count[N_CLASSES + 1]); atomicMax(&a.plan->max_npos, blk_count[N_CLASSES + 2]); }
}

__global__ __launch_bounds__(1024) void k_scan_tiles(const int *in, int *out, int count, int *tile_total)
{
    __shared__ int wsum[16];
    const int tid = threadIdx.x, lane = tid & 63, wave = __builtin_amdgcn_readfirstlane(tid >> 6);
    const int i = blockIdx.x * 1024 + tid;
    const int v = i < count ? in[i] : 0;
    int x = v;
    #pragma unroll
    for (int d = 1; d < 64; d <<= 1) { const int y = __shfl_up(x, d); if (lane >= d) x += y; }
    if (lane == 63) wsum[wave] = x;
    __syncthreads();
    int woff = 0;
    for (int w = 0; w < wave; w++) woff += wsum[w];
    if (i < count) out[i] = woff + x - v;
    if (tid == 1023) tile_total[blockIdx.x] = woff + x;
}
__device__ inline void plan_classes(Plan *p, int gu, int n_slots)
{
    int off = 0, jmax = 0;
    for (int j = 0; j < N_CLASSES; j++) {
        p->class_offset[j] = off;
        off += p->class_count[j];
        if (p->class_count[j] && j <= MAX_J) jmax = j;
        p->class_cursor[j] = 0;
    }
    p->class_offset[N_CLASSES] = off;
    p->n_groups = (n_slots + gu - 1) / gu;
    p->jmax = jmax;
}

__global__ void k_scan_exclusive(const int *in, int *out, int count, int *total_out, Plan *classes, int gu)
{
    __shared__ int wsum[16];
    __shared__ int carry_s;
    const int tid = threadIdx.x, lane = tid & 63, wave = __builtin_amdgcn_readfirstlane(tid >> 6);
    if (tid == 0) carry_s = 0;
    __syncthreads();
    for (int base = 0; base < count; base += 1024) {
        const int i = base + tid;
        const int v = i < count ? in[i] : 0;
        int x = v;
        #pragma unroll
        for (int d = 1; d < 64; d <<= 1) { const int y = __shfl_up(x, d); if (lane >= d) x += y; }
        if (lane == 63) wsum[wave] = x;
        __syncthreads();
        int woff = 0;
        for (int w = 0; w < wave; w++) woff += wsum[w];
        const int carry = carry_s;
        if (i < count) out[i] = carry + woff + x - v;
        __syncthreads();
        if (tid == 1023) carry_s = carry + woff + x;
        __syncthreads();
    }
    if (tid == 0 && total_out) *total_out = carry_s;
    if (tid == 0 && classes) plan_classes(classes, gu, carry_s);
}

struct AssignArgs {
    int m;
    const int *test_p, *flags, *user_nslots, *uslot_base;
    int want_auc;
    Plan *plan;
    int *slot_user, *slot_chunk, *slot_index;
    unsigned char *slot_j;
    int *sc_user, *sc_chunk;
    int force_stream;
    const int *tile_offset;
};

constexpr int ASSIGN_THREADS = 1024;
__global__ __launch_bounds__(ASSIGN_THREADS) void k_assign_slots(AssignArgs a)
{
    __shared__ int blk_count[N_CLASSES], blk_base[N_CLASSES], blk_chunks, blk_chunk_base;
    if (a.plan->csr_bad & CSR_BAD_INDPTR) return;
    const int u = blockIdx.x * blockDim.x + threadIdx.x;
    const int lane = threadIdx.x & 63;
    if (threadIdx.x < N_CLASSES) blk_count[threadIdx.x] = 0;
    if (threadIdx.x == N_CLASSES) blk_chunks = 0;
    __syncthreads();
    const int nsl = u < a.m ? a.user_nslots[u] : 0;
    const int npos = (nsl && a.test_p) ? a.test_p[u + 1] - a.test_p[u] : 0;
    int ubase = 0;
    if (u < a.m) {
        ubase = a.uslot_base[u] + (a.tile_offset ? a.tile_offset[u >> 10] : 0);
        if (a.tile_offset) ((int *)a.uslot_base)[u] = ubase;
    }
    const bool auc_user = nsl && a.want_auc && !(a.flags[u] & UF_ONLY_NDCG);
    int jlast = -1, in_blk = 0;
    const bool streamed = nsl && (a.force_stream || (auc_user && nsl == 1 && npos > POS_CHUNK));
    if (nsl) jlast = streamed ? STREAM_CLASS : auc_user ? chunk_depth(min(POS_CHUNK, npos - (nsl - 1) * POS_CHUNK)) : 0;
    for (int j = 0; j < N_CLASSES; j++) {
        const unsigned long long mk = __ballot(jlast == j);
        if (!mk) continue;
        const int leader = __ffsll((long long)mk) - 1;
        int base = 0;
        if (lane == leader) base = atomicAdd(&blk_count[j], __popcll(mk));
        base = __shfl(base, leader);
        if (jlast == j) in_blk = base + __popcll(mk & ((1ull << lane) - 1));
    }
    int full_at = 0;
    if (nsl > 1) full_at = atomicAdd(&blk_count[MAX_J], nsl - 1);
    const int nch = (streamed && auc_user) ? (npos + POS_CHUNK - 1) / POS_CHUNK : 0;
    int ch_at = 0;
    if (nch) ch_at = atomicAdd(&blk_chunks, nch);
    __syncthreads();
    if (threadIdx.x < N_CLASSES && blk_count[threadIdx.x]) blk_base[threadIdx.x] = atomicAdd(&a.plan->class_cursor[threadIdx.x], blk_count[threadIdx.x]);
    if (threadIdx.x == N_CLASSES && blk_chunks) blk_chunk_base = atomicAdd(&a.plan->n_stream_chunks, blk_chunks);
    __syncthreads();
    if (nch) {
        const int at = blk_chunk_base + ch_at;
        for (int c = 0; c < nch; c++) { a.sc_user[at + c] = u; a.sc_chunk[at + c] = c; }
    }
    if (nsl) {
        const int pos = a.plan->class_offset[jlast] + blk_base[jlast] + in_blk;
        a.slot_user[pos] = u;
        a.slot_chunk[pos] = nsl - 1;
        a.slot_j[pos] = (unsigned char)jlast;
        a.slot_index[ubase + nsl - 1] = pos;
    }
    for (int c = 0; c < nsl - 1; c++) {
        const int pos = a.plan->class_offset[MAX_J] + blk_base[MAX_J] + full_at + c;
        a.slot_user[pos] = u;
        a.slot_chunk[pos] = c;
        a.slot_j[pos] = (unsigned char)MAX_J;
        a.slot_index[ubase + c] = pos;
    }
}

__global__ __launch_bounds__(1024) void k_block_tables(Plan *p, const unsigned char *slot_j, int *gj, long long *grow, int gu)
{
    __shared__ int wsum[16];
    __shared__ long long carry_s;
    if (p->csr_bad & CSR_BAD_INDPTR) return;
    const int tid = threadIdx.x, lane = tid & 63, wave = __builtin_amdgcn_readfirstlane(tid >> 6);
    const int ng = p->n_groups, ns = p->n_slots;
    const int nb = (ng + GROUPS_PER_BLOCK - 1) / GROUPS_PER_BLOCK;
    if (tid == 0) carry_s = 0;
    __syncthreads();
    for (int base = 0; base < nb; base += 1024) {
        const int b = base + tid;
        int jb = 0, ngb = 0;
        if (b < nb) {
            const int glast = min(ng, (b + 1) * GROUPS_PER_BLOCK) - 1;
            const int slast = min(ns, (glast + 1) * gu) - 1;
            jb = slot_j[slast];
            if (jb == STREAM_CLASS) {
                const int first_stream = p->class_offset[STREAM_CLASS];
                jb = first_stream > b * GROUPS_PER_BLOCK * gu ? slot_j[first_stream - 1] : 0;
            }
            ngb = glast - b * GROUPS_PER_BLOCK + 1;
        }
        const int per_group = (1 << jb) - 1;
        const int v = ngb * per_group;
        int x = v;
        #pragma unroll
        for (int d = 1; d < 64; d <<= 1) { const int y = __shfl_up(x, d); if (lane >= d) x += y; }
        if (lane == 63) wsum[wave] = x;
        __syncthreads();
        int woff = 0;
        for (int w = 0; w < wave; w++) woff += wsum[w];
        const long long carry = carry_s;
        const long long mine = carry + woff + x - v;
        for (int q = 0; q < ngb; q++) {
            const int g = b * GROUPS_PER_BLOCK + q;
            gj[g] = jb;
            grow[g] = mine + (long long)q * per_group;
        }
        __syncthreads();
        if (tid == 1023) carry_s = carry + woff + x;
        __syncthreads();
    }
    if (tid == 0) p->total_rows = carry_s;
}

template <class T>
__global__ void k_absmax(const T *X, size_t ld, long long rows, int k, unsigned long long *amax_bits, int *nonfinite)
{
    double mx = 0.; bool bad = false;
    const long long total = rows * k;
    auto take = [&](T xv) {
        const double x = (double)xv;
        const double ax = x < 0 ? -x : x;
        bad |= !(ax <= 1.7976931348623157e308);
        mx = ax > mx ? ax : mx;
    };
    if (ld == (size_t)k && (((size_t)X) & 15) == 0) {
        constexpr int V = 16 / (int)sizeof(T);
        typedef T VecT __attribute__((ext_vector_type(16 / sizeof(T))));
        const long long nv = total / V;
        const long long stride = (long long)gridDim.x * blockDim.x;
        for (long long i = (long long)blockIdx.x * blockDim.x + threadIdx.x; i < nv; i += 4 * stride) {
            VecT q[4];
            #pragma unroll
            for (int u = 0; u < 4; u++) { const long long j = i + u * stride; q[u] = ((const VecT *)X)[j < nv ? j : i]; }
            #pragma unroll
            for (int u = 0; u < 4; u++)
                #pragma unroll
                for (int e = 0; e < V; e++) take(q[u][e]);
        }
        for (long long i = nv * V + (long long)blockIdx.x * blockDim.x + threadIdx.x; i < total; i += (long long)gridDim.x * blockDim.x) take(X[i]);
    } else {
        for (long long i = (long long)blockIdx.x * blockDim.x + threadIdx.x; i < total; i += (long long)gridDim.x * blockDim.x)
            take(X[(size_t)(i / k) * ld + (i % k)]);
    }
    #pragma unroll
    for (int d = 32; d >= 1; d >>= 1) { const double o = __shfl_xor(mx, d); mx = o > mx ? o : mx; }
    __shared__ unsigned long long blk_max;
    __shared__ int blk_bad;
    if (threadIdx.x == 0) { blk_max = 0ull; blk_bad = 0; }
    __syncthreads();
    const bool anybad = __any(bad);
    if ((threadIdx.x & 63) == 0) {
        if (!anybad) atomicMax(&blk_max, (unsigned long long)__double_as_longlong(mx));
        else atomicOr(&blk_bad, 1);
    }
    __syncthreads();
    if (threadIdx.x == 0) {
        if (blk_bad) atomicOr(nonfinite, 1);
        else if (blk_max) atomicMax(amax_bits, blk_max);
    }
}

template <class T, class KeyT>
__device__ __forceinline__ KeyT seed_of_slot(int slot, int stream_slot0, int K, int gu, const int *slot_user, const int *slot_chunk, const int *user_nslots,
                                             const int *flags, const int *test_p, const long long *grow, const T *pos_score, const T *spos_score)
{
    const int u = slot_user[slot];
    if (slot_chunk[slot] != 0 || user_nslots[u] != 1 || (flags[u] & UF_ONLY_NDCG)) return (KeyT)0;
    const int te0 = test_p[u], P = test_p[u + 1] - te0;
    if (P < K) return (KeyT)0;
// ... 668 lines not shown
```

Before: 17.64 million.

## Fuse top-K walk into merge, move NDCG top-values to side kernel, add duplicate detection

The finalize merge now keeps up to eight partition heads in registers and feeds each merged entry directly into the metric walk, which removes the separate pass that re-read the merged list. The per-user NDCG ideal top-value insertion sort moves out of k_finalize into a new side-stream kernel, k_top_values_rows, so finalize needs less LDS. Users with a single slot compute AUC inline from the histogram table, and the k_auc_slots launch is skipped when every active user has exactly one slot. CSR validation now also counts equal neighbouring test items so that duplicates can gate the test-masking path. In exchange the code is more complex, there is an extra kernel launch, and the binary search is skipped for non-extra partitions, which relies on masking being correct.

```diff
diff --git a/recometrics_amd/csrc/rm_device.hpp b/recometrics_amd/csrc/rm_device.hpp
--- a/recometrics_amd/csrc/rm_device.hpp
+++ b/recometrics_amd/csrc/rm_device.hpp
@@ -54,7 +54,8 @@
     int csr_where;
     alignas(128) unsigned long long csr_desc_all[2];
     unsigned long long csr_desc_legit[2];
-    unsigned long long csr_pad[12];
+    unsigned long long csr_eq_all, csr_eq_legit;
+    unsigned long long csr_pad[10];
 };
 enum : int { CSR_BAD_INDPTR = 1, CSR_BAD_INDEX = 2, CSR_UNSORTED_TRAIN = 4, CSR_UNSORTED_TEST = 8 };
 
diff --git a/recometrics_amd/csrc/rm_finalize.hpp b/recometrics_amd/csrc/rm_finalize.hpp
--- a/recometrics_amd/csrc/rm_finalize.hpp
+++ b/recometrics_amd/csrc/rm_finalize.hpp
@@ -7,12 +7,15 @@
 constexpr int MAX_PARTS = 128;
 constexpr int FIN_THREADS = 128;
 constexpr int FIN_TOPV = 64;
-template <class T> inline size_t finalize_lds_bytes(int K, int n_part) { return (sizeof(T) * (size_t)(K < FIN_TOPV ? K : FIN_TOPV) + 4 * (size_t)n_part) * FIN_THREADS; }
+constexpr int FIN_HEADS = 8;
+inline size_t finalize_lds_bytes(int n_part) { return 4 * (size_t)n_part * FIN_THREADS; }
+template <class T> inline size_t top_values_lds_bytes(int K) { return sizeof(T) * (size_t)(K < FIN_TOPV ? K : FIN_TOPV) * FIN_THREADS; }
 
 struct AucPart { unsigned long long sum_ranks; double s1, s2; int nvalid, pad; };
 
 template <class T, class S> struct FinalArgs {
     int m, n, K, n_part, req, cumulative, noise, gu, n_slots;
+    int part_extra;
     const int *slot_user, *slot_chunk;
     const int *train_p, *test_p, *test_i; const T *test_v;
     const int *flags, *user_nslots, *uslot_base, *slot_index;
@@ -72,6 +75,7 @@
     if (slot >= a.stream_slot0) return;
     const int u = a.slot_user[slot], c = a.slot_chunk[slot];
     if (a.flags[u] & UF_ONLY_NDCG) return;
+    if (a.user_nslots[u] == 1) return;
     const int te0 = a.test_p[u], npos = a.test_p[u + 1] - te0;
     const int GUr = a.gu;
     const int g = slot / GUr, ul = slot % GUr;
@@ -798,6 +802,44 @@
 }
 
 template <class T, class S>
+__global__ __launch_bounds__(FIN_THREADS) void k_top_values_rows(FinalArgs<T, S> a)
+{
+    extern __shared__ __attribute__((aligned(16))) char topv_smem[];
+    T *topv = (T *)topv_smem + threadIdx.x;
+    const int u = blockIdx.x * blockDim.x + threadIdx.x;
+    if (u >= a.m || !(a.flags[u] & UF_ACTIVE)) return;
+    const int te0 = a.test_p[u], npos = a.test_p[u + 1] - te0;
+    if (npos > a.heavy_npos) return;
+    const int L = a.K < npos ? a.K : npos;
+    if (L > a.heavy_ld || L > FIN_TOPV) return;
+    const T *tv = a.test_v + te0;
+    bool has_nan_val = false;
+    int cnt = 0;
+    T kth = 0;
+    for (int t0 = 0; t0 < npos; t0 += 8) {
+        T xb[8];
+        #pragma unroll
+        for (int q = 0; q < 8; q++) xb[q] = t0 + q < npos ? tv[t0 + q] : (T)0;
+        #pragma unroll
+        for (int q = 0; q < 8; q++) {
+            if (t0 + q >= npos) break;
+            const T x = xb[q];
+            has_nan_val |= x != x;
+            if (cnt < L || x > kth) {
+                int j = cnt < L ? cnt : L - 1;
+                while (j > 0 && topv[(j - 1) * FIN_THREADS] < x) { topv[j * FIN_THREADS] = topv[(j - 1) * FIN_THREADS]; j--; }
+                topv[j * FIN_THREADS] = x;
+                cnt = cnt < L ? cnt + 1 : cnt;
+                if (cnt == L) kth = topv[(L - 1) * FIN_THREADS];
+            }
+        }
+    }
+    T *out = a.heavy_topv + (size_t)u * a.heavy_ld;
+    for (int i = 0; i < L; i++) out[i] = topv[i * FIN_THREADS];
+    a.heavy_nan[u] = has_nan_val ? 1 : 0;
+}
+
+template <class T, class S>
 __global__ void k_finalize_skipped(FinalArgs<T, S> a)
 {
     const int u = blockIdx.x * blockDim.x + threadIdx.x;
@@ -823,6 +865,47 @@
     const unsigned long long P = (unsigned long long)npos, Nneg = (unsigned long long)C - P;
     if (a.roc) a.roc[u] = (T)(1. - (double)(sum_ranks - (P * (P + 1)) / 2) / (double)(P * Nneg));
     if (a.pr) a.pr[u] = (T)(ap_full / (double)npos);
+}
+
+template <class T, class S>
+__device__ __forceinline__ void finalize_auc_table(const FinalArgs<T, S> &a, int u, int slot, int te0, int npos, int C)
+{
+    const int GUr = a.gu;
+    const int g = slot / GUr, ul = slot % GUr;
+    const int PLg = (1 << a.gj[g]) - 1;
+    const unsigned *H = a.hist + (a.grow[g] + g) * GUr + ul;
+    const S *PS = a.pos_score + (a.grow[g] + g) * GUr + ul;
+    const int pc = min(POS_CHUNK, npos);
+    unsigned long long above = 0, sum_ranks = 0;
+    double s2 = 0;
+    int nvalid = 0;
+    constexpr int B = 8;
+    for (int b0 = PLg; b0 >= 1; b0 -= B) {
+        unsigned hb[B]; S pb[B];
+        #pragma unroll
+        for (int q = 0; q < B; q++) {
+            const int b = b0 - q;
+            hb[q] = b >= 1 ? H[(size_t)b * GUr] : 0u;
+            pb[q] = (b >= 1 && b - 1 < pc) ? PS[(size_t)(b - 1) * GUr] : (S)INFINITY;
+        }
+        #pragma unroll
+        for (int q = 0; q < B; q++) {
+            const int b = b0 - q;
+            if (b < 1) break;
+            above += hb[q];
+            const int j = b - 1;
+            if (j >= pc) continue;
+            const S ps = pb[q];
+            if (isinf(ps) && ps > 0) continue;
+            const unsigned long long rank = above + 1;
+            sum_ranks += rank; nvalid++;
+            s2 += (double)nvalid / (double)rank;
+            if (a.rank_sorted) a.rank_sorted[te0 + j] = (long long)rank;
+        }
+    }
+    const unsigned long long P = (unsigned long long)npos, Nneg = (unsigned long long)C - P;
+    if (a.roc) a.roc[u] = (T)(1. - (double)(sum_ranks - (P * (P + 1)) / 2) / (double)(P * Nneg));
+    if (a.pr) a.pr[u] = (T)(s2 / (double)npos);
 }
 
 template <class T, class S>
@@ -842,8 +925,7 @@
 __global__ void k_finalize(FinalArgs<T, S> a)
 {
     extern __shared__ __attribute__((aligned(16))) char fin_smem[];
-    T *topv_base = (T *)fin_smem;
-    unsigned short *head_base = (unsigned short *)(fin_smem + sizeof(T) * (a.K < FIN_TOPV ? a.K : FIN_TOPV) * FIN_THREADS);
+    unsigned short *head_base = (unsigned short *)fin_smem;
     const int slot = a.fin_slot0 + blockIdx.x * blockDim.x + threadIdx.x;
     if (slot >= a.fin_slot1 || a.slot_chunk[slot] != 0) return;
     const int u = a.slot_user[slot];
@@ -853,7 +935,6 @@
     if (a.status) a.status[u] = 1;
     Entry<S> *M = a.merged + (size_t)u * K;
     const bool merged_ready = a.ext_topk || a.collected;
-    if (!merged_ready) for (int i = 0; i < K; i++) { M[i].s = (S)qnan<float>(); M[i].idx = -1; }
 
     const int ntr = a.train_p[u + 1] - a.train_p[u];
     const int C = n - ntr;
@@ -861,6 +942,43 @@
     const int base = a.uslot_base[u];
     const int s0 = a.slot_index[base];
     const int NP = a.n_part;
+    const int W = K < C ? K : C;
+
+    const int *ti = a.test_i + te0;
+    const T *tv = a.test_v ? a.test_v + te0 : nullptr;
+    const size_t st = (size_t)u * K;
+    T *cp = a.p ? a.p + st : nullptr, *ctp = a.tp ? a.tp + st : nullptr, *cr = a.r ? a.r + st : nullptr;
+    T *cap = a.ap ? a.ap + st : nullptr, *ctap = a.tap ? a.tap + st : nullptr, *cndcg = a.ndcg ? a.ndcg + st : nullptr;
+    T *chit = a.hit ? a.hit + st : nullptr, *crr = a.rr ? a.rr + st : nullptr;
+    const bool cum = a.cumulative;
+
+    const bool top = a.req & (RQ_P | RQ_TP | RQ_R | RQ_AP | RQ_TAP | RQ_NDCG | RQ_HIT | RQ_RR);
+    const bool walked = top && (!kleqn || (a.req & (RQ_AP | RQ_TAP | RQ_RR | RQ_NDCG)));
+    int hits = 0, first = 0x7fffffff;
+    double avg_p = 0, dcg = 0;
+    auto walk_place = [&](int ix, int item, bool search) {
+        if (search) {
+            int lo = 0, hi = npos;
+            while (lo < hi) { const int mid = (lo + hi) >> 1; if (ti[mid] < item) lo = mid + 1; else hi = mid; }
+            if (lo < npos && ti[lo] == item) {
+                hits++;
+                avg_p += hits / (double)(ix + 1);
+                dcg += tv ? ((double)tv[lo] / a.log2tab[ix]) : 0.;
+                first = first < ix ? first : ix;
+            }
+        }
+        if (cum) {
+            const int mn = (ix + 1) < npos ? (ix + 1) : npos;
+            if (cp) cp[ix] = (T)(hits / (double)(ix + 1));
+            if (ctp) ctp[ix] = (T)(hits / (double)mn);
+            if (cr) cr[ix] = (T)(hits / (double)npos);
+            if (cap) cap[ix] = (T)(avg_p / (double)npos);
+            if (ctap) ctap[ix] = (T)(avg_p / (double)mn);
+            if (cndcg) cndcg[ix] = (T)dcg;
+            if (chit) chit[ix] = (T)(hits > 0);
+            if (crr) crr[ix] = (T)(hits ? ((double)1 / (double)(first + 1)) : 0.);
+        }
+    };
 
     unsigned short *head = head_base + threadIdx.x;
     unsigned short *alive = head_base + (size_t)NP * FIN_THREADS + threadIdx.x;
@@ -876,28 +994,75 @@
         vmin = ps.vmin < vmin ? ps.vmin : vmin;
         any_nan |= ps.has_nan != 0;
     }
-    for (int i = 0; i < (merged_ready ? 0 : K); i++) {
-        int best = -1; Entry<S> be; be.s = 0; be.idx = 0;
-        for (int t = 0; t < n_alive; t++) {
-            const int q = alive[t * FIN_THREADS];
-            const int hq = head[q * FIN_THREADS];
-            if (hq >= K) continue;
-            const Entry<S> e = PL[(size_t)q * K + hq];
-            if (best < 0 || ent_before(e, be)) { best = q; be = e; }
-        }
-        if (best >= 0) head[best * FIN_THREADS]++;
-        else be.idx = IDX_EMPTY;
+    const int xq = (a.part_extra && !merged_ready) ? NP - 1 : -1;
+    S m_first = 0, m_last = 0; int m_last_idx = -1;
+    bool zone = false;
+    auto place = [&](int i, Entry<S> be, bool from_extra) {
         if (be.idx == IDX_EMPTY) { be.idx = -1; be.s = (S)qnan<float>(); }
         M[i] = be;
-    }
-    const int W = K < C ? K : C;
+        if (i == 0) m_first = be.s;
+        if (i == W - 1) { m_last = be.s; m_last_idx = be.idx; }
+        if (i < W) {
+            zone |= (be.s < (S)0 ? -be.s : be.s) < (S)6.103515625e-05f;
+            if (walked) walk_place(i, be.idx, xq < 0 || from_extra);
+        }
+    };
+    if (!merged_ready && n_alive <= FIN_HEADS) {
+        Entry<S> he[FIN_HEADS]; int hq[FIN_HEADS], hh[FIN_HEADS];
+        #pragma unroll
+        for (int t = 0; t < FIN_HEADS; t++) {
+            hq[t] = t < n_alive ? (int)alive[t * FIN_THREADS] : 0;
+            hh[t] = t < n_alive ? 0 : K;
+            he[t].s = 0; he[t].idx = IDX_EMPTY;
+            if (t < n_alive) he[t] = PL[(size_t)hq[t] * K];
+        }
+        for (int i = 0; i < K; i++) {
+            int bt = -1; Entry<S> be; be.s = 0; be.idx = 0;
+            #pragma unroll
+            for (int t = 0; t < FIN_HEADS; t++)
+                if (hh[t] < K && (bt < 0 || ent_before(he[t], be))) { bt = t; be = he[t]; }
+            bool from_extra = false;
+            if (bt >= 0) {
+                int qb = 0, nh = 0;
+                #pragma unroll
+                for (int t = 0; t < FIN_HEADS; t++) if (t == bt) { qb = hq[t]; nh = ++hh[t]; }
+                from_extra = qb == xq;
+                Entry<S> ne; ne.s = 0; ne.idx = IDX_EMPTY;
+                if (nh < K) ne = PL[(size_t)qb * K + nh];
+                #pragma unroll
+                for (int t = 0; t < FIN_HEADS; t++) if (t == bt) he[t] = ne;
+            } else be.idx = IDX_EMPTY;
+            place(i, be, from_extra);
+        }
+    } else if (!merged_ready) {
+        for (int i = 0; i < K; i++) {
+            int best = -1; Entry<S> be; be.s = 0; be.idx = 0;
+            for (int t = 0; t < n_alive; t++) {
+                const int q = alive[t * FIN_THREADS];
+                const int hq = head[q * FIN_THREADS];
+                if (hq >= K) continue;
+                const Entry<S> e = PL[(size_t)q * K + hq];
+                if (best < 0 || ent_before(e, be)) { best = q; be = e; }
+            }
+            if (best >= 0) head[best * FIN_THREADS]++;
+            else be.idx = IDX_EMPTY;
+            place(i, be, best == xq);
+        }
+    } else {
+        m_first = M[0].s; m_last = M[W - 1].s; m_last_idx = M[W - 1].idx;
+        for (int i = 0; i < W; i++) {
+            const Entry<S> e = M[i];
+            zone |= (e.s < (S)0 ? -e.s : e.s) < (S)6.103515625e-05f;
+            if (walked) walk_place(i, e.idx, true);
+        }
+    }
 
     const bool ref_full = ((a.req & RQ_ROC) && !only_ndcg) || K >= C;
     bool invalid = any_nan;
     if (a.noise) invalid |= (vmax == vmin) || isinf(vmax) || isinf(vmin);
     else {
-        const S hi = M[0].s, lo = ref_full ? vmin : M[W - 1].s;
-        invalid |= isinf(hi) || isinf(lo) || hi == lo || M[W - 1].idx < 0;
+        const S hi = m_first, lo = ref_full ? vmin : m_last;
+        invalid |= isinf(hi) || isinf(lo) || hi == lo || m_last_idx < 0;
     }
     if (invalid) {
         for (int i = 0; i < K; i++) { M[i].s = (S)qnan<float>(); M[i].idx = -1; }
@@ -905,48 +1070,9 @@
         fill_user_nan(a, u); return;
     }
     if (a.status) a.status[u] = 0;
-    if (a.noise_flag) {
-        bool zone = false;
-        for (int i = 0; i < W; i++) { const S x = M[i].s; zone |= (x < (S)0 ? -x : x) < (S)6.103515625e-05f; }
-        if (zone && atomicExch(&a.noise_flag[u], 1) == 0) atomicAdd(&a.plan->n_noise_flagged, 1);
-    }
-
-    const int *ti = a.test_i + te0;
-    const T *tv = a.test_v ? a.test_v + te0 : nullptr;
-    const size_t st = (size_t)u * K;
-    T *cp = a.p ? a.p + st : nullptr, *ctp = a.tp ? a.tp + st : nullptr, *cr = a.r ? a.r + st : nullptr;
-    T *cap = a.ap ? a.ap + st : nullptr, *ctap = a.tap ? a.tap + st : nullptr, *cndcg = a.ndcg ? a.ndcg + st : nullptr;
-    T *chit = a.hit ? a.hit + st : nullptr, *crr = a.rr ? a.rr + st : nullptr;
-    const bool cum = a.cumulative;
-
-    const bool top = a.req & (RQ_P | RQ_TP | RQ_R | RQ_AP | RQ_TAP | RQ_NDCG | RQ_HIT | RQ_RR);
-    bool walked = false;
-    int hits = 0, first = 0x7fffffff;
-    double avg_p = 0, dcg = 0;
-    if (top && (!kleqn || (a.req & (RQ_AP | RQ_TAP | RQ_RR | RQ_NDCG)))) {
-        walked = true;
-        for (int ix = 0; ix < W; ix++) {
-            const int item = M[ix].idx;
-            int lo = 0, hi = npos;
-            while (lo < hi) { const int mid = (lo + hi) >> 1; if (ti[mid] < item) lo = mid + 1; else hi = mid; }
-            if (lo < npos && ti[lo] == item) {
-                hits++;
-                avg_p += hits / (double)(ix + 1);
-                dcg += tv ? ((double)tv[lo] / a.log2tab[ix]) : 0.;
-                first = first < ix ? first : ix;
-            }
-            if (cum) {
-                const int mn = (ix + 1) < npos ? (ix + 1) : npos;
-                if (cp) cp[ix] = (T)(hits / (double)(ix + 1));
-                if (ctp) ctp[ix] = (T)(hits / (double)mn);
-                if (cr) cr[ix] = (T)(hits / (double)npos);
-                if (cap) cap[ix] = (T)(avg_p / (double)npos);
-                if (ctap) ctap[ix] = (T)(avg_p / (double)mn);
-                if (cndcg) cndcg[ix] = (T)dcg;
-                if (chit) chit[ix] = (T)(hits > 0);
-                if (crr) crr[ix] = (T)(hits ? ((double)1 / (double)(first + 1)) : 0.);
-            }
-        }
+    if (a.noise_flag && zone && atomicExch(&a.noise_flag[u], 1) == 0) atomicAdd(&a.plan->n_noise_flagged, 1);
+
+    if (walked) {
         if (!cum) {
             const int mn = K < npos ? K : npos;
             if (a.p) a.p[u] = (T)((double)hits / (double)K);
@@ -989,95 +1115,53 @@
         if (slot >= a.auc_defer_slot0) {
             if (a.roc) a.roc[u] = (T)0;
             if (a.pr) a.pr[u] = (T)0;
-        } else finalize_auc(a, u, base, npos, C);
+        } else if (slot < a.stream_slot0 && a.user_nslots[u] == 1) finalize_auc_table(a, u, slot, te0, npos, C);
+        else finalize_auc(a, u, base, npos, C);
     }
 
     if (a.ndcg) {
         const int L = K < npos ? K : npos;
-        constexpr int TOPV = FIN_TOPV;
-        T *topv = topv_base + threadIdx.x;
-        bool has_nan_val = false;
-        const bool buffered = L <= TOPV;
-        auto pick_next = [&](bool have_prev, T pv, int pi, T &ov, int &oi) {
-            bool found = false; T bv = 0; int bi = -1;
-            for (int t = 0; t < npos; t++) {
-                const T x = tv[t];
-                if (have_prev && !(x < pv || (x == pv && t > pi))) continue;
-                if (!found || x > bv) { found = true; bv = x; bi = t; }
-            }
-            ov = bv; oi = bi; return found;
-        };
-        const bool listed = a.heavy_topv && npos > a.heavy_npos && L <= a.heavy_ld;
-        const T *hv = listed ? a.heavy_topv + (size_t)u * a.heavy_ld : nullptr;
-        if (listed) has_nan_val = a.heavy_nan[u] != 0;
-        if (listed && buffered) {
-            for (int i = 0; i < L; i++) topv[i * FIN_THREADS] = hv[i];
-        } else if (listed) {
-        } else if (buffered) {
-            int cnt = 0;
-            T kth = 0;
-            for (int t0 = 0; t0 < npos; t0 += 8) {
-                T xb[8];
-                #pragma unroll
-                for (int q = 0; q < 8; q++) xb[q] = t0 + q < npos ? tv[t0 + q] : (T)0;
-                #pragma unroll
-                for (int q = 0; q < 8; q++) {
-                    if (t0 + q >= npos) break;
-                    const T x = xb[q];
-                    has_nan_val |= x != x;
-                    if (cnt < L || x > kth) {
-                        int j = cnt < L ? cnt : L - 1;
-                        while (j > 0 && topv[(j - 1) * FIN_THREADS] < x) { topv[j * FIN_THREADS] = topv[(j - 1) * FIN_THREADS]; j--; }
-                        topv[j * FIN_THREADS] = x;
-                        cnt = cnt < L ? cnt + 1 : cnt;
-                        if (cnt == L) kth = topv[(L - 1) * FIN_THREADS];
-                    }
-                }
-            }
-        } else {
-            for (int t = 0; t < npos; t++) has_nan_val |= tv[t] != tv[t];
-        }
-        T pv = 0; int pi = -1; bool hp = false;
-        auto next_value = [&](int i) -> T {
-            if (buffered) return topv[i * FIN_THREADS];
-            if (listed) return hv[i];
-            T x; int xi; pick_next(hp, pv, pi, x, xi); hp = true; pv = x; pi = xi; return x;
-        };
-        T vmaxv = 0, vlast = 0;
-        if (buffered) { vmaxv = topv[0]; vlast = topv[(L - 1) * FIN_THREADS]; }
-        else if (listed) { vmaxv = hv[0]; vlast = hv[L - 1]; }
-        else {
-            for (int i = 0; i < L; i++) { const T x = next_value(i); if (i == 0) vmaxv = x; vlast = x; }
-            hp = false; pv = 0; pi = -1;
-        }
+        const T *hv = a.heavy_topv + (size_t)u * a.heavy_ld;
+        const bool has_nan_val = a.heavy_nan[u] != 0;
+        const T vmaxv = hv[0], vlast = hv[L - 1];
         if (has_nan_val || isinf(vmaxv) || isinf(vlast) || vmaxv <= 0) {
             if (!cum) a.ndcg[u] = qnan<T>(); else for (int i = 0; i < K; i++) cndcg[i] = qnan<T>();
             return;
         }
+        constexpr int B = 8;
         double idcg = 0;
         if (!cum) {
-            for (int ix = 0; ix < L; ix++) {
-                const T x = next_value(ix);
-                if (!(vlast >= 0) && x <= 0) break;
-                idcg += (double)x / a.log2tab[ix];
+            bool stop = false;
+            for (int i0 = 0; i0 < L && !stop; i0 += B) {
+                T xb[B]; double lb[B];
+                #pragma unroll
+                for (int q = 0; q < B; q++) { const bool in = i0 + q < L; xb[q] = in ? hv[i0 + q] : (T)0; lb[q] = in ? a.log2tab[i0 + q] : 1.; }
+                #pragma unroll
+                for (int q = 0; q < B; q++) {
+                    if (i0 + q >= L) break;
+                    const T x = xb[q];
+                    if (!(vlast >= 0) && x <= 0) { stop = true; break; }
+                    idcg += (double)x / lb[q];
+                }
             }
             a.ndcg[u] = (T)(dcg / idcg);
         } else {
-            if (vlast >= 0) {
-                for (int ix = 0; ix < L; ix++) {
-                    const T x = next_value(ix);
-                    idcg += (double)x / a.log2tab[ix];
-                    cndcg[ix] = (T)((double)cndcg[ix] / idcg);
+            bool frozen = false;
+            for (int i0 = 0; i0 < L; i0 += B) {
+                T xb[B], cb[B]; double lb[B];
+                #pragma unroll
+                for (int q = 0; q < B; q++) {
+                    const bool in = i0 + q < L;
+                    xb[q] = in ? hv[i0 + q] : (T)0; lb[q] = in ? a.log2tab[i0 + q] : 1.; cb[q] = in ? cndcg[i0 + q] : (T)0;
                 }
-            } else {
-                int ix = 0;
-                for (; ix < L; ix++) {
-                    const T x = next_value(ix);
-                    if (x < 0) break;
-                    idcg += (double)x / a.log2tab[ix];
-                    cndcg[ix] = (T)((double)cndcg[ix] / idcg);
+                #pragma unroll
+                for (int q = 0; q < B; q++) {
+                    if (i0 + q >= L) break;
+                    const T x = xb[q];
+                    frozen |= !(vlast >= 0) && x < 0;
+                    if (!frozen) idcg += (double)x / lb[q];
+                    cndcg[i0 + q] = (T)((double)cb[q] / idcg);
                 }
-                for (; ix < L; ix++) cndcg[ix] = (T)((double)cndcg[ix] / idcg);
             }
             if (npos < K) { const int e = K < C ? K : C; for (int i = npos; i < e; i++) cndcg[i] = cndcg[npos - 1]; }
         }
diff --git a/recometrics_amd/csrc/rm_lib.hip b/recometrics_amd/csrc/rm_lib.hip
--- a/recometrics_amd/csrc/rm_lib.hip
+++ b/recometrics_amd/csrc/rm_lib.hip
@@ -186,6 +186,7 @@
     double acc[4] = {0, 0, 0, 0};
     PackedItems packed; DenseRows dense; DiscountTable discounts;
     bool high_priority = false;
+    unsigned long long dups_tag = 0; bool test_dups = false;
     Plan *pinned_plan = nullptr;
     void stage_ms(float ms[4]) const
     {
@@ -567,7 +568,7 @@
     int u_split, j_shallow; size_t lds_l;
 };
 template <class T>
-Geometry sweep_geometry(const Call<T> &c, const Plan &hp, int NG, bool want_auc, bool want_lane, bool ext_topk, bool check_nan, bool dense_ok,
+Geometry sweep_geometry(const Call<T> &c, const Plan &hp, int NG, bool want_auc, bool want_lane, bool ext_topk, bool check_nan, bool dense_ok, bool test_dups,
                         const Switches &sw)
 {
     typedef Prec<T> P;
@@ -615,7 +616,7 @@
     }
     g.n_splits = n_splits; g.tail_ublocks = tail_ublocks; g.tail_splits = tail_splits;
     g.part_splits = std::max(n_splits, tail_splits);
-    g.mask_test = std::is_same<T, float>::value && want_auc && !ext_topk && !check_nan && hp.n_slots > 0 &&
+    g.mask_test = std::is_same<T, float>::value && want_auc && !ext_topk && !check_nan && hp.n_slots > 0 && !test_dups &&
                   dense_ok && hp.n_slots == hp.n_active && hp.n_only_ndcg == 0 &&
                   nsub * g.part_splits + 1 <= MAX_PARTS && !sw.no_test_mask;
     g.use_ext_bits = c.ext_bits != nullptr && c.ext_words == dense_row_words(n) && (!c.ext_masked || g.mask_test);
@@ -656,7 +657,7 @@
     bool want_lane = false, ext_topk = false, items_known = false, dense_ok = false;
     bool bits_early = false, bits_early_masked = false, masked_from_bits = false, flat_early = false;
     Plan hp{};
-    int n_slots = 0, n_stream = 0, stream_slot0 = 0; bool check_nan = false;
+    int n_slots = 0, n_stream = 0, stream_slot0 = 0; bool check_nan = false, test_dups = false;
     Geometry g{};
     FinalArgs<T, T> fa{};
     Entry<T> *merged = nullptr; long long *rank_sorted = nullptr;
@@ -818,6 +819,11 @@
             break;
         }
         throw_csr_defects(hp, c, cx);
+        if (!c.reco && !c.csr_checked) {
+            if (cx.dups_tag != c.items_tag || c.items_tag == 0) { cx.dups_tag = c.items_tag; cx.test_dups = false; }
+            test_dups = hp.csr_eq_all != hp.csr_eq_legit;
+            cx.test_dups |= test_dups;
+        } else test_dups = !c.reco && c.items_tag != 0 && cx.dups_tag == c.items_tag && cx.test_dups;
         n_slots = hp.n_slots;
         n_stream = (want_auc || ext_topk) ? hp.class_count[STREAM_CLASS] : 0;
         stream_slot0 = n_stream > 0 ? hp.class_offset[STREAM_CLASS] : n_slots;
@@ -831,12 +837,14 @@
 
     void launch_top_values()
     {
-        if (!(fa.ndcg && hp.n_heavy > 0)) return;
-        fa.heavy_ld = std::max(1, std::min(K, hp.max_npos));
+        if (!fa.ndcg) return;
+        fa.heavy_ld = std::max(1, std::min(K, std::max(hp.max_npos, POS_CHUNK)));
         fa.heavy_topv = (T *)ws.get("heavy_topv", sizeof(T) * (size_t)m * (size_t)fa.heavy_ld);
         fa.heavy_nan = (unsigned char *)ws.get("heavy_nan", (size_t)m);
         fa.heavy_users = heavy_users; fa.n_heavy = hp.n_heavy;
-        hipLaunchKernelGGL((k_top_values<T, T>), dim3(cdiv((long long)hp.n_heavy * WAVE, 256)), dim3(256), 0, side.fork(SIDE_FORK), fa);
+        hipStream_t st = side.fork(SIDE_FORK);
+        hipLaunchKernelGGL((k_top_values_rows<T, T>), dim3(cdiv(m, FIN_THREADS)), dim3(FIN_THREADS), top_values_lds_bytes<T>(K), st, fa);
+        if (hp.n_heavy > 0) hipLaunchKernelGGL((k_top_values<T, T>), dim3(cdiv((long long)hp.n_heavy * WAVE, 256)), dim3(256), 0, st, fa);
         side.mark(SIDE_TOP_VALUES);
     }
 
@@ -1077,7 +1085,7 @@
 
     void finalize()
     {
-        fa.n_part = g.n_part; fa.pl = pl; fa.pst = pst; fa.hist = hist; fa.pos_score = pos_score; fa.pos_item_tab = pos_item;
+        fa.n_part = g.n_part; fa.part_extra = g.part_extra; fa.pl = pl; fa.pst = pst; fa.hist = hist; fa.pos_score = pos_score; fa.pos_item_tab = pos_item;
         fa.stream_slot0 = stream_slot0; fa.stream_scores = stream_scores; fa.stream_ld = stream_ld;
         fa.spos_score = spos_score; fa.spos_item = spos_item; fa.shist = shist;
         fa.rank_generic = (g_sw.rank_generic ? 1 : 0);
@@ -1104,9 +1112,9 @@
         if (n_slots > 0) {
             if (want_auc) {
                 if (n_stream > 0 && !ranks_beside) { rank_streamed_rows(0, n_stream, stream); if (auc_launch) auc_streamed_rows(0, n_stream, stream); }
-                if (stream_slot0 > 0) hipLaunchKernelGGL((k_auc_slots<T, T>), dim3(cdiv(stream_slot0, 256)), dim3(256), 0, stream, fa);
+                if (stream_slot0 > 0 && hp.n_slots > hp.n_active) hipLaunchKernelGGL((k_auc_slots<T, T>), dim3(cdiv(stream_slot0, 256)), dim3(256), 0, stream, fa);
             }
-            const size_t fin_lds = finalize_lds_bytes<T>(K, g.n_part);
+            const size_t fin_lds = finalize_lds_bytes(g.n_part);
             HIP_CHECK(hipFuncSetAttribute((const void *)k_finalize<T, T>, hipFuncAttributeMaxDynamicSharedMemorySize, (int)fin_lds));
             fa.auc_defer_slot0 = n_slots;
             if (ranks_beside && (req & (RQ_ROC | RQ_PR)) && !g_sw.no_defer_auc) {
@@ -1144,7 +1152,7 @@
     Pipeline<T> p(c, stream, cx);
     p.begin();
     p.plan_stage();
-    p.g = sweep_geometry<T>(c, p.hp, p.NG, p.want_auc, p.want_lane, p.ext_topk, p.check_nan, p.dense_ok, g_sw);
+    p.g = sweep_geometry<T>(c, p.hp, p.NG, p.want_auc, p.want_lane, p.ext_topk, p.check_nan, p.dense_ok, p.test_dups, g_sw);
     p.prep();
     p.sweep();
     if (c.reco) p.finalize_reco(); else p.finalize();
diff --git a/recometrics_amd/csrc/rm_prep.hpp b/recometrics_amd/csrc/rm_prep.hpp
--- a/recometrics_amd/csrc/rm_prep.hpp
+++ b/recometrics_amd/csrc/rm_prep.hpp
@@ -40,7 +40,7 @@
     if (plan->csr_bad & CSR_BAD_INDPTR) return;
     const long long e0 = indptr[0], e1 = indptr[m];
     const bool aligned = (((size_t)idx) & 15) == 0;
-    unsigned desc = 0; bool bad = false; long long bad_at = 0;
+    unsigned desc = 0, eq = 0; bool bad = false; long long bad_at = 0;
     for (long long g = (e0 >> 2) + (long long)blockIdx.x * blockDim.x + threadIdx.x; (g << 2) < e1; g += (long long)gridDim.x * blockDim.x) {
         const long long e = g << 2;
         if (e >= e0 && e + 4 < e1 && aligned) {
@@ -48,14 +48,14 @@
             const int x4 = idx[e + 4];
             const int x[5] = {q.x, q.y, q.z, q.w, x4};
             #pragma unroll
-            for (int i = 0; i < 4; i++) { if ((unsigned)x[i] >= (unsigned)n) { bad = true; bad_at = e + i; } desc += x[i] > x[i + 1]; }
+            for (int i = 0; i < 4; i++) { if ((unsigned)x[i] >= (unsigned)n) { bad = true; bad_at = e + i; } desc += x[i] > x[i + 1]; eq += x[i] == x[i + 1]; }
         } else {
             for (int i = 0; i < 4; i++) {
                 const long long f = e + i;
                 if (f < e0 || f >= e1) continue;
                 const int v = idx[f];
                 if ((unsigned)v >= (unsigned)n) { bad = true; bad_at = f; }
-                if (f + 1 < e1) desc += v > idx[f + 1];
+                if (f + 1 < e1) { const int w = idx[f + 1]; desc += v > w; eq += v == w; }
             }
         }
     }
@@ -65,37 +65,41 @@
         atomicOr(&plan->csr_bad, CSR_BAD_INDEX); plan->csr_where = lo;
     }
     #pragma unroll
-    for (int d = 32; d >= 1; d >>= 1) desc += __shfl_xor(desc, d);
-    __shared__ unsigned blk;
-    if (threadIdx.x == 0) blk = 0;
+    for (int d = 32; d >= 1; d >>= 1) { desc += __shfl_xor(desc, d); eq += __shfl_xor(eq, d); }
+    __shared__ unsigned blk, blk_eq;
+    if (threadIdx.x == 0) { blk = 0; blk_eq = 0; }
     __syncthreads();
     if ((threadIdx.x & 63) == 0 && desc) atomicAdd(&blk, desc);
+    if ((threadIdx.x & 63) == 0 && eq && which == 1) atomicAdd(&blk_eq, eq);
     __syncthreads();
     if (threadIdx.x == 0 && blk) atomicAdd(&plan->csr_desc_all[which], (unsigned long long)blk);
+    if (threadIdx.x == 0 && blk_eq) atomicAdd(&plan->csr_eq_all, (unsigned long long)blk_eq);
 }
 __global__ __launch_bounds__(1024) void k_check_csr_starts(int m, const int *train_p, const int *train_i, const int *test_p, const int *test_i, Plan *plan)
 {
     if (plan->csr_bad & CSR_BAD_INDPTR) return;
-    __shared__ unsigned blk[2];
-    if (threadIdx.x < 2) blk[threadIdx.x] = 0;
+    __shared__ unsigned blk[3];
+    if (threadIdx.x < 3) blk[threadIdx.x] = 0;
     __syncthreads();
     const int u = blockIdx.x * blockDim.x + threadIdx.x;
-    unsigned d0 = 0, d1 = 0;
+    unsigned d0 = 0, d1 = 0, q1 = 0;
     if (u >= 1 && u < m) {
         const int s = train_p[u], e1 = train_p[m], e0 = train_p[0];
         if (train_p[u - 1] < s && s > e0 && s < e1) d0 = train_i[s - 1] > train_i[s];
         if (test_p) {
             const int t = test_p[u], f1 = test_p[m], f0 = test_p[0];
-            if (test_p[u - 1] < t && t > f0 && t < f1) d1 = test_i[t - 1] > test_i[t];
-        }
-    }
-    const unsigned long long b0 = __ballot(d0), b1 = __ballot(d1);
+            if (test_p[u - 1] < t && t > f0 && t < f1) { const int x = test_i[t - 1], y = test_i[t]; d1 = x > y; q1 = x == y; }
+        }
+    }
+    const unsigned long long b0 = __ballot(d0), b1 = __ballot(d1), b2 = __ballot(q1);
     if ((threadIdx.x & 63) == 0) {
         if (b0) atomicAdd(&blk[0], (unsigned)__popcll(b0));
         if (b1) atomicAdd(&blk[1], (unsigned)__popcll(b1));
+        if (b2) atomicAdd(&blk[2], (unsigned)__popcll(b2));
     }
     __syncthreads();
     if (threadIdx.x < 2 && blk[threadIdx.x]) atomicAdd(&plan->csr_desc_legit[threadIdx.x], (unsigned long long)blk[threadIdx.x]);
+    if (threadIdx.x == 2 && blk[2]) atomicAdd(&plan->csr_eq_legit, (unsigned long long)blk[2]);
 }
 
 __global__ void k_classify(ClassifyArgs a)
```

Result: no change. 17.60 million (-0.2%).
